# suyashk12/hipgp

Hardware: NVIDIA B200
Metric: toeplitz_matvec_GBps_in_pcg_1e6grid (higher is better)
Workload: dtype f32

## Files before the change

### hipgp_b200/csrc/cols_blk_kernel.cuh

```cuda
#pragma once
#include "fast_kernels.cuh"
#include "tma_maps.cuh"

namespace hipgp {

#ifdef HIPGP_EMU
static inline void nbar_sync(int id, int count) { emu::g_named_barrier[id].sync(count); }
static inline void warp_sync_all() {
    const int tid = (int)(threadIdx.x + blockDim.x * (threadIdx.y + blockDim.y * threadIdx.z));
    emu::g_warp_barrier[tid >> 5].wait();
}
#else
__device__ __forceinline__ void nbar_sync(int id, int count) { asm volatile("bar.sync %0, %1;" ::"r"(id), "r"(count) : "memory"); }
__device__ __forceinline__ void warp_sync_all() { __syncwarp(); }
#endif

template <int GS> __device__ __forceinline__ void blk_sync(int b) {
    if (GS == 32) warp_sync_all(); else nbar_sync(1 + b, GS);
}

template <int R, int S, class T>
__device__ __forceinline__ void blk_fill_pairs(TwPair<T>* dst, const cplx<T>* tab, int tid, int nt) {
    for (int i = tid; i < TwPairs<R>::n * S; i += nt) { const int p = i / S; dst[i] = tw_pair_global<R, S, T>(tab, p, i - p * S); }
}
template <int R, int S, bool SM, class T> __device__ __forceinline__ TwPair<T> blk_pair(const cplx<T>* tab, int p, int j) {
    return SM ? reinterpret_cast<const TwPair<T>*>(tab)[p * S + j] : tw_pair_global<R, S, T>(tab, p, j);
}

template <int R, int S, bool SM, class T>
__device__ __forceinline__ void blk_twiddles(cplx<T>* w, const cplx<T>* tab, int j) {
#pragma unroll
    for (int p = 0; p < TwPairs<R>::n; ++p) {
        const TwPair<T> e = blk_pair<R, S, SM, T>(tab, p, j);
        w[2 * p + 1] = e.a;
        if (2 * p + 2 < R) w[2 * p + 2] = e.b;
    }
}

template <int R, int S, bool SM, bool CONJ, int CH, class T>
__device__ __forceinline__ void blk_twiddle_mul(Lane<T>* v, const cplx<T>* tab, int j) {
    constexpr int PC = CH / 2 > 0 ? CH / 2 : 1;
#pragma unroll
    for (int p0 = 0; p0 < TwPairs<R>::n; p0 += PC) {
        TwPair<T> e[PC];
#pragma unroll
        for (int c = 0; c < PC; ++c) if (p0 + c < TwPairs<R>::n) e[c] = blk_pair<R, S, SM, T>(tab, p0 + c, j);
#pragma unroll
        for (int c = 0; c < PC; ++c) if (p0 + c < TwPairs<R>::n) {
            const int r = 2 * (p0 + c) + 1;
            v[r] = CONJ ? lmulc(v[r], e[c].a) : lmul(v[r], e[c].a);
            if (r + 1 < R) v[r + 1] = CONJ ? lmulc(v[r + 1], e[c].b) : lmul(v[r + 1], e[c].b);
        }
#ifndef HIPGP_EMU
        if (p0 + PC < TwPairs<R>::n) asm volatile("" ::: "memory");
#endif
    }
}

template <class T, int NL, int NT, int MINB, int R0, int R1, int R2>
struct ColsBlkCfg {
    using G = TileGeo<T, NL, R0, R1, R2>;
    static constexpr int Ln = G::Ln, BS = Ln / R0, GS = NT / R0;
    static constexpr int IB2 = (BS / R1) * NL, IB3 = (BS / R2) * NL;
    static constexpr bool ok = (NT % R0 == 0) && (GS % 32 == 0) && (GS == 32 || R0 <= 15) && (IB2 % GS == 0) && (IB3 % GS == 0) &&
                               ((IB2 / GS) * R1 <= 16) && ((IB3 / GS) * R2 <= 16) && (BS % R2 == 0);
    static constexpr size_t tw_bytes = 2 * sizeof(cplx<T>) * (size_t)((R0 / 2) * (Ln / R0) + (R1 / 2) * (BS / R1));
    static constexpr size_t side_bytes = (size_t)(Ln + Ln / R2) * NL * 8;
    static constexpr bool tw_smem = (size_t)MINB * (G::smem_bytes() + side_bytes + tw_bytes + 1024) <= 228 * 1024;
    static constexpr size_t smem_bytes = G::smem_bytes() + side_bytes + (tw_smem ? tw_bytes : 0);
};

template <class T, int NL, int NT, int MINB, int R0, int R1, int R2>
__global__ void __launch_bounds__(NT, MINB) cols_blk_kernel(const HIPGP_GRID_CONSTANT ColsParams<T> P, const HIPGP_GRID_CONSTANT ColsTmaMaps maps) {
    using Cfg = ColsBlkCfg<T, NL, NT, MINB, R0, R1, R2>;
    using G = typename Cfg::G;
    constexpr int Ln = G::Ln, RLAST = R2, LPT = LaneInfo<T>::LPT, TBL = NL * LPT, S0 = Ln / R0;
    constexpr int BS = Cfg::BS, GS = Cfg::GS, S1 = BS / R1;
    constexpr bool TWS = Cfg::tw_smem;
    constexpr int TWCH = R0 >= 16 ? 5 : R0;
    static_assert(Cfg::ok, "radix list / tile shape not usable with block-local middle sections");
    constexpr int LEG0 = G::leg(S0), LEG1 = G::leg(S1);
    constexpr int SPEC_LANE = 8;
    constexpr int SIDE_SLOTS = Ln + Ln / RLAST;
    constexpr int SIDE_LANES = SIDE_SLOTS * NL / 2;
    HIPGP_DYN_SMEM(smem_raw);
    Lane<T>* s = reinterpret_cast<Lane<T>*>(smem_raw);
    unsigned char* side = smem_raw + G::smem_bytes();
    const int tid = threadIdx.x;
    if (P.done_flag && *P.done_flag) return;
    const int blk = tid / GS, u = tid - blk * GS;

    const cplx<T>* tw0 = P.f.twst + P.f.twoff[0];
    const cplx<T>* tw1 = P.f.twst + P.f.twoff[1];
    __shared__ unsigned long long s_bar[3];
    const bool tma_in = P.tma_in != 0, tma_spec = P.tma_spec != 0;
    if ((tma_in || tma_spec) && tid == 0) { tma_bar_init(&s_bar[0]); tma_bar_init(&s_bar[1]); warps_bar_init(&s_bar[2], NT / 32); tma_fence_before_issue(); }
    if (tma_in || tma_spec) __syncthreads();
    if (TWS) {
        TwPair<T>* t0 = reinterpret_cast<TwPair<T>*>(side + Cfg::side_bytes);
        TwPair<T>* t1 = t0 + TwPairs<R0>::n * S0;
        blk_fill_pairs<R0, S0, T>(t0, tw0, tid, NT);
        blk_fill_pairs<R1, S1, T>(t1, tw1, tid, NT);
        tw0 = reinterpret_cast<const cplx<T>*>(t0); tw1 = reinterpret_cast<const cplx<T>*>(t1);
        __syncthreads();
    }

    const int mode = P.mode;
    const size_t pitch = (size_t)P.pitch;
    const size_t spitch = P.spec_pitch ? (size_t)P.spec_pitch : (size_t)P.pitch;
    const long ntiles = (long)P.nx * P.ny * P.nz;
    unsigned tile_bz = 0;
    auto tile_origin = [&](long t, long& c0, size_t& ioff, size_t& ooff) {
        const unsigned tt = (unsigned)t, nx = (unsigned)P.nx, ny = (unsigned)P.ny, nz = (unsigned)P.nz;
        unsigned bx, by, bz;
        if (P.batch_fastest) { bz = tt % nz; const unsigned r = tt / nz; bx = r % nx; by = r / nx; }
        else { bx = tt % nx; const unsigned r = tt / nx; by = r % ny; bz = r / ny; }
        c0 = (long)bx * TBL;
        tile_bz = bz;
        ioff = (size_t)by * P.in_ostride + (size_t)bz * P.in_bstride + c0;
        ooff = (size_t)by * P.out_ostride + (size_t)bz * P.out_bstride + c0;
    };
    auto sslot = [](int p) { return p + (p >> G::LOGRL); };
    const bool spec_smem = P.spec_stage != 0;
    const int n_in = P.n_in, n_out = P.n_out;
    const bool stage_in = P.in_stage != 0;
    const bool zero_hi = is_pow2(R0) && n_in <= Ln / 2;
    const bool out_lo = is_pow2(R0) && n_out <= Ln / 2;
    const size_t rstep = (size_t)S0 * pitch;

    auto prefetch_input = [&](long t) {
        long c0; size_t ioff, ooff;
        tile_origin(t, c0, ioff, ooff);
        const long nvalid = P.inner - c0;
        const cplx<T>* in = P.in + ioff;
        constexpr int NIT = (SIDE_LANES + NT - 1) / NT;
        const int total = n_in * NL;
#pragma unroll
        for (int k = 0; k < NIT; ++k) {
            const int w = tid + k * NT;
            const int i = w / NL, lane = w - i * NL;
            if (w < total && (long)lane * LPT < nvalid) cp_async<16>(side + (size_t)w * 16, in + (size_t)i * pitch + lane * LPT);
        }
        cp_async_commit();
    };

    auto issue_input = [&](long t) {
        long c0; size_t ioff, ooff;
        tile_origin(t, c0, ioff, ooff);
        const unsigned box_bytes = (unsigned)P.tma_in_rows * NL * 16u;
        tma_fence_before_issue();
        tma_bar_expect(&s_bar[0], box_bytes * (unsigned)P.tma_in_nbox);
        for (int k = 0; k < P.tma_in_nbox; ++k)
            tma_load_box3(side + (size_t)k * box_bytes, &maps.in, (int)(2 * c0), k * P.tma_in_rows, (int)tile_bz, &s_bar[0]);
    };
    auto stage_next = [&](long tn) {
        if (tn >= ntiles) return;
        if (tma_in) { if (tid == 0) issue_input(tn); }
        else if (stage_in) prefetch_input(tn);
    };

    stage_next((long)blockIdx.x);
    for (unsigned iter = 0;; ++iter) {
        const long t = (long)blockIdx.x + (long)iter * gridDim.x;
        if (t >= ntiles) break;
        const unsigned ph = iter & 1u;
        long c0; size_t ioff, ooff;
        tile_origin(t, c0, ioff, ooff);
        const long nvalid = P.inner - c0;
        const cplx<T>* in = P.in + ioff;
        cplx<T>* out = P.out + ooff;
        if (tma_in) { tma_bar_wait(&s_bar[0], ph, 8, NT); if (mode != CM_FUSED) __syncthreads(); }
        else { cp_async_wait_all(); __syncthreads(); }

        if (mode != CM_INV) {
#pragma unroll 1
            for (int it = tid; it < S0 * NL; it += NT) {
                const int lane = it % NL, j = it / NL;
                const bool ok = (long)lane * LPT < nvalid;
                Lane<T> v[R0];
                if (tma_in) {
                    const Lane<T>* sp = reinterpret_cast<const Lane<T>*>(side) + (j * NL + lane);
#pragma unroll
                    for (int r = 0; r < R0 / 2; ++r) v[r] = sp[r * S0 * NL];
                    lbfly_zero_hi<R0, T>(v);
                } else if (stage_in) {
                    const Lane<T>* sp = reinterpret_cast<const Lane<T>*>(side) + (j * NL + lane);
                    if (zero_hi) {
#pragma unroll
                        for (int r = 0; r < R0 / 2; ++r) v[r] = (ok && j + r * S0 < n_in) ? sp[r * S0 * NL] : lzero<T>();
                        lbfly_zero_hi<R0, T>(v);
                    } else {
#pragma unroll
                        for (int r = 0; r < R0; ++r) v[r] = (ok && j + r * S0 < n_in) ? sp[r * S0 * NL] : lzero<T>();
                        lbfly<R0, false, T>(v);
                    }
                } else {
                    const cplx<T>* gp = in + (size_t)j * pitch + lane * LPT;
                    if (zero_hi) {
#pragma unroll
                        for (int r = 0; r < R0 / 2; ++r) v[r] = (ok && j + r * S0 < n_in) ? lane_from_global(gp + r * rstep) : lzero<T>();
                        lbfly_zero_hi<R0, T>(v);
                    } else {
#pragma unroll
                        for (int r = 0; r < R0; ++r) v[r] = (ok && j + r * S0 < n_in) ? lane_from_global(gp + r * rstep) : lzero<T>();
                        lbfly<R0, false, T>(v);
                    }
                }
                blk_twiddle_mul<R0, S0, TWS, false, TWCH>(v, tw0, j);
                Lane<T>* base = s + (G::slot(j) * NL + lane);
#pragma unroll
                for (int r = 0; r < R0; ++r) base[r * LEG0] = v[r];
            }
            __syncthreads();
            if (!(mode == CM_FUSED && spec_smem)) stage_next(t + gridDim.x);
        }

        const int pb = blk * BS;
        if (mode == CM_FUSED && spec_smem && tma_spec) {
            if (tid == 0) {
                tma_fence_before_issue();
                tma_bar_expect(&s_bar[1], (unsigned)Cfg::side_bytes);
                tma_load_box3(side, &maps.spec, (int)c0, 0, 0, &s_bar[1]);
            }
        } else if (mode == CM_FUSED && spec_smem) {
            const unsigned char* sp = reinterpret_cast<const unsigned char*>(P.spec) + (size_t)c0 * sizeof(T);
            constexpr int ROWB = NL * SPEC_LANE;
            constexpr int CH = ROWB >= 16 ? 16 : 8, NCH = ROWB / CH;
            constexpr int NIT = (BS * NCH + GS - 1) / GS;
#pragma unroll
            for (int k = 0; k < NIT; ++k) {
                const int w = u + k * GS;
                const int p = pb + w / NCH, c = w % NCH;
                if (w < BS * NCH) cp_async<CH>(side + (size_t)sslot(p) * ROWB + c * CH, sp + (size_t)p * spitch * sizeof(T) + c * CH);
            }
            cp_async_commit();
        }
        if (mode != CM_INV) {
            constexpr int NIT = Cfg::IB2 / GS;
            Lane<T> v[NIT][R1];
            cplx<T> w[NIT][R1];
            Lane<T>* base[NIT];
#pragma unroll
            for (int k = 0; k < NIT; ++k) {
                const int q = u + k * GS;
                const int lane = q % NL, j = q / NL;
                base[k] = s + (G::slot(pb + j) * NL + lane);
                blk_twiddles<R1, S1, TWS>(w[k], tw1, j);
#pragma unroll
                for (int r = 0; r < R1; ++r) v[k][r] = base[k][r * LEG1];
            }
#pragma unroll
            for (int k = 0; k < NIT; ++k) {
                lbfly<R1, false, T>(v[k]);
#pragma unroll
                for (int r = 1; r < R1; ++r) v[k][r] = lmul(v[k][r], w[k][r]);
#pragma unroll
                for (int r = 0; r < R1; ++r) base[k][r * LEG1] = v[k][r];
            }
            if (mode == CM_FUSED && spec_smem) {
                if (tma_spec) tma_bar_wait(&s_bar[1], ph, 9, NT);
                else cp_async_wait_all();
            }
            blk_sync<GS>(blk);
        }
        {
            constexpr int NIT = Cfg::IB3 / GS;
// ... 106 lines not shown
```

### hipgp_b200/csrc/conv_kernels.cuh

```cuda
#pragma once
#include "fft_engine.cuh"

namespace hipgp {

enum RowsFwdMode { RF_PLAIN = 0, RF_PUPDATE = 1, RF_XRUPDATE = 2, RF_SELFDOT = 3 };
enum RowsInvMode { RI_PLAIN = 0, RI_DOT = 1 };
enum DotKind { DOT_PAP = 0, DOT_ZR = 1, DOT_RR = 2 };
enum ColsMode { CM_FWD = 0, CM_INV = 1, CM_FUSED = 2 };
enum SpecKind { SPEC_NONE = 0, SPEC_REAL = 1, SPEC_CPLX = 2, SPEC_CPLX_CONJ = 3 };

struct PcgDev {
    double* zr;
    double* zr_prev;
    double* pAp;
    double* rr;
    const double* rr_all;
    double* partial;
    unsigned* row_cnt;
    unsigned* rhs_cnt;
    int* flags;
    double tol;
    int B;
    int cg_mode;
};

template <class T> __device__ __forceinline__ T warp_sum(T v) {
#pragma unroll
    for (int o = 16; o > 0; o >>= 1) v += __shfl_xor_sync(0xffffffffu, v, o);
    return v;
}

__device__ __forceinline__ void pcg_finalize(const PcgDev& st, int kind, long g0, long g1, int nrows, int tid, int nthreads) {
    __shared__ unsigned s_last;
    __shared__ double s_red[32];
    const int b0 = (int)(g0 / nrows), b1 = (int)((g1 - 1) / nrows);
    for (int b = b0; b <= b1; ++b) {
        const long lo = g0 > (long)b * nrows ? g0 : (long)b * nrows;
        const long hi = g1 < (long)(b + 1) * nrows ? g1 : (long)(b + 1) * nrows;
        __syncthreads();
        if (tid == 0) {
            __threadfence();
            const unsigned done = atomicAdd(st.row_cnt + b, (unsigned)(hi - lo)) + (unsigned)(hi - lo);
            s_last = (done == (unsigned)nrows);
        }
        __syncthreads();
        if (!s_last) continue;
        __threadfence();
        double acc = 0.0;
        const volatile double* part = st.partial + (long)b * nrows;
        for (int i = tid; i < nrows; i += nthreads) acc += part[i];
        acc = warp_sum(acc);
        if ((tid & 31) == 0) s_red[tid >> 5] = acc;
        __syncthreads();
        if (tid < 32) {
            double v = tid < (nthreads >> 5) ? s_red[tid] : 0.0;
            v = warp_sum(v);
            if (tid == 0) {
                st.row_cnt[b] = 0;
                if (kind == DOT_PAP) st.pAp[b] = v;
                else if (kind == DOT_ZR) { st.zr_prev[b] = st.zr[b]; st.zr[b] = v; }
                else {
                    st.rr[b] = v;
                    if (st.cg_mode) { st.zr_prev[b] = st.zr[b]; st.zr[b] = v; }
                }
                __threadfence();
                if (kind == DOT_RR) {
                    const unsigned nb = atomicAdd(st.rhs_cnt, 1u) + 1u;
                    if (nb == (unsigned)st.B) {
                        __threadfence();
                        bool all = true;
                        const volatile double* rr = st.rr_all ? st.rr_all : st.rr;
                        for (int i = 0; i < st.B; ++i) all = all && (sqrt(rr[i]) < st.tol);
                        st.rhs_cnt[0] = 0;
                        st.flags[1] += 1;
                        st.flags[2] = 0;
                        if (all) st.flags[0] = 1;
                    }
                }
            }
        }
    }
}

template <class T>
struct RowsParams {
    const T* in;
    T* out;
    T* v0;
    T* v1;
    const T* v2;
    cplx<T>* W;
    long total_rows;
    int nrows;
    int n_real;
    int L, H;
    long W_pitch;
    int W_rows;
    LineFft<T> f;
    const cplx<T>* twL;
    const cplx<T>* twLp;
    const int* part;
    const int* pairq;
    const int* pairs; const cplx<T>* pairw; int npair0;
    const int* quadq; const cplx<T>* quadw; int nquad;
    int RB, RBP;
    int mode, dot_kind, do_fft;
    int vec_ok;
    int vec16_ok;
    int tma_ok;
    int tma_op;
    const void* spec; int spec_kind;
    PcgDev st;
};

template <class T>
__global__ void __launch_bounds__(256) rows_fwd_kernel(RowsParams<T> P) {
    HIPGP_DYN_SMEM(smem_raw);
    cplx<T>* s = reinterpret_cast<cplx<T>*>(smem_raw);
    const int tid = threadIdx.x, nthreads = blockDim.x;
    const int warp = tid >> 5, lane = tid & 31, nwarps = nthreads >> 5;
    if (P.mode != RF_PLAIN && P.st.flags[0]) return;
    const long g0 = (long)blockIdx.x * P.RB;
    const long g1 = g0 + P.RB < P.total_rows ? g0 + P.RB : P.total_rows;
    const int nl = (int)(g1 - g0);
    const int H = P.H, RBP = P.RBP, n = P.n_real;

    for (int line = warp; line < P.RB; line += nwarps) {
        if (line >= nl) {
            if (P.do_fft) for (int k = lane; k < H; k += 32) s[(size_t)k * RBP + line] = mk<T>(0, 0);
            continue;
        }
        const long g = g0 + line;
        const int b = (int)(g / P.nrows);
        const size_t off = (size_t)g * n;
        T acc = 0;
        T coef = 0;
        bool first = false;
        if (P.mode == RF_PUPDATE) {
            first = P.st.flags[2] != 0;
            coef = first ? (T)0 : (T)(P.st.zr[b] / P.st.zr_prev[b]);
        } else if (P.mode == RF_XRUPDATE) {
            coef = (T)(P.st.zr[b] / P.st.pAp[b]);
        }
        for (int k = lane; k < H; k += 32) {
            T e[2];
#pragma unroll
            for (int h = 0; h < 2; ++h) {
                const int i = 2 * k + h;
                T val = 0;
                if (i < n) {
                    if (P.mode == RF_PLAIN) {
                        val = P.in[off + i];
                    } else if (P.mode == RF_PUPDATE) {
                        const T z = P.in[off + i];
                        val = first ? z : z + coef * P.v0[off + i];
                        P.v0[off + i] = val;
                    } else if (P.mode == RF_SELFDOT) {
                        val = P.in[off + i];
                        acc += val * val;
                    } else {
                        const T pv = P.v2[off + i];
                        P.v1[off + i] = P.v1[off + i] + coef * pv;
                        val = P.v0[off + i] - coef * P.in[off + i];
                        P.v0[off + i] = val;
                        acc += val * val;
                    }
                }
                e[h] = val;
            }
            if (P.do_fft) s[(size_t)k * RBP + line] = mk<T>(e[0], e[1]);
        }
        if (P.mode == RF_XRUPDATE || P.mode == RF_SELFDOT) {
            const double tot = warp_sum((double)acc);
            if (lane == 0) P.st.partial[g] = tot;
        }
    }
    if (P.mode == RF_XRUPDATE) pcg_finalize(P.st, DOT_RR, g0, g1, P.nrows, tid, nthreads);
    if (P.mode == RF_SELFDOT) pcg_finalize(P.st, DOT_ZR, g0, g1, P.nrows, tid, nthreads);
    if (!P.do_fft) return;
    __syncthreads();

    fft_forward(s, RBP, P.RB, P.f, tid, nthreads);

    for (int w = tid; w < H * P.RB; w += nthreads) {
        const int line = w % P.RB, p = w / P.RB;
        const int k = P.f.rev[p];
        if (k == 0) {
            const cplx<T> z = s[line];
            s[line] = mk<T>((T)2 * (z.x + z.y), 0);
            s[(size_t)H * RBP + line] = mk<T>((T)2 * (z.x - z.y), 0);
        } else {
            const int k2 = H - k;
            if (k <= k2) {
                const int p2 = P.f.pos[k2];
                const cplx<T> a = s[(size_t)p * RBP + line], c = conj(s[(size_t)p2 * RBP + line]);
                const cplx<T> E = a + c;
                const cplx<T> d = a - c;
                const cplx<T> O = mk<T>(d.y, -d.x);
                const cplx<T> t = P.twL[k] * O;
                s[(size_t)p * RBP + line] = E + t;
                if (k != k2) s[(size_t)p2 * RBP + line] = conj(E - t);
            }
        }
    }
    __syncthreads();

    for (int line = warp; line < nl; line += nwarps) {
        const long g = g0 + line;
        cplx<T>* dst = P.W + ((size_t)(g / P.nrows) * P.W_rows + (g % P.nrows)) * P.W_pitch;
        for (int q = lane; q <= H; q += 32) dst[q] = s[(size_t)q * RBP + line];
    }
}

template <class T>
__device__ __forceinline__ cplx<T> apply_spec(cplx<T> v, const void* spec, int kind, size_t idx) {
    if (kind == SPEC_REAL) return v * reinterpret_cast<const T*>(spec)[idx];
    const cplx<T> sv = reinterpret_cast<const cplx<T>*>(spec)[idx];
    return kind == SPEC_CPLX ? v * sv : mulc(v, sv);
}

template <class T>
__global__ void __launch_bounds__(256) rows_inv_kernel(RowsParams<T> P) {
    HIPGP_DYN_SMEM(smem_raw);
    cplx<T>* s = reinterpret_cast<cplx<T>*>(smem_raw);
    const int tid = threadIdx.x, nthreads = blockDim.x;
    const int warp = tid >> 5, lane = tid & 31, nwarps = nthreads >> 5;
    if (P.mode != RI_PLAIN && P.st.flags[0]) return;
    const long g0 = (long)blockIdx.x * P.RB;
    const long g1 = g0 + P.RB < P.total_rows ? g0 + P.RB : P.total_rows;
    const int nl = (int)(g1 - g0);
    const int H = P.H, RBP = P.RBP, n = P.n_real;

    for (int line = warp; line < P.RB; line += nwarps) {
        if (line >= nl) {
            for (int q = lane; q <= H; q += 32) s[(size_t)q * RBP + line] = mk<T>(0, 0);
            continue;
        }
        const long g = g0 + line;
        const cplx<T>* src = P.W + ((size_t)(g / P.nrows) * P.W_rows + (g % P.nrows)) * P.W_pitch;
        for (int q = lane; q <= H; q += 32) {
            cplx<T> v = src[q];
            if (P.spec_kind != SPEC_NONE) v = apply_spec(v, P.spec, P.spec_kind, (size_t)q);
            s[(size_t)q * RBP + line] = v;
        }
    }
    __syncthreads();

    for (int w = tid; w < H * P.RB; w += nthreads) {
        const int line = w % P.RB, p = w / P.RB;
        const int k = P.f.rev[p];
        if (k == 0) {
            const T y0 = s[line].x, yh = s[(size_t)H * RBP + line].x;
            s[line] = mk<T>(y0 + yh, y0 - yh);
        } else {
            const int k2 = H - k;
            if (k <= k2) {
                const int p2 = P.f.pos[k2];
                const cplx<T> a = s[(size_t)p * RBP + line], c = conj(s[(size_t)p2 * RBP + line]);
                const cplx<T> E = a + c;
                const cplx<T> O = mulc(a - c, P.twL[k]);
                const cplx<T> iO = mk<T>(-O.y, O.x);
                s[(size_t)p * RBP + line] = E + iO;
                if (k != k2) s[(size_t)p2 * RBP + line] = conj(E - iO);
            }
        }
    }
    __syncthreads();

    fft_inverse(s, RBP, P.RB, P.f, tid, nthreads);

    for (int line = warp; line < nl; line += nwarps) {
        const long g = g0 + line;
        const size_t off = (size_t)g * n;
        T acc = 0;
        for (int k = lane; k < H; k += 32) {
            const cplx<T> z = s[(size_t)k * RBP + line];
            const int i = 2 * k;
            if (i < n) { P.out[off + i] = z.x; if (P.mode == RI_DOT) acc += z.x * P.v0[off + i]; }
            if (i + 1 < n) { P.out[off + i + 1] = z.y; if (P.mode == RI_DOT) acc += z.y * P.v0[off + i + 1]; }
        }
        if (P.mode == RI_DOT) {
            const double tot = warp_sum((double)acc);
            if (lane == 0) P.st.partial[g] = tot;
        }
    }
    if (P.mode == RI_DOT) pcg_finalize(P.st, P.dot_kind, g0, g1, P.nrows, tid, nthreads);
}

template <class T>
struct ColsParams {
    const cplx<T>* in;
    cplx<T>* out;
    int n_in, n_out;
    long inner;
    long pitch;
    long in_ostride, in_bstride, out_ostride, out_bstride;
    LineFft<T> f;
    int TB, TBP;
    int mode;
    const void* spec; int spec_kind;
    long spec_pitch;
    int spec_stage;
    int in_stage;
    int nx, ny, nz;
    int tma_in, tma_in_rows, tma_in_nbox;
    int tma_spec;
    int batch_fastest;
    const int* done_flag;
    int out_split_len; long out_split_stride;
    int in_split_len; long in_split_stride;
};
template <class T> __device__ __forceinline__ size_t cols_rowoff(int i, long pitch, int split_len, long split_stride) {
    return split_len ? (size_t)(i / split_len) * split_stride + (size_t)(i % split_len) * pitch : (size_t)i * pitch;
}

template <class T>
__global__ void __launch_bounds__(512) cols_pass_kernel(ColsParams<T> P) {
    HIPGP_DYN_SMEM(smem_raw);
    cplx<T>* s = reinterpret_cast<cplx<T>*>(smem_raw);
    const int tid = threadIdx.x, nthreads = blockDim.x;
    if (P.done_flag && *P.done_flag) return;
    const long c0 = (long)blockIdx.x * P.TB;
    const int nc = (int)(P.inner - c0 < P.TB ? P.inner - c0 : P.TB);
    const int L = P.f.Ln, TB = P.TB, TBP = P.TBP;
    const cplx<T>* in = P.in + (size_t)blockIdx.y * P.in_ostride + (size_t)blockIdx.z * P.in_bstride + c0;
    cplx<T>* out = P.out + (size_t)blockIdx.y * P.out_ostride + (size_t)blockIdx.z * P.out_bstride + c0;

    const int rows_in = P.mode == CM_INV ? L : P.n_in;
    for (int w = tid; w < L * TB; w += nthreads) {
        const int c = w % TB, i = w / TB;
        cplx<T> v = mk<T>(0, 0);
        if (i < rows_in && c < nc) v = in[cols_rowoff<T>(i, P.pitch, P.in_split_len, P.in_split_stride) + c];
        s[(size_t)i * TBP + c] = v;
    }
    __syncthreads();

    if (P.mode != CM_INV) fft_forward(s, TBP, TB, P.f, tid, nthreads);
    if (P.mode == CM_FUSED) {
        for (int w = tid; w < L * TB; w += nthreads) {
            const int c = w % TB, i = w / TB;
            if (c < nc) s[(size_t)i * TBP + c] = apply_spec(s[(size_t)i * TBP + c], P.spec, P.spec_kind, (size_t)i * (P.spec_pitch ? P.spec_pitch : P.pitch) + c0 + c);
        }
        __syncthreads();
    }
    if (P.mode != CM_FWD) fft_inverse(s, TBP, TB, P.f, tid, nthreads);

    const int rows_out = P.mode == CM_FWD ? L : P.n_out;
    for (int w = tid; w < rows_out * TB; w += nthreads) {
        const int c = w % TB, i = w / TB;
        if (c < nc) out[cols_rowoff<T>(i, P.pitch, P.out_split_len, P.out_split_stride) + c] = s[(size_t)i * TBP + c];
    }
}


}
```

### hipgp_b200/csrc/fast_kernels.cuh

```cuda
#pragma once
#include "lane_fft.cuh"

namespace hipgp {

template <class T> __device__ __forceinline__ void ld2(const T* p, bool vec, T& a, T& b, bool ok0, bool ok1) {
    if (vec && ok1) { const cplx<T> t = ld_stream(reinterpret_cast<const cplx<T>*>(p)); a = t.x; b = t.y; }
    else { a = ok0 ? ld_stream(p) : (T)0; b = ok1 ? ld_stream(p + 1) : (T)0; }
}
template <class T> __device__ __forceinline__ void st2(T* p, bool vec, T a, T b, bool ok0, bool ok1) {
    if (vec && ok1) { st_stream(reinterpret_cast<cplx<T>*>(p), mk<T>(a, b)); }
    else { if (ok0) st_stream(p, a); if (ok1) st_stream(p + 1, b); }
}

__device__ __forceinline__ double team_sum(double v, int tw) {
    for (int o = tw >> 1; o > 0; o >>= 1) v += __shfl_xor_sync(0xffffffffu, v, o);
    return v;
}

__device__ __forceinline__ Lane<float> lane_spec(Lane<float> v, const void* spec, int kind, size_t idx) {
    if (kind == SPEC_REAL) {
        const cplx<float> sv = ld_stream(reinterpret_cast<const cplx<float>*>(reinterpret_cast<const float*>(spec) + idx));
        return lmul_real2(v, sv.x, sv.y);
    }
    const cplx<float>* sp = reinterpret_cast<const cplx<float>*>(spec) + idx;
    const cplx<float> w0 = ld_stream(sp), w1 = ld_stream(sp + 1);
    return kind == SPEC_CPLX ? lmul_cplx2<false>(v, w0, w1) : lmul_cplx2<true>(v, w0, w1);
}
__device__ __forceinline__ Lane<double> lane_spec(Lane<double> v, const void* spec, int kind, size_t idx) {
    if (kind == SPEC_REAL) return lscale(v, ld_stream(reinterpret_cast<const double*>(spec) + idx));
    const cplx<double> w = ld_stream(reinterpret_cast<const cplx<double>*>(spec) + idx);
    return kind == SPEC_CPLX ? lmul(v, w) : lmulc(v, w);
}
__device__ __forceinline__ Lane<float> lane_spec_smem(Lane<float> v, const void* p) {
    const float2 s2 = *reinterpret_cast<const float2*>(p);
    Lane<float> r; r.re = __fmul2_rn(v.re, s2); r.im = __fmul2_rn(v.im, s2); return r;
}
__device__ __forceinline__ Lane<double> lane_spec_smem(Lane<double> v, const void* p) { return lscale(v, *reinterpret_cast<const double*>(p)); }

template <class T, int NL, int NT, int MINB, int R0, int... Rs>
__global__ void __launch_bounds__(NT, MINB) cols_fast_kernel(ColsParams<T> P) {
    using G = TileGeo<T, NL, R0, Rs...>;
    constexpr int Ln = G::Ln, NST = G::NST, RLAST = G::RLAST, LPT = LaneInfo<T>::LPT, TBL = NL * LPT, S0 = Ln / R0;
    HIPGP_DYN_SMEM(smem_raw);
    Lane<T>* s = reinterpret_cast<Lane<T>*>(smem_raw);
    const int tid = threadIdx.x;
    if (P.done_flag && *P.done_flag) return;
    const int mode = P.mode;
    const size_t pitch = (size_t)P.pitch;
    const size_t spitch = P.spec_pitch ? (size_t)P.spec_pitch : (size_t)P.pitch;
    const long ntiles = (long)P.nx * P.ny * P.nz;
    auto tile_origin = [&](long t, long& c0, size_t& ioff, size_t& ooff) {
        long bx, by, bz;
        if (P.batch_fastest) { bz = t % P.nz; const long r = t / P.nz; bx = r % P.nx; by = r / P.nx; }
        else { bx = t % P.nx; const long r = t / P.nx; by = r % P.ny; bz = r / P.ny; }
        c0 = bx * TBL;
        ioff = (size_t)by * P.in_ostride + (size_t)bz * P.in_bstride + c0;
        ooff = (size_t)by * P.out_ostride + (size_t)bz * P.out_bstride + c0;
    };

    if constexpr (NST == 1) {
        for (long t = blockIdx.x; t < ntiles; t += gridDim.x) {
            long c0; size_t ioff, ooff;
            tile_origin(t, c0, ioff, ooff);
            const long nvalid = P.inner - c0;
            const cplx<T>* in = P.in + ioff;
            cplx<T>* out = P.out + ooff;
            for (int lane = tid; lane < NL; lane += NT) {
                if ((long)lane * LPT >= nvalid) continue;
                const int rows_in = mode == CM_INV ? Ln : P.n_in;
                const int rows_out = mode == CM_FWD ? Ln : P.n_out;
                Lane<T> v[R0];
#pragma unroll
                for (int r = 0; r < R0; ++r)
                    v[r] = r < rows_in ? lane_from_global(in + cols_rowoff<T>(r, P.pitch, P.in_split_len, P.in_split_stride) + lane * LPT) : lzero<T>();
                if (mode != CM_INV) lbfly<R0, false, T>(v);
                if (mode == CM_FUSED) {
#pragma unroll
                    for (int r = 0; r < R0; ++r) v[r] = lane_spec(v[r], P.spec, P.spec_kind, (size_t)r * spitch + c0 + lane * LPT);
                }
                if (mode != CM_FWD) lbfly<R0, true, T>(v);
#pragma unroll
                for (int r = 0; r < R0; ++r)
                    if (r < rows_out) lane_to_global(out + cols_rowoff<T>(r, P.pitch, P.out_split_len, P.out_split_stride) + lane * LPT, v[r]);
            }
        }
        return;
    } else {
        constexpr int LEG0 = G::leg(S0);
        constexpr int SPEC_LANE = 8;
        constexpr int SIDE_SLOTS = Ln + Ln / RLAST;
        constexpr int SIDE_LANES = SIDE_SLOTS * NL / 2;
        unsigned char* side = smem_raw + G::smem_bytes();
        auto sslot = [](int p) { return p + (p >> G::LOGRL); };
        const cplx<T>* tw0 = P.f.twst + P.f.twoff[0];
        const bool spec_smem = P.spec_stage != 0;
        const int n_in = P.n_in, n_out = P.n_out;
        const bool stage_in = P.in_stage != 0;
        const bool zero_hi = is_pow2(R0) && n_in <= Ln / 2;
        const bool out_lo = is_pow2(R0) && n_out <= Ln / 2;
        const size_t rstep = (size_t)S0 * pitch;

        auto prefetch_input = [&](long t) {
            long c0; size_t ioff, ooff;
            tile_origin(t, c0, ioff, ooff);
            const long nvalid = P.inner - c0;
            const cplx<T>* in = P.in + ioff;
            constexpr int NIT = (SIDE_LANES + NT - 1) / NT;
            const int total = n_in * NL;
#pragma unroll
            for (int k = 0; k < NIT; ++k) {
                const int w = tid + k * NT;
                const int i = w / NL, lane = w - i * NL;
                if (w < total && (long)lane * LPT < nvalid) cp_async<16>(side + (size_t)w * 16, in + (size_t)i * pitch + lane * LPT);
            }
            cp_async_commit();
        };

        long t = blockIdx.x;
        if (stage_in && t < ntiles) prefetch_input(t);
        for (; t < ntiles; t += gridDim.x) {
            long c0; size_t ioff, ooff;
            tile_origin(t, c0, ioff, ooff);
            const long nvalid = P.inner - c0;
            const cplx<T>* in = P.in + ioff;
            cplx<T>* out = P.out + ooff;
            cp_async_wait_all();
            __syncthreads();

            if (mode != CM_INV) {
#pragma unroll 1
                for (int it = tid; it < S0 * NL; it += NT) {
                    const int lane = it % NL, j = it / NL;
                    const bool ok = (long)lane * LPT < nvalid;
                    cplx<T> w[R0];
                    lane_twiddles<R0, S0>(w, tw0, j);
                    Lane<T> v[R0];
                    if (stage_in) {
                        const Lane<T>* sp = reinterpret_cast<const Lane<T>*>(side) + (j * NL + lane);
                        if (zero_hi) {
#pragma unroll
                            for (int r = 0; r < R0 / 2; ++r) v[r] = (ok && j + r * S0 < n_in) ? sp[r * S0 * NL] : lzero<T>();
                            lbfly_zero_hi<R0, T>(v);
                        } else {
#pragma unroll
                            for (int r = 0; r < R0; ++r) v[r] = (ok && j + r * S0 < n_in) ? sp[r * S0 * NL] : lzero<T>();
                            lbfly<R0, false, T>(v);
                        }
                    } else {
                        const cplx<T>* gp = in + (size_t)j * pitch + lane * LPT;
                        if (zero_hi) {
#pragma unroll
                            for (int r = 0; r < R0 / 2; ++r) v[r] = (ok && j + r * S0 < n_in) ? lane_from_global(gp + r * rstep) : lzero<T>();
                            lbfly_zero_hi<R0, T>(v);
                        } else {
#pragma unroll
                            for (int r = 0; r < R0; ++r) v[r] = (ok && j + r * S0 < n_in) ? lane_from_global(gp + r * rstep) : lzero<T>();
                            lbfly<R0, false, T>(v);
                        }
                    }
#pragma unroll
                    for (int r = 1; r < R0; ++r) v[r] = lmul(v[r], w[r]);
                    Lane<T>* base = s + (G::slot(j) * NL + lane);
#pragma unroll
                    for (int r = 0; r < R0; ++r) base[r * LEG0] = v[r];
                }
                __syncthreads();
                if (spec_smem) {
                    const unsigned char* sp = reinterpret_cast<const unsigned char*>(P.spec) + (size_t)c0 * sizeof(T);
                    constexpr int ROWB = NL * SPEC_LANE;
                    constexpr int CH = ROWB >= 16 ? 16 : 8, NCH = ROWB / CH;
                    constexpr int NIT = (Ln * NCH + NT - 1) / NT;
#pragma unroll
                    for (int k = 0; k < NIT; ++k) {
                        const int w = tid + k * NT;
                        const int p = w / NCH, c = w - p * NCH;
                        if (w < Ln * NCH) cp_async<CH>(side + (size_t)sslot(p) * ROWB + c * CH, sp + (size_t)p * spitch * sizeof(T) + c * CH);
                    }
                    cp_async_commit();
                }
                LaneMidFwd<G, T, NL, NT, Ln / R0, 1, Rs...>::run(s, P.f, tid);
                if (spec_smem) { cp_async_wait_all(); __syncthreads(); }
            }

            {
#pragma unroll 2
                for (int it = tid; it < (Ln / RLAST) * NL; it += NT) {
                    const int lane = it % NL, bf = it / NL;
                    const bool ok = (long)lane * LPT < nvalid;
                    const int p0 = bf * RLAST;
                    Lane<T>* base = s + (G::slot(p0) * NL + lane);
                    Lane<T> v[RLAST];
                    if (mode == CM_INV) {
                        const cplx<T>* gp = in + cols_rowoff<T>(p0, P.pitch, P.in_split_len, P.in_split_stride) + lane * LPT;
#pragma unroll
                        for (int r = 0; r < RLAST; ++r) v[r] = ok ? lane_from_global(gp + r * pitch) : lzero<T>();
                    } else {
#pragma unroll
                        for (int r = 0; r < RLAST; ++r) v[r] = base[r * NL];
                        lbfly<RLAST, false, T>(v);
                    }
                    if (mode == CM_FUSED) {
                        if (spec_smem) {
                            const unsigned char* sp = side + ((size_t)sslot(p0) * NL + lane) * SPEC_LANE;
#pragma unroll
                            for (int r = 0; r < RLAST; ++r) v[r] = lane_spec_smem(v[r], sp + r * NL * SPEC_LANE);
                        } else if (ok) {
                            const size_t sidx = (size_t)p0 * spitch + c0 + lane * LPT;
#pragma unroll
                            for (int r = 0; r < RLAST; ++r) v[r] = lane_spec(v[r], P.spec, P.spec_kind, sidx + (size_t)r * spitch);
                        }
                    }
                    if (mode == CM_FWD) {
                        if (ok) {
                            cplx<T>* gp = out + cols_rowoff<T>(p0, P.pitch, P.out_split_len, P.out_split_stride) + lane * LPT;
#pragma unroll
                            for (int r = 0; r < RLAST; ++r) lane_to_global(gp + r * pitch, v[r]);
                        }
                    } else {
                        lbfly<RLAST, true, T>(v);
#pragma unroll
                        for (int r = 0; r < RLAST; ++r) base[r * NL] = v[r];
                    }
                }
                __syncthreads();
            }
            if (stage_in && t + gridDim.x < ntiles) prefetch_input(t + gridDim.x);
            if (mode == CM_FWD) continue;

            LaneMidInv<G, T, NL, NT, Ln / R0, 1, Rs...>::run(s, P.f, tid);
            {
#pragma unroll 1
                for (int it = tid; it < S0 * NL; it += NT) {
                    const int lane = it % NL, j = it / NL;
                    const bool ok = (long)lane * LPT < nvalid;
                    cplx<T> w[R0];
                    lane_twiddles<R0, S0>(w, tw0, j);
                    const Lane<T>* base = s + (G::slot(j) * NL + lane);
                    Lane<T> v[R0];
#pragma unroll
                    for (int r = 0; r < R0; ++r) v[r] = base[r * LEG0];
#pragma unroll
                    for (int r = 1; r < R0; ++r) v[r] = lmulc(v[r], w[r]);
                    cplx<T>* gp = out + (size_t)j * pitch + lane * LPT;
                    lbfly<R0, true, T>(v);
                    if (ok) {
                        if (out_lo) {
#pragma unroll
                            for (int r = 0; r < R0 / 2; ++r) if (j + r * S0 < n_out) lane_to_global(gp + r * rstep, v[r]);
                        } else {
#pragma unroll
                            for (int r = 0; r < R0; ++r) if (j + r * S0 < n_out) lane_to_global(gp + r * rstep, v[r]);
                        }
                    }
                }
            }
        }
    }
}

struct __align__(8) QuadIdx { int a, b; };

template <class T, int NL, int NT, int MINB, int R0, int... Rs>
__global__ void __launch_bounds__(NT, MINB) rows_fwd_fast_kernel(RowsParams<T> P) {
    using G = TileGeo<T, NL, R0, Rs...>;
    constexpr int H = G::Ln, NST = G::NST, RLAST = G::RLAST, LPT = LaneInfo<T>::LPT, NROW = NL * LPT, S0 = H / R0;
    constexpr int LEG0 = G::leg(NST > 1 ? S0 : 1);
    HIPGP_DYN_SMEM(smem_raw);
    Lane<T>* s = reinterpret_cast<Lane<T>*>(smem_raw);
    const int tid = threadIdx.x;
    if (P.mode != RF_PLAIN && P.st.flags[0]) return;
    const long g0 = (long)blockIdx.x * NROW;
    const long g1 = g0 + NROW < P.total_rows ? g0 + NROW : P.total_rows;
    const int nl = (int)(g1 - g0);
    const int n = P.n_real;
    const int mode = P.mode;
    const bool vec = ((n & 1) == 0) && P.vec_ok;
    const bool first_it = (mode == RF_PUPDATE) && (P.st.flags[2] != 0);
    const bool want_dot = (mode == RF_XRUPDATE || mode == RF_SELFDOT);
    __shared__ T s_coef[32];
    __shared__ long s_wbase[32];
    __shared__ double s_part[32];
    if (tid < NROW && tid < nl) {
        const long gr = g0 + tid;
        const long b = gr / P.nrows;
        s_wbase[tid] = (b * P.W_rows + (gr - b * P.nrows)) * P.W_pitch;
        T coef = 0;
        if (mode == RF_PUPDATE) coef = first_it ? (T)0 : (T)(P.st.zr[b] / P.st.zr_prev[b]);
        else if (mode == RF_XRUPDATE) coef = (T)(P.st.zr[b] / P.st.pAp[b]);
        s_coef[tid] = coef;
    }
    __syncthreads();

    const int SROW = (n + 3) & ~3;
    T* side = reinterpret_cast<T*>(smem_raw + G::smem_bytes());
    bool streamed = false;
#ifndef HIPGP_EMU
    bool bulk_store_pending = false;
    if (P.tma_ok && P.vec16_ok && SROW == n && (mode == RF_PLAIN || mode == RF_SELFDOT || P.tma_op)) {
        constexpr int CH = 16 / (int)sizeof(T);
        __shared__ __align__(8) unsigned long long s_mbar;
        const unsigned bytes = (unsigned)((size_t)nl * n * sizeof(T));
        const size_t goff = (size_t)g0 * n;
        T* bufA = reinterpret_cast<T*>(smem_raw);
        T* bufB = bufA + (size_t)NROW * SROW;
        const bool two = mode == RF_PUPDATE && !first_it, three = mode == RF_XRUPDATE;
        if (tid == 0) { mbar_init(&s_mbar, 1); fence_proxy_async(); }
        __syncthreads();
        if (tid == 0) {
            mbar_arrive_expect_tx(&s_mbar, bytes * (three ? 3u : (two ? 2u : 1u)));
            bulk_g2s(side, P.in + goff, bytes, &s_mbar);
            if (two) bulk_g2s(bufA, (const T*)P.v0 + goff, bytes, &s_mbar);
            if (three) { bulk_g2s(bufA, (const T*)P.v0 + goff, bytes, &s_mbar); bulk_g2s(bufB, P.v2 + goff, bytes, &s_mbar); }
        }
        constexpr int NW = NT / 32, WPR = NW > NROW ? NW / NROW : 1;
        constexpr int tws = WPR > 1 ? 32 : (H / CH >= 32 ? 32 : (H / CH >= 16 ? 16 : (H / CH >= 8 ? 8 : 4)));
        constexpr int rpw = 32 / tws, TW = WPR > 1 ? 32 * WPR : tws, rstep = WPR > 1 ? NW / WPR : NW * rpw;
        const int warp = tid >> 5, l32 = tid & 31;
        const int ln = WPR > 1 ? l32 + 32 * (warp % WPR) : l32 % tws;
        const int nch = n / CH;
        mbar_wait(&s_mbar, 0);
        if (mode != RF_PLAIN && !(mode == RF_PUPDATE && first_it)) {
            for (int rbase = WPR > 1 ? warp / WPR : warp * rpw; rbase < nl; rbase += rstep) {
                const int row = rbase + (WPR > 1 ? 0 : l32 / tws);
                const bool ractive = row < nl;
                double acc = 0.0;
                if (ractive) {
                    T* srow = side + (size_t)row * SROW;
                    const T* arow = bufA + (size_t)row * SROW;
                    const T* brow = bufB + (size_t)row * SROW;
                    const size_t off = goff + (size_t)row * n;
                    const T coef = s_coef[row];
                    if (three) {
                        constexpr int BS = 4;
                        for (int cb = ln; cb < nch; cb += TW * BS) {
                            Vec16<T> xv[BS];
#pragma unroll
                            for (int k = 0; k < BS; ++k) { const int c = cb + TW * k; if (c < nch) xv[k] = ldv_stream((const T*)P.v1 + off + (size_t)c * CH); }
#pragma unroll
                            for (int k = 0; k < BS; ++k) {
                                const int c = cb + TW * k;
                                if (c < nch) {
                                    Vec16<T> q = *reinterpret_cast<const Vec16<T>*>(srow + c * CH);
                                    const Vec16<T> rv = *reinterpret_cast<const Vec16<T>*>(arow + c * CH);
                                    const Vec16<T> pv = *reinterpret_cast<const Vec16<T>*>(brow + c * CH);
#pragma unroll
                                    for (int e = 0; e < CH; ++e) { xv[k].v[e] = xv[k].v[e] + coef * pv.v[e]; q.v[e] = rv.v[e] - coef * q.v[e]; acc += (double)(q.v[e] * q.v[e]); }
                                    stv_stream(P.v1 + off + (size_t)c * CH, xv[k]);
                                    *reinterpret_cast<Vec16<T>*>(srow + c * CH) = q;
                                }
                            }
                        }
                    } else if (two) {
                        for (int c = ln; c < nch; c += TW) {
                            Vec16<T> z = *reinterpret_cast<const Vec16<T>*>(srow + c * CH);
                            const Vec16<T> pv = *reinterpret_cast<const Vec16<T>*>(arow + c * CH);
#pragma unroll
                            for (int e = 0; e < CH; ++e) z.v[e] = z.v[e] + coef * pv.v[e];
                            *reinterpret_cast<Vec16<T>*>(srow + c * CH) = z;
                        }
                    } else {
                        for (int c = ln; c < nch; c += TW) {
                            const Vec16<T> z = *reinterpret_cast<const Vec16<T>*>(srow + c * CH);
#pragma unroll
                            for (int e = 0; e < CH; ++e) acc += (double)(z.v[e] * z.v[e]);
                        }
                    }
                }
                if (want_dot) {
                    acc = team_sum(acc, WPR > 1 ? 32 : tws);
                    if (ractive && (WPR > 1 ? l32 == 0 : ln == 0)) s_part[row * WPR + warp % WPR] = acc;
                }
            }
        }
        if (mode == RF_PUPDATE || mode == RF_XRUPDATE) {
            fence_proxy_async();
            __syncthreads();
            if (tid == 0) {
                asm volatile("cp.async.bulk.global.shared::cta.bulk_group [%0], [%1], %2;" ::"l"(P.v0 + goff), "r"((unsigned)__cvta_generic_to_shared(side)), "r"(bytes) : "memory");
                asm volatile("cp.async.bulk.commit_group;" ::: "memory");
            }
            bulk_store_pending = true;
        }
        if (want_dot) {
            __syncthreads();
            if (tid < nl) { double a = 0.0; for (int k = 0; k < WPR; ++k) a += s_part[tid * WPR + k]; P.st.partial[g0 + tid] = a; }
        }
        streamed = true;
    }
#endif
    if (!streamed) {
        constexpr int CH = 16 / (int)sizeof(T);
        constexpr int NW = NT / 32, WPR = NW > NROW ? NW / NROW : 1;
        const bool chunked = P.vec16_ok && (n % CH == 0);
        constexpr int tws = WPR > 1 ? 32 : (H / CH >= 32 ? 32 : (H / CH >= 16 ? 16 : (H / CH >= 8 ? 8 : 4)));
        constexpr int rpw = 32 / tws;
        constexpr int TW = WPR > 1 ? 32 * WPR : tws;
        const int warp = tid >> 5, l32 = tid & 31;
        const int ln = WPR > 1 ? l32 + 32 * (warp % WPR) : l32 % tws;
        constexpr int rstep = WPR > 1 ? NW / WPR : NW * rpw;
        for (int rbase = WPR > 1 ? warp / WPR : warp * rpw; rbase < nl; rbase += rstep) {
            const int row = rbase + (WPR > 1 ? 0 : l32 / tws);
            const bool ractive = row < nl;
            T* srow = side + (size_t)(ractive ? row : 0) * SROW;
            const size_t off = (size_t)(g0 + (ractive ? row : 0)) * n;
            const T coef = s_coef[ractive ? row : 0];
            double acc = 0.0;
            if (!ractive) {
            } else if (chunked) {
                const int nch = n / CH;
                auto finish = [&](int c, Vec16<T> a) {
                    if (want_dot) {
#pragma unroll
                        for (int k = 0; k < CH; ++k) acc += (double)(a.v[k] * a.v[k]);
                    }
                    *reinterpret_cast<Vec16<T>*>(srow + c * CH) = a;
                };
#define HIPGP_PIPE(LOAD, PROC)                                                                              \
                {                                                                                           \
                    const int step = TW * BS;                                                               \
                    int cb = ln;                                                                            \
                    LOAD(0, cb);                                                                            \
                    for (; cb < nch; cb += 2 * step) {                                                      \
                        if (cb + step < nch) { LOAD(1, cb + step); }                                        \
                        PROC(0, cb);                                                                        \
                        if (cb + 2 * step < nch) { LOAD(0, cb + 2 * step); }                                \
                        if (cb + step < nch) { PROC(1, cb + step); }                                        \
                    }                                                                                       \
                }
                if (mode == RF_XRUPDATE) {
                    constexpr int BS = 1;
                    Vec16<T> a[2][BS], pv[2][BS], xv[2][BS], rv[2][BS];
#define HIPGP_LD(S, CB)                                                                                     \
                    _Pragma("unroll") for (int k = 0; k < BS; ++k) {                                        \
                        const int c = (CB) + TW * k;                                                        \
                        if (c < nch) {                                                                      \
                            const size_t o = off + (size_t)c * CH;                                          \
                            a[S][k] = ldv_stream(P.in + o); pv[S][k] = ldv_stream(P.v2 + o);                \
                            xv[S][k] = ldv_stream((const T*)P.v1 + o); rv[S][k] = ldv_stream((const T*)P.v0 + o); \
                        }                                                                                   \
                    }
#define HIPGP_PR(S, CB)                                                                                     \
                    _Pragma("unroll") for (int k = 0; k < BS; ++k) {                                        \
                        const int c = (CB) + TW * k;                                                        \
                        if (c < nch) {                                                                      \
                            const size_t o = off + (size_t)c * CH;                                          \
                            _Pragma("unroll") for (int e = 0; e < CH; ++e) {                                \
                                xv[S][k].v[e] = xv[S][k].v[e] + coef * pv[S][k].v[e];                       \
                                a[S][k].v[e] = rv[S][k].v[e] - coef * a[S][k].v[e];                         \
                            }                                                                               \
                            stv_stream(P.v1 + o, xv[S][k]);                                                 \
                            stv_stream(P.v0 + o, a[S][k]);                                                  \
                            finish(c, a[S][k]);                                                             \
                        }                                                                                   \
                    }
                    HIPGP_PIPE(HIPGP_LD, HIPGP_PR)
#undef HIPGP_LD
#undef HIPGP_PR
                } else if (mode == RF_PUPDATE && !first_it) {
                    constexpr int BS = 2;
                    Vec16<T> a[2][BS], pv[2][BS];
#define HIPGP_LD(S, CB)                                                                                     \
                    _Pragma("unroll") for (int k = 0; k < BS; ++k) {                                        \
                        const int c = (CB) + TW * k;                                                        \
                        if (c < nch) { const size_t o = off + (size_t)c * CH; a[S][k] = ldv_stream(P.in + o); pv[S][k] = ldv_stream((const T*)P.v0 + o); } \
                    }
#define HIPGP_PR(S, CB)                                                                                     \
                    _Pragma("unroll") for (int k = 0; k < BS; ++k) {                                        \
                        const int c = (CB) + TW * k;                                                        \
                        if (c < nch) {                                                                      \
                            _Pragma("unroll") for (int e = 0; e < CH; ++e) a[S][k].v[e] = a[S][k].v[e] + coef * pv[S][k].v[e]; \
                            stv_stream(P.v0 + off + (size_t)c * CH, a[S][k]);                               \
                            finish(c, a[S][k]);                                                             \
                        }                                                                                   \
                    }
                    HIPGP_PIPE(HIPGP_LD, HIPGP_PR)
#undef HIPGP_LD
#undef HIPGP_PR
                } else {
                    constexpr int BS = 4;
                    const bool wr = mode == RF_PUPDATE;
                    Vec16<T> a[2][BS];
#define HIPGP_LD(S, CB)                                                                                     \
                    _Pragma("unroll") for (int k = 0; k < BS; ++k) { const int c = (CB) + TW * k; if (c < nch) a[S][k] = ldv_stream(P.in + off + (size_t)c * CH); }
#define HIPGP_PR(S, CB)                                                                                     \
                    _Pragma("unroll") for (int k = 0; k < BS; ++k) {                                        \
                        const int c = (CB) + TW * k;                                                        \
                        if (c < nch) { if (wr) stv_stream(P.v0 + off + (size_t)c * CH, a[S][k]); finish(c, a[S][k]); } \
                    }
                    HIPGP_PIPE(HIPGP_LD, HIPGP_PR)
#undef HIPGP_LD
#undef HIPGP_PR
                }
#undef HIPGP_PIPE
            } else {
                for (int i = ln; i < n; i += TW) {
                    const size_t o = off + i;
                    T a = ld_stream(P.in + o);
                    if (mode == RF_PUPDATE) {
                        if (!first_it) a = a + coef * ld_stream((const T*)P.v0 + o);
                        st_stream(P.v0 + o, a);
                    } else if (mode == RF_XRUPDATE) {
                        const T pv = ld_stream(P.v2 + o);
                        st_stream(P.v1 + o, ld_stream((const T*)P.v1 + o) + coef * pv);
                        a = ld_stream((const T*)P.v0 + o) - coef * a;
                        st_stream(P.v0 + o, a);
                    }
                    if (want_dot) acc += (double)(a * a);
                    srow[i] = a;
                }
            }
            if (ractive) for (int i = n + ln; i < SROW; i += TW) srow[i] = (T)0;
            if (want_dot) {
                acc = team_sum(acc, WPR > 1 ? 32 : tws);
                if (ractive && (WPR > 1 ? l32 == 0 : ln == 0)) s_part[row * WPR + warp % WPR] = acc;
            }
        }
        if (want_dot) {
            __syncthreads();
            if (tid < nl) { double a = 0.0; for (int k = 0; k < WPR; ++k) a += s_part[tid * WPR + k]; P.st.partial[g0 + tid] = a; }
        }
    }
    __syncthreads();
    if (want_dot) pcg_finalize(P.st, mode == RF_XRUPDATE ? DOT_RR : DOT_ZR, g0, g1, P.nrows, tid, NT);

    {
        const bool zero_hi = is_pow2(R0) && R0 > 1 && (n + 1) / 2 <= H / 2;
        const cplx<T>* tw0 = P.f.twst + P.f.twoff[0];
#pragma unroll 1
        for (int it = tid; it < S0 * NL; it += NT) {
            const int lane = it % NL, j = it / NL;
            cplx<T> w[R0];
            if (NST > 1) lane_twiddles<R0, S0>(w, tw0, j);
            const T* srow0 = side + (size_t)(lane * LPT) * SROW;
            const T* srow1 = side + (size_t)(lane * LPT + LPT - 1) * SROW;
            const bool ok0 = lane * LPT < nl, ok1 = lane * LPT + LPT - 1 < nl;
            auto elem = [&](int r) -> Lane<T> {
                const int i = 2 * (j + r * S0);
                const bool in_row = i < SROW;
                const cplx<T> e0 = (ok0 && in_row) ? *reinterpret_cast<const cplx<T>*>(srow0 + i) : mk<T>(0, 0);
                const cplx<T> e1 = (LPT == 2 && ok1 && in_row) ? *reinterpret_cast<const cplx<T>*>(srow1 + i) : mk<T>(0, 0);
                return lane_make(e0, e1);
            };
            Lane<T> v[R0];
            if (zero_hi) {
#pragma unroll
                for (int r = 0; r < R0 / 2; ++r) v[r] = elem(r);
                lbfly_zero_hi<R0, T>(v);
            } else {
#pragma unroll
                for (int r = 0; r < R0; ++r) v[r] = elem(r);
                lbfly<R0, false, T>(v);
            }
            if (NST > 1) {
#pragma unroll
                for (int r = 1; r < R0; ++r) v[r] = lmul(v[r], w[r]);
            }
            Lane<T>* base = s + (G::slot(j) * NL + lane);
#pragma unroll
            for (int r = 0; r < R0; ++r) base[r * LEG0] = v[r];
        }
    }
    __syncthreads();

    if constexpr (NST > 1) {
        LaneMidFwd<G, T, NL, NT, H / R0, 1, Rs...>::run(s, P.f, tid);
        lane_stage<G, T, NL, NT, RLAST, RLAST, false>(s, P.f.twst, tid);
        __syncthreads();
    }

    constexpr int NPAIR0 = NST > 1 ? RLAST / 2 + 1 : H / 2 + 1;
    constexpr int NQUAD = NST > 1 ? (H - RLAST) / 4 : 0;
#pragma unroll 1
    for (int it = tid; it < NPAIR0 * NL; it += NT) {
        const int lane = it % NL, pi = it / NL;
        const QuadIdx pq = reinterpret_cast<const QuadIdx*>(P.pairs)[pi];
        const int q = pq.a, q2 = pq.b;
        Lane<T> Xa, Xb;
        bool two;
        if (q == 0) {
            const Lane<T> z = s[lane];
            Lane<T> zs; zs.re = z.im; zs.im = z.re;
            Xa = lscale(z + zs, (T)2); Xb = lscale(z - zs, (T)2);
            Xa.im = lzero<T>().im; Xb.im = lzero<T>().im;
            two = true;
        } else {
            const cplx<T> wq = ldg_c(P.pairw + pi);
            const Lane<T> a = s[G::slot(q) * NL + lane], c = lconj(s[G::slot(q2) * NL + lane]);
            const Lane<T> E = a + c;
            const Lane<T> t = lmul(lmi<false>(a - c), wq);
            Xa = E + t; Xb = lconj(E - t);
            two = q2 != q;
        }
#pragma unroll
        for (int l = 0; l < LPT; ++l) {
            const int row = lane * LPT + l;
            if (row < nl) {
                cplx<T>* dst = P.W + s_wbase[row];
                WRow<T>::store1(dst, q, lane_get(Xa, l));
                if (two) WRow<T>::store1(dst, q2, lane_get(Xb, l));
            }
        }
    }
    if constexpr (NQUAD > 0) {
        constexpr int QIT = (NQUAD * NL + NT - 1) / NT;
        QuadIdx qq[QIT]; cplx<T> wa[QIT], wa1[QIT];
#pragma unroll
        for (int k = 0; k < QIT; ++k) {
            const int it = tid + k * NT, qi = it / NL;
            if (it < NQUAD * NL) { qq[k] = reinterpret_cast<const QuadIdx*>(P.quadq)[qi]; wa[k] = ldg_c(P.quadw + 2 * qi); wa1[k] = ldg_c(P.quadw + 2 * qi + 1); }
        }
#pragma unroll
        for (int k = 0; k < QIT; ++k) {
            const int it = tid + k * NT, lane = it % NL;
            if (it < NQUAD * NL) {
                const Lane<T>* pa = s + (G::slot(qq[k].a) * NL + lane);
                const Lane<T>* pb = s + (G::slot(qq[k].b) * NL + lane);
                const Lane<T> za = pa[0], za1 = pa[NL], zb = pb[0], zb1 = pb[NL];
                Lane<T> c = lconj(zb1);
                Lane<T> E = za + c;
                Lane<T> t = lmul(lmi<false>(za - c), wa[k]);
                const Lane<T> Xa = E + t, Xb1 = lconj(E - t);
                c = lconj(zb);
                E = za1 + c;
                t = lmul(lmi<false>(za1 - c), wa1[k]);
                const Lane<T> Xa1 = E + t, Xb = lconj(E - t);
                const bool self = qq[k].a == qq[k].b;
#pragma unroll
                for (int l = 0; l < LPT; ++l) {
                    const int row = lane * LPT + l;
                    if (row < nl) {
                        cplx<T>* dst = P.W + s_wbase[row];
                        if (self) WRow<T>::store2(dst, qq[k].a, lane_get(Xa, l), lane_get(Xb1, l));
                        else { WRow<T>::store2(dst, qq[k].a, lane_get(Xa, l), lane_get(Xa1, l)); WRow<T>::store2(dst, qq[k].b, lane_get(Xb, l), lane_get(Xb1, l)); }
                    }
                }
            }
        }
    }
#ifndef HIPGP_EMU
    if (bulk_store_pending && tid == 0) asm volatile("cp.async.bulk.wait_group.read 0;" ::: "memory");
#endif
}

template <class T, int NL, int NT, int MINB, int R0, int... Rs>
__global__ void __launch_bounds__(NT, MINB) rows_inv_fast_kernel(RowsParams<T> P) {
    using G = TileGeo<T, NL, R0, Rs...>;
    constexpr int H = G::Ln, NST = G::NST, RLAST = G::RLAST, LPT = LaneInfo<T>::LPT, NROW = NL * LPT, S0 = H / R0;
    constexpr int LEG0 = G::leg(NST > 1 ? S0 : 1);
    HIPGP_DYN_SMEM(smem_raw);
    Lane<T>* s = reinterpret_cast<Lane<T>*>(smem_raw);
    const int tid = threadIdx.x;
    if (P.mode != RI_PLAIN && P.st.flags[0]) return;
    const long g0 = (long)blockIdx.x * NROW;
    const long g1 = g0 + NROW < P.total_rows ? g0 + NROW : P.total_rows;
    const int nl = (int)(g1 - g0);
    const int n = P.n_real;

    __shared__ long s_wbase[32];
    __shared__ double s_part[32];
    if (tid < NROW && tid < nl) {
        const long gr = g0 + tid;
        const long b = gr / P.nrows;
        s_wbase[tid] = (b * P.W_rows + (gr - b * P.nrows)) * P.W_pitch;
    }
    __syncthreads();

    const int spec_kind = P.spec_kind;
    constexpr int NPAIR0 = NST > 1 ? RLAST / 2 + 1 : H / 2 + 1;
    constexpr int NQUAD = NST > 1 ? (H - RLAST) / 4 : 0;
#pragma unroll 1
    for (int it = tid; it < NPAIR0 * NL; it += NT) {
        const int lane = it % NL, pi = it / NL;
        const QuadIdx pq = reinterpret_cast<const QuadIdx*>(P.pairs)[pi];
        const int q = pq.a, q2 = pq.b;
        const cplx<T> wq = ldg_c(P.pairw + pi);
        cplx<T> ya[LPT], yc[LPT];
#pragma unroll
        for (int l = 0; l < LPT; ++l) {
            const int row = lane * LPT + l;
            ya[l] = mk<T>(0, 0); yc[l] = mk<T>(0, 0);
            if (row < nl) {
                const cplx<T>* src = P.W + s_wbase[row];
                ya[l] = WRow<T>::load1(src, q); yc[l] = WRow<T>::load1(src, q2);
                if (spec_kind != SPEC_NONE) { ya[l] = apply_spec(ya[l], P.spec, spec_kind, (size_t)q); yc[l] = apply_spec(yc[l], P.spec, spec_kind, (size_t)q2); }
            }
        }
        const Lane<T> a = lane_make(ya[0], ya[LPT - 1]);
        Lane<T> c = lane_make(yc[0], yc[LPT - 1]);
        if (q == 0) {
            Lane<T> z; z.re = (a + c).re; z.im = (a - c).re;
            s[lane] = z;
        } else {
            c = lconj(c);
            const Lane<T> E = a + c;
            const Lane<T> iO = lmi<true>(lmulc(a - c, wq));
            s[G::slot(q) * NL + lane] = E + iO;
            if (q2 != q) s[G::slot(q2) * NL + lane] = lconj(E - iO);
        }
    }
    if constexpr (NQUAD > 0) {
        constexpr int QIT = (NQUAD * NL + NT - 1) / NT;
        QuadIdx qq[QIT]; cplx<T> wa[QIT], wa1[QIT];
        cplx<T> ya[QIT][LPT], ya1[QIT][LPT], yb[QIT][LPT], yb1[QIT][LPT];
#pragma unroll
        for (int k = 0; k < QIT; ++k) {
            int it = tid + k * NT;
            it = it < NQUAD * NL ? it : NQUAD * NL - 1;
            const int qi = it / NL;
            qq[k] = reinterpret_cast<const QuadIdx*>(P.quadq)[qi]; wa[k] = ldg_c(P.quadw + 2 * qi); wa1[k] = ldg_c(P.quadw + 2 * qi + 1);
        }
#pragma unroll
        for (int k = 0; k < QIT; ++k) {
            int it = tid + k * NT;
            it = it < NQUAD * NL ? it : NQUAD * NL - 1;
            const int lane = it % NL;
#pragma unroll
            for (int l = 0; l < LPT; ++l) {
                const int row = lane * LPT + l;
                const cplx<T>* src = P.W + s_wbase[row < nl ? row : nl - 1];
                WRow<T>::load2(src, qq[k].a, ya[k][l], ya1[k][l]);
                WRow<T>::load2(src, qq[k].b, yb[k][l], yb1[k][l]);
            }
        }
#pragma unroll
        for (int k = 0; k < QIT; ++k) {
            const int it = tid + k * NT, lane = it % NL;
            if (it < NQUAD * NL) {
                const bool self = qq[k].a == qq[k].b;
                if (spec_kind != SPEC_NONE) {
#pragma unroll
                    for (int l = 0; l < LPT; ++l) {
                        ya[k][l] = apply_spec(ya[k][l], P.spec, spec_kind, (size_t)qq[k].a); ya1[k][l] = apply_spec(ya1[k][l], P.spec, spec_kind, (size_t)qq[k].a + 1);
                        yb[k][l] = apply_spec(yb[k][l], P.spec, spec_kind, (size_t)qq[k].b); yb1[k][l] = apply_spec(yb1[k][l], P.spec, spec_kind, (size_t)qq[k].b + 1);
                    }
                }
                const Lane<T> A = lane_make(ya[k][0], ya[k][LPT - 1]), A1 = lane_make(ya1[k][0], ya1[k][LPT - 1]);
                const Lane<T> Bn = lane_make(yb[k][0], yb[k][LPT - 1]), B1 = lane_make(yb1[k][0], yb1[k][LPT - 1]);
                Lane<T>* pa = s + (G::slot(qq[k].a) * NL + lane);
                Lane<T>* pb = s + (G::slot(qq[k].b) * NL + lane);
                Lane<T> c = lconj(B1);
                Lane<T> E = A + c;
                Lane<T> iO = lmi<true>(lmulc(A - c, wa[k]));
                pa[0] = E + iO;
                pb[NL] = lconj(E - iO);
                if (!self) {
                    c = lconj(Bn);
                    E = A1 + c;
                    iO = lmi<true>(lmulc(A1 - c, wa1[k]));
                    pa[NL] = E + iO;
                    pb[0] = lconj(E - iO);
                }
            }
        }
    }
    __syncthreads();

    if constexpr (NST > 1) {
        lane_stage<G, T, NL, NT, RLAST, RLAST, true>(s, P.f.twst, tid);
        __syncthreads();
        LaneMidInv<G, T, NL, NT, H / R0, 1, Rs...>::run(s, P.f, tid);
    }

    const int SROW = (n + 3) & ~3;
    T* side = reinterpret_cast<T*>(smem_raw + G::smem_bytes());
    const bool want_dot = P.mode == RI_DOT;
    {
        const bool out_lo = is_pow2(R0) && R0 > 1 && (n + 1) / 2 <= H / 2;
        const cplx<T>* tw0 = P.f.twst + P.f.twoff[0];
#pragma unroll 1
        for (int it = tid; it < S0 * NL; it += NT) {
            const int lane = it % NL, j = it / NL;
            cplx<T> w[R0];
            if (NST > 1) lane_twiddles<R0, S0>(w, tw0, j);
            const Lane<T>* base = s + (G::slot(j) * NL + lane);
            Lane<T> v[R0];
#pragma unroll
            for (int r = 0; r < R0; ++r) v[r] = base[r * LEG0];
            if (NST > 1) {
#pragma unroll
                for (int r = 1; r < R0; ++r) v[r] = lmulc(v[r], w[r]);
            }
            lbfly<R0, true, T>(v);
            T* srow0 = side + (size_t)(lane * LPT) * SROW;
            T* srow1 = side + (size_t)(lane * LPT + LPT - 1) * SROW;
            auto put = [&](int r) {
                const int i = 2 * (j + r * S0);
                if (i < SROW) {
                    *reinterpret_cast<cplx<T>*>(srow0 + i) = lane_get(v[r], 0);
                    if (LPT == 2) *reinterpret_cast<cplx<T>*>(srow1 + i) = lane_get(v[r], LPT - 1);
                }
            };
            if (out_lo) {
#pragma unroll
                for (int r = 0; r < R0 / 2; ++r) put(r);
            } else {
#pragma unroll
                for (int r = 0; r < R0; ++r) put(r);
            }
        }
    }
#ifndef HIPGP_EMU
    const bool tma_any = P.tma_ok && P.vec16_ok && SROW == n;
    const bool tma_out = !want_dot && tma_any;
    const bool tma_dot = want_dot && tma_any;
    if (tma_any) fence_proxy_async();
#else
    const bool tma_out = false, tma_dot = false;
#endif
    __syncthreads();
#ifndef HIPGP_EMU
    if (tma_out) {
        if (tid == 0) bulk_s2g(P.out + (size_t)g0 * n, side, (unsigned)((size_t)nl * n * sizeof(T)));
        return;
    }
    if (tma_dot && tid == 0) bulk_s2g_issue(P.out + (size_t)g0 * n, side, (unsigned)((size_t)nl * n * sizeof(T)));
#endif
    {
        constexpr int CH = 16 / (int)sizeof(T);
        constexpr int NW = NT / 32, WPR = NW > NROW ? NW / NROW : 1;
        const bool chunked = P.vec16_ok && (n % CH == 0);
        constexpr int tws = WPR > 1 ? 32 : (H / CH >= 32 ? 32 : (H / CH >= 16 ? 16 : (H / CH >= 8 ? 8 : 4)));
        constexpr int rpw = 32 / tws;
        constexpr int TW = WPR > 1 ? 32 * WPR : tws;
        const int warp = tid >> 5, l32 = tid & 31;
        const int ln = WPR > 1 ? l32 + 32 * (warp % WPR) : l32 % tws;
        constexpr int rstep = WPR > 1 ? NW / WPR : NW * rpw;
        for (int rbase = WPR > 1 ? warp / WPR : warp * rpw; rbase < nl; rbase += rstep) {
            const int row = rbase + (WPR > 1 ? 0 : l32 / tws);
            const bool ractive = row < nl;
            const T* srow = side + (size_t)(ractive ? row : 0) * SROW;
            const size_t off = (size_t)(g0 + (ractive ? row : 0)) * n;
            double acc = 0.0;
            if (!ractive) {
            } else if (chunked) {
                const int nch = n / CH;
                constexpr int BS = 8;
                for (int cb = ln; cb < nch; cb += TW * BS) {
                    Vec16<T> ov[BS];
                    if (want_dot) {
#pragma unroll
                        for (int k = 0; k < BS; ++k) { const int c = cb + TW * k; if (c < nch) ov[k] = ldv_stream((const T*)P.v0 + off + (size_t)c * CH); }
                    }
#pragma unroll
                    for (int k = 0; k < BS; ++k) {
                        const int c = cb + TW * k;
                        if (c < nch) {
                            const Vec16<T> y = *reinterpret_cast<const Vec16<T>*>(srow + c * CH);
                            if (want_dot) {
#pragma unroll
                                for (int e = 0; e < CH; ++e) acc += (double)(y.v[e] * ov[k].v[e]);
                            }
                            if (!tma_dot) stv_stream(P.out + off + (size_t)c * CH, y);
                        }
                    }
                }
            } else if (sizeof(T) == 4 && (n & 1) == 0 && P.vec_ok) {
                for (int c = ln; c < n / 2; c += TW) {
                    const cplx<T> y = *reinterpret_cast<const cplx<T>*>(srow + 2 * c);
                    if (want_dot) {
                        const cplx<T> ov = ld_stream(reinterpret_cast<const cplx<T>*>((const T*)P.v0 + off + 2 * c));
                        acc += (double)(y.x * ov.x) + (double)(y.y * ov.y);
                    }
                    st_stream(reinterpret_cast<cplx<T>*>(P.out + off + 2 * c), y);
                }
            } else {
                for (int i = ln; i < n; i += TW) {
                    const T y = srow[i];
                    if (want_dot) acc += (double)(y * ld_stream((const T*)P.v0 + off + i));
                    st_stream(P.out + off + i, y);
                }
            }
            if (want_dot) {
                acc = team_sum(acc, WPR > 1 ? 32 : tws);
                if (ractive && (WPR > 1 ? l32 == 0 : ln == 0)) s_part[row * WPR + warp % WPR] = acc;
            }
        }
    }
#ifndef HIPGP_EMU
    if (tma_dot && tid == 0) bulk_s2g_wait();
#endif
    if (want_dot) {
        __syncthreads();
        constexpr int WPR2 = (NT / 32) > NROW ? (NT / 32) / NROW : 1;
        if (tid < nl) { double a = 0.0; for (int k = 0; k < WPR2; ++k) a += s_part[tid * WPR2 + k]; P.st.partial[g0 + tid] = a; }
        pcg_finalize(P.st, P.dot_kind, g0, g1, P.nrows, tid, NT);
    }
}

}
```

### hipgp_b200/csrc/fast_launch.cuh

```cuda
#pragma once
#include "plan_types.cuh"
#include "fast_kernels.cuh"
#include "cols_blk_kernel.cuh"

namespace hipgp {

constexpr int cfg_min(int a, int b) { return a < b ? a : b; }
constexpr int cfg_max(int a, int b) { return a > b ? a : b; }
constexpr int pow2_floor(int x) { return x <= 1 ? 1 : 2 * pow2_floor(x / 2); }

template <class T, int... Rs>
struct FastCfg {
    using List = RL<Rs...>;
    static constexpr int Ln = RLInfo<List>::N;
    static constexpr int RMAX = RLMax<List>::value;
    static constexpr int BFN = Ln / RMAX;
    static constexpr int NL0 = pow2_floor(cfg_max(1, cfg_min(256 / cfg_max(BFN, 1), 4096 / Ln)));
    static constexpr int NL = cfg_max(1, cfg_min(16, NL0));
    static constexpr int NT = cfg_min(512, cfg_max(32, (BFN * NL + 31) / 32 * 32));
    static constexpr int MINB = cfg_max(1, 512 / NT);
    static constexpr int LPT = LaneInfo<T>::LPT;
    static constexpr int S0 = Ln / (RLInfo<List>::count ? RLFirst<List>::value : 1);
    static constexpr int NLR = cfg_max(1, NL / 4);
    static constexpr int NTR = cfg_min(512, cfg_max(32, (BFN * NLR + 31) / 32 * 32));
    static constexpr int MINBR = cfg_max(1, 512 / NTR);
    static constexpr int RLASTv = RLLast<List>::value;
    static constexpr bool WIDEN = (NL == 1) && (RLInfo<List>::count > 1) && ((size_t)(Ln + Ln / RLASTv) * 2 * 24 <= 222 * 1024);
    static constexpr int CMULF = 2;
    static constexpr bool CMUL = !WIDEN && NL == 2 && ((size_t)(Ln + Ln / RLASTv) * NL * CMULF * 24 <= 222 * 1024) && BFN * NL * CMULF <= 512;
    static constexpr int NLC = WIDEN ? 2 : (CMUL ? NL * CMULF : NL);
    static constexpr int NTC = (WIDEN || CMUL) ? cfg_min(512, cfg_max(32, (BFN * NLC + 31) / 32 * 32)) : NT;
    static constexpr int MINBC = (WIDEN || CMUL) ? cfg_max(1, 512 / NTC) : MINB;
};

static void launch_check(const char* what, int len, int nl, int nt, size_t smem, long grid) {
    const cudaError_t e = cudaGetLastError();
    if (e != cudaSuccess)
        throw Error(std::string(what) + " launch failed (length " + std::to_string(len) + ", lanes " + std::to_string(nl) + ", threads " + std::to_string(nt) +
                    ", shared " + std::to_string(smem) + " B, grid " + std::to_string(grid) + "): " + cudaGetErrorString(e));
}

template <class T, int... Rs>
static void launch_rows_fast_t(hipgp_plan* pl, bool inverse, RowsParams<T>& P, cudaStream_t st) {
    using C = FastCfg<T, Rs...>;
    using G = TileGeo<T, C::NLR, Rs...>;
    constexpr int NROW = C::NLR * C::LPT;
    static_assert(NROW <= 32, "per-row scalars are held in 32-entry shared arrays");
    P.RB = NROW; P.RBP = NROW;
    {
        constexpr int NST = G::NST, H = C::Ln;
        const int want_q = NST > 1 ? (H - G::RLAST) / 4 : 0, want_p = NST > 1 ? G::RLAST / 2 + 1 : H / 2 + 1;
        if (P.nquad != want_q || P.npair0 != want_p) throw Error("internal: unexpected r2c pair structure for H = " + std::to_string(H));
    }
    const size_t smem = G::smem_bytes() + sizeof(T) * (size_t)((P.n_real + 3) & ~3) * NROW;
    if (smem > 227 * 1024) throw Error("row pass: rows too long for the shared-memory side buffer");
    static const char* env_nt = getenv("HIPGP_NO_TMA");
    static const char* env_nf = getenv("HIPGP_NO_TMA_FUSED");
    P.tma_ok = env_nt ? 0 : 1;
    P.tma_op = (!env_nf && !inverse && 2 * sizeof(T) * (size_t)((P.n_real + 3) & ~3) * NROW <= G::smem_bytes()) ? 1 : 0;
    dim3 grid((unsigned)((P.total_rows + NROW - 1) / NROW));
    PROF_BEGIN(pl, inverse ? 2 : 0, st);
    if (inverse) {
        auto k = rows_inv_fast_kernel<T, C::NLR, C::NTR, C::MINBR, Rs...>;
        if (smem > 40 * 1024) HIPGP_SET_MAX_SMEM(k, smem);
        HIPGP_LAUNCH(k, grid, dim3(C::NTR), smem, st, P);
    } else {
        auto k = rows_fwd_fast_kernel<T, C::NLR, C::NTR, C::MINBR, Rs...>;
        if (smem > 40 * 1024) HIPGP_SET_MAX_SMEM(k, smem);
        HIPGP_LAUNCH(k, grid, dim3(C::NTR), smem, st, P);
    }
    PROF_END(pl, st);
    launch_check("row pass", C::Ln, C::NLR, C::NTR, smem, (long)grid.x);
    pl->launches++;
}

template <class K>
static int resident_ctas(K kernel, int nthreads, size_t smem) {
#ifdef HIPGP_EMU
    (void)kernel; (void)nthreads; (void)smem;
    return 3;
#else
    int dev = 0, sms = 0, per = 0;
    CK(cudaGetDevice(&dev));
    CK(cudaDeviceGetAttribute(&sms, cudaDevAttrMultiProcessorCount, dev));
    CK(cudaOccupancyMaxActiveBlocksPerMultiprocessor(&per, kernel, nthreads, smem));
    return sms * (per > 0 ? per : 1);
#endif
}

template <class T, int LEN, int... Rs>
static void launch_cols_fast_t(hipgp_plan* pl, ColsParams<T>& P, long n_outer, long B, cudaStream_t st) {
    using C = FastCfg<T, Rs...>;
    using G = TileGeo<T, C::NLC, Rs...>;
    static_assert(C::Ln == LEN, "radix list does not multiply to the length");
    constexpr int TBL = C::NLC * C::LPT;
    P.TB = TBL; P.TBP = TBL;
    if ((P.in_split_len && (P.mode != CM_INV || P.in_split_len % G::RLAST)) || (P.out_split_len && (P.mode != CM_FWD || P.out_split_len % G::RLAST)))
        throw Error("split row blocks are supported for forward-only outputs / inverse-only inputs, in multiples of the last radix");
    const size_t side_bytes = G::NST > 1 ? (size_t)(C::Ln + C::Ln / G::RLAST) * C::NLC * 8 : 0;
    static const char* env_ns = getenv("HIPGP_NO_STAGE");
    const bool use_side = G::NST > 1 && !env_ns;
    P.spec_stage = (use_side && P.mode == CM_FUSED && P.spec_kind == SPEC_REAL) ? 1 : 0;
    P.in_stage = (use_side && P.mode != CM_INV && (size_t)P.n_in * C::NLC * 16 <= side_bytes) ? 1 : 0;
    const size_t smem = G::smem_bytes() + ((P.spec_stage || P.in_stage) ? side_bytes : 0);
    P.nx = (int)((P.inner + TBL - 1) / TBL); P.ny = (int)n_outer; P.nz = (int)B;
    {
        const size_t spec_bytes = (size_t)G::Ln * (size_t)P.inner * (P.spec_kind == SPEC_REAL ? sizeof(T) : 2 * sizeof(T));
        P.batch_fastest = (P.mode == CM_FUSED && B > 1 && spec_bytes > ((size_t)48 << 20) && (size_t)TBL * sizeof(cplx<T>) >= 128) ? 1 : 0;
    }
    auto k = cols_fast_kernel<T, C::NLC, C::NTC, C::MINBC, Rs...>;
    if (smem > 40 * 1024) HIPGP_SET_MAX_SMEM(k, smem);
    const long ntiles = (long)P.nx * P.ny * P.nz;
    const long grid = std::min<long>(ntiles, resident_ctas(k, C::NTC, smem));
    PROF_BEGIN(pl, 1, st);
    HIPGP_LAUNCH(k, dim3((unsigned)grid), dim3(C::NTC), smem, st, P);
    PROF_END(pl, st);
    launch_check("column pass", C::Ln, C::NLC, C::NTC, smem, grid);
    pl->launches++;
}

template <class T, int LEN, int... Rs> struct ColsBlkLaunch {
    static bool run(hipgp_plan*, ColsParams<T>&, long, long, cudaStream_t) { return false; }
};
template <class T, int LEN, int R0, int R1, int R2> struct ColsBlkLaunch<T, LEN, R0, R1, R2> {
    using C = FastCfg<T, R0, R1, R2>;
    using Cfg = ColsBlkCfg<T, C::NLC, C::NTC, C::MINBC, R0, R1, R2>;
    static bool run(hipgp_plan* pl, ColsParams<T>& P, long n_outer, long B, cudaStream_t st) {
        if constexpr (!Cfg::ok) { (void)pl; (void)P; (void)n_outer; (void)B; (void)st; return false; }
        else {
            static const char* env_blk = getenv("HIPGP_COLS_BLK");
            if (env_blk && env_blk[0] == '0') return false;
            static const char* env_tws = getenv("HIPGP_BLK_NEEDS_TWS");
            if (!Cfg::tw_smem && env_tws && env_tws[0] == '1') return false;
            if ((long)((P.inner + C::NLC * C::LPT - 1) / (C::NLC * C::LPT)) * n_outer * B >= (1L << 31)) return false;
            using G = typename Cfg::G;
            constexpr int TBL = C::NLC * C::LPT;
            P.TB = TBL; P.TBP = TBL;
            if ((P.in_split_len && (P.mode != CM_INV || P.in_split_len % G::RLAST)) || (P.out_split_len && (P.mode != CM_FWD || P.out_split_len % G::RLAST)))
                throw Error("split row blocks are supported for forward-only outputs / inverse-only inputs, in multiples of the last radix");
            static const char* env_ns = getenv("HIPGP_NO_STAGE");
            const bool use_side = !env_ns;
            P.spec_stage = (use_side && P.mode == CM_FUSED && P.spec_kind == SPEC_REAL) ? 1 : 0;
            P.in_stage = (use_side && P.mode != CM_INV && (size_t)P.n_in * C::NLC * 16 <= Cfg::side_bytes) ? 1 : 0;
            const size_t smem = Cfg::smem_bytes;
            P.nx = (int)((P.inner + TBL - 1) / TBL); P.ny = (int)n_outer; P.nz = (int)B;
            {
                const size_t spec_bytes = (size_t)G::Ln * (size_t)P.inner * (P.spec_kind == SPEC_REAL ? sizeof(T) : 2 * sizeof(T));
                P.batch_fastest = (P.mode == CM_FUSED && B > 1 && spec_bytes > ((size_t)48 << 20) && (size_t)TBL * sizeof(cplx<T>) >= 128) ? 1 : 0;
            }
            ColsTmaMaps maps{};
            P.tma_in = P.tma_spec = 0;
            static const char* env_nt = getenv("HIPGP_NO_TMA_COLS");
            if (!env_nt) {
                constexpr int HALF = C::Ln / 2;
                const int nbox = (HALF + 255) / 256;
                if (P.in_stage && P.n_in <= HALF && P.in_ostride == 0 && n_outer == 1 && HALF % nbox == 0 && is_pow2(R0)) {
                    const unsigned long long dim[3] = {(unsigned long long)(2 * P.pitch), (unsigned long long)P.n_in, (unsigned long long)B};
                    const unsigned long long bstr = (unsigned long long)(P.in_bstride ? P.in_bstride : (long)P.n_in * P.pitch);
                    const unsigned long long str[2] = {(unsigned long long)P.pitch * sizeof(cplx<T>), bstr * sizeof(cplx<T>)};
                    const unsigned box[3] = {(unsigned)(2 * TBL), (unsigned)(HALF / nbox), 1u};
                    if (encode_map3(&maps.in, P.in, (int)sizeof(T), dim, str, box)) { P.tma_in = 1; P.tma_in_rows = HALF / nbox; P.tma_in_nbox = nbox; }
                }
                if (P.spec_stage && C::Ln / R2 <= 256 && (TBL * sizeof(T)) % 16 == 0) {
                    const long sp = P.spec_pitch ? P.spec_pitch : P.pitch;
                    const unsigned long long dim[3] = {(unsigned long long)sp, (unsigned long long)R2, (unsigned long long)(C::Ln / R2)};
                    const unsigned long long str[2] = {(unsigned long long)sp * sizeof(T), (unsigned long long)sp * R2 * sizeof(T)};
                    const unsigned box[3] = {(unsigned)TBL, (unsigned)(R2 + 1), (unsigned)(C::Ln / R2)};
                    if (encode_map3(&maps.spec, P.spec, (int)sizeof(T), dim, str, box)) P.tma_spec = 1;
                }
            }
            auto k = cols_blk_kernel<T, C::NLC, C::NTC, C::MINBC, R0, R1, R2>;
            if (smem > 40 * 1024) HIPGP_SET_MAX_SMEM(k, smem);
            const long ntiles = (long)P.nx * P.ny * P.nz;
            const long grid = std::min<long>(ntiles, resident_ctas(k, C::NTC, smem));
            PROF_BEGIN(pl, 1, st);
            HIPGP_LAUNCH(k, dim3((unsigned)grid), dim3(C::NTC), smem, st, P, maps);
            PROF_END(pl, st);
            launch_check("column pass (block-local)", C::Ln, C::NLC, C::NTC, smem, grid);
            pl->launches++;
            return true;
        }
    }
};

template <class T>
static bool cols_lane_aligned(const ColsParams<T>& P) {
    constexpr long A = 16 / (long)sizeof(cplx<T>);
    auto al = [&](long v) { return v % A == 0; };
    return ((uintptr_t)P.in % 16 == 0) && ((uintptr_t)P.out % 16 == 0) && ((uintptr_t)P.spec % 16 == 0) && al(P.pitch) && al(P.in_ostride) &&
           al(P.in_bstride) && al(P.out_ostride) && al(P.out_bstride) && al(P.in_split_stride) && al(P.out_split_stride) &&
           al(P.spec_pitch);
}

template <class T, int LEN> struct FastList;
#define X(LEN, ...)                                                                                         \
    template <class T> struct FastList<T, LEN> {                                                            \
        static void rows(hipgp_plan* pl, bool inv, RowsParams<T>& P, cudaStream_t st) { launch_rows_fast_t<T, __VA_ARGS__>(pl, inv, P, st); } \
        static void cols(hipgp_plan* pl, ColsParams<T>& P, long no, long B, cudaStream_t st) {         \
            if (!ColsBlkLaunch<T, LEN, __VA_ARGS__>::run(pl, P, no, B, st)) launch_cols_fast_t<T, LEN, __VA_ARGS__>(pl, P, no, B, st); } \
    };
HIPGP_FAST_LIST(X)
#undef X
template <class T, int LEN> void launch_rows_fast_len(hipgp_plan* pl, bool inverse, RowsParams<T>& P, cudaStream_t st) { FastList<T, LEN>::rows(pl, inverse, P, st); }
template <class T, int LEN> bool launch_cols_fast_len(hipgp_plan* pl, ColsParams<T>& P, long n_outer, long B, cudaStream_t st) {
    if (!cols_lane_aligned<T>(P)) throw Error("column pass: pointers / strides are not 16-byte aligned");
    FastList<T, LEN>::cols(pl, P, n_outer, B, st);
    return true;
}
}
```

### hipgp_b200/csrc/lane_fft.cuh

```cuda
#pragma once
#include "conv_kernels.cuh"

namespace hipgp {

#ifdef HIPGP_EMU
static inline float2 __fadd2_rn(float2 a, float2 b) { return float2{a.x + b.x, a.y + b.y}; }
static inline float2 __fmul2_rn(float2 a, float2 b) { return float2{a.x * b.x, a.y * b.y}; }
static inline float2 __ffma2_rn(float2 a, float2 b, float2 c) { return float2{std::fma(a.x, b.x, c.x), std::fma(a.y, b.y, c.y)}; }
#endif

template <class T> struct Lane;
template <> struct __align__(16) Lane<float> { float2 re, im; };
template <> struct __align__(16) Lane<double> { double re, im; };
template <class T> struct LaneInfo { static constexpr int LPT = sizeof(T) == 4 ? 2 : 1; };

__device__ __forceinline__ float2 bc2(float s) { return make_float2(s, s); }
__device__ __forceinline__ float2 neg2(float2 a) { return make_float2(-a.x, -a.y); }

template <class T> __device__ __forceinline__ Lane<T> lzero();
template <> __device__ __forceinline__ Lane<float> lzero<float>() { Lane<float> r; r.re = bc2(0.f); r.im = bc2(0.f); return r; }
template <> __device__ __forceinline__ Lane<double> lzero<double>() { Lane<double> r; r.re = 0.0; r.im = 0.0; return r; }

__device__ __forceinline__ Lane<float> operator+(Lane<float> a, Lane<float> b) { Lane<float> r; r.re = __fadd2_rn(a.re, b.re); r.im = __fadd2_rn(a.im, b.im); return r; }
__device__ __forceinline__ Lane<float> operator-(Lane<float> a, Lane<float> b) { Lane<float> r; r.re = __fadd2_rn(a.re, neg2(b.re)); r.im = __fadd2_rn(a.im, neg2(b.im)); return r; }
__device__ __forceinline__ Lane<float> lmul(Lane<float> a, cplx<float> w) {
    Lane<float> r;
    r.re = __ffma2_rn(a.re, bc2(w.x), __fmul2_rn(a.im, bc2(-w.y)));
    r.im = __ffma2_rn(a.re, bc2(w.y), __fmul2_rn(a.im, bc2(w.x)));
    return r;
}
__device__ __forceinline__ Lane<float> lmulc(Lane<float> a, cplx<float> w) {
    Lane<float> r;
    r.re = __ffma2_rn(a.re, bc2(w.x), __fmul2_rn(a.im, bc2(w.y)));
    r.im = __ffma2_rn(a.im, bc2(w.x), __fmul2_rn(a.re, bc2(-w.y)));
    return r;
}
__device__ __forceinline__ Lane<float> lscale(Lane<float> a, float s) { Lane<float> r; r.re = __fmul2_rn(a.re, bc2(s)); r.im = __fmul2_rn(a.im, bc2(s)); return r; }
__device__ __forceinline__ Lane<float> lfma(Lane<float> a, float s, Lane<float> c) { Lane<float> r; r.re = __ffma2_rn(a.re, bc2(s), c.re); r.im = __ffma2_rn(a.im, bc2(s), c.im); return r; }
__device__ __forceinline__ Lane<float> lconj(Lane<float> a) { a.im = neg2(a.im); return a; }
template <bool INV> __device__ __forceinline__ Lane<float> lmi(Lane<float> a) {
    Lane<float> r;
    if (INV) { r.re = neg2(a.im); r.im = a.re; } else { r.re = a.im; r.im = neg2(a.re); }
    return r;
}
__device__ __forceinline__ Lane<float> lmul_real2(Lane<float> a, float s0, float s1) {
    Lane<float> r; const float2 s = make_float2(s0, s1); r.re = __fmul2_rn(a.re, s); r.im = __fmul2_rn(a.im, s); return r;
}
template <bool CONJ> __device__ __forceinline__ Lane<float> lmul_cplx2(Lane<float> a, cplx<float> w0, cplx<float> w1) {
    const float2 wx = make_float2(w0.x, w1.x), wy = make_float2(CONJ ? -w0.y : w0.y, CONJ ? -w1.y : w1.y);
    Lane<float> r;
    r.re = __ffma2_rn(a.re, wx, __fmul2_rn(a.im, neg2(wy)));
    r.im = __ffma2_rn(a.re, wy, __fmul2_rn(a.im, wx));
    return r;
}

__device__ __forceinline__ Lane<double> operator+(Lane<double> a, Lane<double> b) { Lane<double> r; r.re = a.re + b.re; r.im = a.im + b.im; return r; }
__device__ __forceinline__ Lane<double> operator-(Lane<double> a, Lane<double> b) { Lane<double> r; r.re = a.re - b.re; r.im = a.im - b.im; return r; }
__device__ __forceinline__ Lane<double> lmul(Lane<double> a, cplx<double> w) { Lane<double> r; r.re = a.re * w.x - a.im * w.y; r.im = a.re * w.y + a.im * w.x; return r; }
__device__ __forceinline__ Lane<double> lmulc(Lane<double> a, cplx<double> w) { Lane<double> r; r.re = a.re * w.x + a.im * w.y; r.im = a.im * w.x - a.re * w.y; return r; }
__device__ __forceinline__ Lane<double> lscale(Lane<double> a, double s) { Lane<double> r; r.re = a.re * s; r.im = a.im * s; return r; }
__device__ __forceinline__ Lane<double> lfma(Lane<double> a, double s, Lane<double> c) { Lane<double> r; r.re = c.re + s * a.re; r.im = c.im + s * a.im; return r; }
__device__ __forceinline__ Lane<double> lconj(Lane<double> a) { a.im = -a.im; return a; }
template <bool INV> __device__ __forceinline__ Lane<double> lmi(Lane<double> a) {
    Lane<double> r;
    if (INV) { r.re = -a.im; r.im = a.re; } else { r.re = a.im; r.im = -a.re; }
    return r;
}

__device__ __forceinline__ cplx<float> lane_get(const Lane<float>& a, int l) { return l ? mk<float>(a.re.y, a.im.y) : mk<float>(a.re.x, a.im.x); }
__device__ __forceinline__ cplx<double> lane_get(const Lane<double>& a, int) { return mk<double>(a.re, a.im); }
__device__ __forceinline__ void lane_set(Lane<float>& a, int l, cplx<float> v) { if (l) { a.re.y = v.x; a.im.y = v.y; } else { a.re.x = v.x; a.im.x = v.y; } }
__device__ __forceinline__ void lane_set(Lane<double>& a, int, cplx<double> v) { a.re = v.x; a.im = v.y; }

struct __align__(16) Raw16f { float a, b, c, d; };
#ifdef HIPGP_EMU
template <class V> __device__ __forceinline__ V ld_stream(const V* p) { return *p; }
template <class V> __device__ __forceinline__ void st_stream(V* p, V v) { *p = v; }
#else
__device__ __forceinline__ float ld_stream(const float* p) { return __ldcg(p); }
__device__ __forceinline__ double ld_stream(const double* p) { return __ldcg(p); }
__device__ __forceinline__ cplx<float> ld_stream(const cplx<float>* p) { const float2 t = __ldcg(reinterpret_cast<const float2*>(p)); return mk<float>(t.x, t.y); }
__device__ __forceinline__ cplx<double> ld_stream(const cplx<double>* p) { const double2 t = __ldcg(reinterpret_cast<const double2*>(p)); return mk<double>(t.x, t.y); }
__device__ __forceinline__ void st_stream(float* p, float v) { __stcg(p, v); }
__device__ __forceinline__ void st_stream(double* p, double v) { __stcg(p, v); }
__device__ __forceinline__ void st_stream(cplx<float>* p, cplx<float> v) { __stcg(reinterpret_cast<float2*>(p), make_float2(v.x, v.y)); }
__device__ __forceinline__ void st_stream(cplx<double>* p, cplx<double> v) { __stcg(reinterpret_cast<double2*>(p), make_double2(v.x, v.y)); }
#endif
template <class T> struct Vec16;
template <> struct __align__(16) Vec16<float> { float v[4]; };
template <> struct __align__(16) Vec16<double> { double v[2]; };
#ifdef HIPGP_EMU
template <class T> __device__ __forceinline__ Vec16<T> ldv_stream(const T* p) { return *reinterpret_cast<const Vec16<T>*>(p); }
template <class T> __device__ __forceinline__ void stv_stream(T* p, Vec16<T> v) { *reinterpret_cast<Vec16<T>*>(p) = v; }
#else
__device__ __forceinline__ Vec16<float> ldv_stream(const float* p) { const float4 t = __ldcg(reinterpret_cast<const float4*>(p)); Vec16<float> r; r.v[0] = t.x; r.v[1] = t.y; r.v[2] = t.z; r.v[3] = t.w; return r; }
__device__ __forceinline__ Vec16<double> ldv_stream(const double* p) { const double2 t = __ldcg(reinterpret_cast<const double2*>(p)); Vec16<double> r; r.v[0] = t.x; r.v[1] = t.y; return r; }
__device__ __forceinline__ void stv_stream(float* p, Vec16<float> v) { __stcg(reinterpret_cast<float4*>(p), make_float4(v.v[0], v.v[1], v.v[2], v.v[3])); }
__device__ __forceinline__ void stv_stream(double* p, Vec16<double> v) { __stcg(reinterpret_cast<double2*>(p), make_double2(v.v[0], v.v[1])); }
#endif
__device__ __forceinline__ Lane<float> lane_from_global(const cplx<float>* p) {
#ifdef HIPGP_EMU
    return *reinterpret_cast<const Lane<float>*>(p);
#else
    const float4 t = __ldcg(reinterpret_cast<const float4*>(p));
    Lane<float> r; r.re = make_float2(t.x, t.y); r.im = make_float2(t.z, t.w); return r;
#endif
}
__device__ __forceinline__ Lane<double> lane_from_global(const cplx<double>* p) {
#ifdef HIPGP_EMU
    return *reinterpret_cast<const Lane<double>*>(p);
#else
    const double2 t = __ldcg(reinterpret_cast<const double2*>(p));
    Lane<double> r; r.re = t.x; r.im = t.y; return r;
#endif
}
__device__ __forceinline__ void lane_to_global(cplx<float>* p, Lane<float> v) {
#ifdef HIPGP_EMU
    *reinterpret_cast<Lane<float>*>(p) = v;
#else
    __stcg(reinterpret_cast<float4*>(p), make_float4(v.re.x, v.re.y, v.im.x, v.im.y));
#endif
}
__device__ __forceinline__ void lane_to_global(cplx<double>* p, Lane<double> v) {
#ifdef HIPGP_EMU
    *reinterpret_cast<Lane<double>*>(p) = v;
#else
    __stcg(reinterpret_cast<double2*>(p), make_double2(v.re, v.im));
#endif
}

__device__ __forceinline__ float2 pack2(float a, float b) {
#ifdef HIPGP_EMU
    return make_float2(a, b);
#else
    unsigned long long r;
    asm("mov.b64 %0, {%1, %2};" : "=l"(r) : "f"(a), "f"(b));
    float2 o;
    asm("mov.b64 {%0, %1}, %2;" : "=f"(o.x), "=f"(o.y) : "l"(r));
    return o;
#endif
}
__device__ __forceinline__ Lane<float> lane_make(cplx<float> v0, cplx<float> v1) { Lane<float> r; r.re = pack2(v0.x, v1.x); r.im = pack2(v0.y, v1.y); return r; }
__device__ __forceinline__ Lane<double> lane_make(cplx<double> v0, cplx<double>) { Lane<double> r; r.re = v0.x; r.im = v0.y; return r; }

template <class T> struct WRow;
template <> struct WRow<float> {
    static __device__ __forceinline__ void store1(cplx<float>* row, int q, cplx<float> v) {
        float* f = reinterpret_cast<float*>(row) + 4 * (q >> 1) + (q & 1); st_stream(f, v.x); st_stream(f + 2, v.y);
    }
    static __device__ __forceinline__ cplx<float> load1(const cplx<float>* row, int q) {
        const float* f = reinterpret_cast<const float*>(row) + 4 * (q >> 1) + (q & 1); return mk<float>(ld_stream(f), ld_stream(f + 2));
    }
    static __device__ __forceinline__ void store2(cplx<float>* row, int q, cplx<float> v0, cplx<float> v1) {
        Lane<float> t; t.re = make_float2(v0.x, v1.x); t.im = make_float2(v0.y, v1.y);
        lane_to_global(row + q, t);
    }
    static __device__ __forceinline__ void load2(const cplx<float>* row, int q, cplx<float>& v0, cplx<float>& v1) {
        const Lane<float> t = lane_from_global(row + q);
        v0 = mk<float>(t.re.x, t.im.x); v1 = mk<float>(t.re.y, t.im.y);
    }
};
template <> struct WRow<double> {
    static __device__ __forceinline__ void store1(cplx<double>* row, int q, cplx<double> v) { st_stream(row + q, v); }
    static __device__ __forceinline__ cplx<double> load1(const cplx<double>* row, int q) { return ld_stream(row + q); }
    static __device__ __forceinline__ void store2(cplx<double>* row, int q, cplx<double> v0, cplx<double> v1) { st_stream(row + q, v0); st_stream(row + q + 1, v1); }
    static __device__ __forceinline__ void load2(const cplx<double>* row, int q, cplx<double>& v0, cplx<double>& v1) { v0 = ld_stream(row + q); v1 = ld_stream(row + q + 1); }
};

template <int BYTES> __device__ __forceinline__ void cp_async(void* smem_dst, const void* gmem_src) {
#ifdef HIPGP_EMU
    std::memcpy(smem_dst, gmem_src, BYTES);
#else
    const unsigned sa = (unsigned)__cvta_generic_to_shared(smem_dst);
    if (BYTES == 16) asm volatile("cp.async.cg.shared.global [%0], [%1], 16;" ::"r"(sa), "l"(gmem_src));
    else asm volatile("cp.async.ca.shared.global [%0], [%1], 8;" ::"r"(sa), "l"(gmem_src));
#endif
}
__device__ __forceinline__ void cp_async_commit() {
#ifndef HIPGP_EMU
    asm volatile("cp.async.commit_group;" ::: "memory");
#endif
}
__device__ __forceinline__ void cp_async_wait_all() {
#ifndef HIPGP_EMU
    asm volatile("cp.async.wait_group 0;" ::: "memory");
#endif
}

#ifndef HIPGP_EMU
__device__ __forceinline__ void mbar_init(unsigned long long* bar, unsigned count) {
    asm volatile("mbarrier.init.shared::cta.b64 [%0], %1;" ::"r"((unsigned)__cvta_generic_to_shared(bar)), "r"(count) : "memory");
}
__device__ __forceinline__ void fence_proxy_async() { asm volatile("fence.proxy.async.shared::cta;" ::: "memory"); }
__device__ __forceinline__ void mbar_arrive_expect_tx(unsigned long long* bar, unsigned bytes) {
    asm volatile("mbarrier.arrive.expect_tx.shared::cta.b64 _, [%0], %1;" ::"r"((unsigned)__cvta_generic_to_shared(bar)), "r"(bytes) : "memory");
}
__device__ __forceinline__ void mbar_wait(unsigned long long* bar, unsigned parity) {
    const unsigned a = (unsigned)__cvta_generic_to_shared(bar);
    asm volatile(
        "{\n\t.reg .pred P1;\n\t"
        "HIPGP_MBAR_WAIT:\n\t"
        "mbarrier.try_wait.parity.shared::cta.b64 P1, [%0], %1, 0x989680;\n\t"
        "@P1 bra HIPGP_MBAR_DONE;\n\t"
        "bra HIPGP_MBAR_WAIT;\n\t"
        "HIPGP_MBAR_DONE:\n\t}" ::"r"(a), "r"(parity) : "memory");
}
__device__ __forceinline__ void bulk_g2s(void* smem_dst, const void* gmem_src, unsigned bytes, unsigned long long* bar) {
    asm volatile("cp.async.bulk.shared::cluster.global.mbarrier::complete_tx::bytes [%0], [%1], %2, [%3];"
                 ::"r"((unsigned)__cvta_generic_to_shared(smem_dst)), "l"(gmem_src), "r"(bytes), "r"((unsigned)__cvta_generic_to_shared(bar)) : "memory");
}
__device__ __forceinline__ void bulk_s2g(void* gmem_dst, const void* smem_src, unsigned bytes) {
    asm volatile("cp.async.bulk.global.shared::cta.bulk_group [%0], [%1], %2;" ::"l"(gmem_dst), "r"((unsigned)__cvta_generic_to_shared(smem_src)), "r"(bytes) : "memory");
    asm volatile("cp.async.bulk.commit_group;" ::: "memory");
    asm volatile("cp.async.bulk.wait_group.read 0;" ::: "memory");
}
__device__ __forceinline__ void bulk_s2g_issue(void* gmem_dst, const void* smem_src, unsigned bytes) {
    asm volatile("cp.async.bulk.global.shared::cta.bulk_group [%0], [%1], %2;" ::"l"(gmem_dst), "r"((unsigned)__cvta_generic_to_shared(smem_src)), "r"(bytes) : "memory");
    asm volatile("cp.async.bulk.commit_group;" ::: "memory");
}
__device__ __forceinline__ void bulk_s2g_wait() { asm volatile("cp.async.bulk.wait_group.read 0;" ::: "memory"); }
#endif

template <bool INV, class E> __device__ __forceinline__ void lb2(E* v) { const E a = v[0], b = v[1]; v[0] = a + b; v[1] = a - b; }
template <bool INV, class E> __device__ __forceinline__ void lb4(E* v) {
    const E a = v[0] + v[2], b = v[0] - v[2], c = v[1] + v[3], d = lmi<INV>(v[1] - v[3]);
    v[0] = a + c; v[1] = b + d; v[2] = a - c; v[3] = b - d;
}
template <bool INV, class T, class E> __device__ __forceinline__ void lb8(E* v) {
    const T h = (T)0.70710678118654752440;
    E e[4] = {v[0] + v[4], v[1] + v[5], v[2] + v[6], v[3] + v[7]};
    E o[4] = {v[0] - v[4], v[1] - v[5], v[2] - v[6], v[3] - v[7]};
    o[1] = lmul(o[1], mk<T>(h, INV ? h : -h));
    o[2] = lmi<INV>(o[2]);
    o[3] = lmul(o[3], mk<T>(-h, INV ? h : -h));
    lb4<INV>(e); lb4<INV>(o);
    v[0] = e[0]; v[2] = e[1]; v[4] = e[2]; v[6] = e[3];
    v[1] = o[0]; v[3] = o[1]; v[5] = o[2]; v[7] = o[3];
}
template <bool INV, class T, class E> __device__ __forceinline__ void lb16_tail(E (&t)[4][4], E* v) {
    const T c1 = (T)0.92387953251128675613, s1 = (T)0.38268343236508977173, h = (T)0.70710678118654752440;
    const cplx<T> w1 = mk<T>(c1, INV ? s1 : -s1), w2 = mk<T>(h, INV ? h : -h), w3 = mk<T>(s1, INV ? c1 : -c1);
    const cplx<T> w6 = mk<T>(-h, INV ? h : -h), w9 = mk<T>(-c1, INV ? -s1 : s1);
    t[1][1] = lmul(t[1][1], w1); t[1][2] = lmul(t[1][2], w2); t[1][3] = lmul(t[1][3], w3);
    t[2][1] = lmul(t[2][1], w2); t[2][2] = lmi<INV>(t[2][2]); t[2][3] = lmul(t[2][3], w6);
    t[3][1] = lmul(t[3][1], w3); t[3][2] = lmul(t[3][2], w6); t[3][3] = lmul(t[3][3], w9);
#pragma unroll
    for (int c = 0; c < 4; ++c) {
        E u[4] = {t[0][c], t[1][c], t[2][c], t[3][c]};
        lb4<INV>(u);
#pragma unroll
        for (int d = 0; d < 4; ++d) v[c + 4 * d] = u[d];
    }
}
template <bool INV, class T, class E> __device__ __forceinline__ void lb16(E* v) {
    E t[4][4];
#pragma unroll
    for (int b = 0; b < 4; ++b) {
        E u[4] = {v[b], v[b + 4], v[b + 8], v[b + 12]};
        lb4<INV>(u);
#pragma unroll
        for (int c = 0; c < 4; ++c) t[b][c] = u[c];
    }
    lb16_tail<INV, T>(t, v);
}
template <bool INV, class T, class E> __device__ __forceinline__ void lb3(E* v) {
    const T s = (T)0.86602540378443864676;
    const E t = v[1] + v[2];
    const E m = lfma(t, (T)-0.5, v[0]);
    const E j = lmi<INV>(lscale(v[1] - v[2], s));
    v[0] = v[0] + t; v[1] = m + j; v[2] = m - j;
}
template <bool INV, class T, class E> __device__ __forceinline__ void lb5(E* v) {
    const T c1 = (T)0.30901699437494742410, c2 = (T)-0.80901699437494742410;
    const T s1 = (T)0.95105651629515357212, s2 = (T)0.58778525229247312917;
    const E a1 = v[1] + v[4], a2 = v[2] + v[3], b1 = v[1] - v[4], b2 = v[2] - v[3];
    const E m1 = lfma(a2, c2, lfma(a1, c1, v[0]));
    const E m2 = lfma(a2, c1, lfma(a1, c2, v[0]));
    const E j1 = lmi<INV>(lfma(b2, s2, lscale(b1, s1)));
    const E j2 = lmi<INV>(lfma(b2, -s1, lscale(b1, s2)));
    v[0] = v[0] + a1 + a2;
    v[1] = m1 + j1; v[4] = m1 - j1; v[2] = m2 + j2; v[3] = m2 - j2;
}
template <int R, bool INV, class T, class E> __device__ __forceinline__ void lbfly(E* v) {
    if (R == 2) lb2<INV>(v);
    else if (R == 3) lb3<INV, T>(v);
    else if (R == 4) lb4<INV>(v);
    else if (R == 5) lb5<INV, T>(v);
    else if (R == 8) lb8<INV, T>(v);
    else lb16<INV, T>(v);
}
template <int R, class T, class E> __device__ __forceinline__ void lbfly_zero_hi(E* v) {
    if (R == 2) { v[1] = v[0]; }
    else if (R == 4) {
        const E a = v[0], c = v[1], d = lmi<false>(v[1]);
        v[0] = a + c; v[1] = a + d; v[2] = a - c; v[3] = a - d;
    } else if (R == 8) {
        const T h = (T)0.70710678118654752440;
        E e[4] = {v[0], v[1], v[2], v[3]};
        E o[4] = {v[0], lmul(v[1], mk<T>(h, -h)), lmi<false>(v[2]), lmul(v[3], mk<T>(-h, -h))};
        lb4<false>(e); lb4<false>(o);
        v[0] = e[0]; v[2] = e[1]; v[4] = e[2]; v[6] = e[3];
        v[1] = o[0]; v[3] = o[1]; v[5] = o[2]; v[7] = o[3];
    } else {
        E t[4][4];
#pragma unroll
        for (int b = 0; b < 4; ++b) {
            const E a = v[b], c = v[b + 4], d = lmi<false>(c);
            t[b][0] = a + c; t[b][1] = a + d; t[b][2] = a - c; t[b][3] = a - d;
        }
        lb16_tail<false, T>(t, v);
    }
}

template <int... Rs> struct RL {};
template <class L> struct RLInfo;
template <> struct RLInfo<RL<>> { static constexpr int N = 1; static constexpr int count = 0; };
template <int R0, int... Rs> struct RLInfo<RL<R0, Rs...>> {
    static constexpr int N = R0 * RLInfo<RL<Rs...>>::N;
    static constexpr int count = 1 + RLInfo<RL<Rs...>>::count;
};
template <class L> struct RLLast;
template <int R0> struct RLLast<RL<R0>> { static constexpr int value = R0; };
template <int R0, int R1, int... Rs> struct RLLast<RL<R0, R1, Rs...>> { static constexpr int value = RLLast<RL<R1, Rs...>>::value; };
template <class L> struct RLFirst;
template <int R0, int... Rs> struct RLFirst<RL<R0, Rs...>> { static constexpr int value = R0; };
template <class L> struct RLMax;
template <int R0> struct RLMax<RL<R0>> { static constexpr int value = R0; };
template <int R0, int R1, int... Rs> struct RLMax<RL<R0, R1, Rs...>> {
    static constexpr int rest = RLMax<RL<R1, Rs...>>::value;
    static constexpr int value = R0 > rest ? R0 : rest;
};
__host__ __device__ constexpr bool is_pow2(int x) { return x > 0 && (x & (x - 1)) == 0; }
__host__ __device__ constexpr int ilog2(int x) { return x <= 1 ? 0 : 1 + ilog2(x >> 1); }

template <class T, int NL, int... Rs>
struct TileGeo {
    using List = RL<Rs...>;
    static constexpr int Ln = RLInfo<List>::N;
    static constexpr int NST = RLInfo<List>::count;
    static constexpr int RLAST = RLLast<List>::value;
    static constexpr int LOGRL = ilog2(RLAST);
    static constexpr bool PAD = (NL < 8) && (NST > 1) && is_pow2(RLAST);
    __host__ __device__ static constexpr int slot(int p) { return PAD ? p + (p >> LOGRL) : p; }
    static constexpr int SLOTS = PAD ? Ln + Ln / RLAST : Ln;
    __host__ __device__ static constexpr size_t smem_bytes(int extra_slots = 0) { return sizeof(Lane<T>) * (size_t)(SLOTS + extra_slots) * NL; }
    __host__ __device__ static constexpr int leg(int S) { return (S == 1 ? 1 : (PAD ? S + (S >> LOGRL) : S)) * NL; }
};

template <int R, int S, class T>
__device__ __forceinline__ void lane_twiddles(cplx<T>* w, const cplx<T>* __restrict__ tab, int j) {
    if (TwLayout<T>::paired) {
#pragma unroll
        for (int p = 0; p < TwPairs<R>::n; ++p) {
            const TwPair<T> e = tw_pair_global<R, S, T>(tab, p, j);
            w[2 * p + 1] = e.a;
            if (2 * p + 2 < R) w[2 * p + 2] = e.b;
        }
    } else {
#pragma unroll
        for (int r = 1; r < R; ++r) w[r] = ldg_c(tab + (r - 1) * S + j);
    }
}

template <class G, class T, int NL, int Nt, int R, bool INV>
__device__ __forceinline__ void lane_stage_item(Lane<T>* s, const cplx<T>* __restrict__ tab, int it) {
    constexpr int S = Nt / R, LEG = G::leg(S);
    const int lane = it % NL, bf = it / NL;
    const int blk = bf / S, j = bf - blk * S;
    Lane<T>* base = s + (G::slot(blk * Nt + j) * NL + lane);
    cplx<T> w[R];
    if (S > 1) lane_twiddles<R, S>(w, tab, j);
    Lane<T> v[R];
#pragma unroll
    for (int r = 0; r < R; ++r) v[r] = base[r * LEG];
    if (INV) {
        if (S > 1) {
#pragma unroll
            for (int r = 1; r < R; ++r) v[r] = lmulc(v[r], w[r]);
        }
        lbfly<R, true, T>(v);
    } else {
        lbfly<R, false, T>(v);
        if (S > 1) {
#pragma unroll
            for (int r = 1; r < R; ++r) v[r] = lmul(v[r], w[r]);
        }
    }
#pragma unroll
    for (int r = 0; r < R; ++r) base[r * LEG] = v[r];
}
template <class G, class T, int NL, int NT, int Nt, int R, bool INV>
__device__ __forceinline__ void lane_stage(Lane<T>* s, const cplx<T>* __restrict__ tab, int tid) {
    constexpr int ITEMS = (G::Ln / R) * NL, NIT = (ITEMS + NT - 1) / NT;
    if constexpr (ITEMS % NT == 0 && NIT * R <= 16) {
#pragma unroll
        for (int k = 0; k < NIT; ++k) lane_stage_item<G, T, NL, Nt, R, INV>(s, tab, tid + k * NT);
    } else {
#pragma unroll 1
        for (int it = tid; it < ITEMS; it += NT) lane_stage_item<G, T, NL, Nt, R, INV>(s, tab, it);
    }
}

template <class G, class T, int NL, int NT, int Nt, int STG, int... Rs> struct LaneMidFwd;
template <class G, class T, int NL, int NT, int Nt, int STG, int R0> struct LaneMidFwd<G, T, NL, NT, Nt, STG, R0> {
    static __device__ __forceinline__ void run(Lane<T>*, const LineFft<T>&, int) {}
};
template <class G, class T, int NL, int NT, int Nt, int STG, int R0, int R1, int... Rs> struct LaneMidFwd<G, T, NL, NT, Nt, STG, R0, R1, Rs...> {
    static __device__ __forceinline__ void run(Lane<T>* s, const LineFft<T>& f, int tid) {
        lane_stage<G, T, NL, NT, Nt, R0, false>(s, f.twst + f.twoff[STG], tid);
        __syncthreads();
        LaneMidFwd<G, T, NL, NT, Nt / R0, STG + 1, R1, Rs...>::run(s, f, tid);
    }
};
template <class G, class T, int NL, int NT, int Nt, int STG, int... Rs> struct LaneMidInv;
template <class G, class T, int NL, int NT, int Nt, int STG, int R0> struct LaneMidInv<G, T, NL, NT, Nt, STG, R0> {
    static __device__ __forceinline__ void run(Lane<T>*, const LineFft<T>&, int) {}
};
template <class G, class T, int NL, int NT, int Nt, int STG, int R0, int R1, int... Rs> struct LaneMidInv<G, T, NL, NT, Nt, STG, R0, R1, Rs...> {
    static __device__ __forceinline__ void run(Lane<T>* s, const LineFft<T>& f, int tid) {
        LaneMidInv<G, T, NL, NT, Nt / R0, STG + 1, R1, Rs...>::run(s, f, tid);
        lane_stage<G, T, NL, NT, Nt, R0, true>(s, f.twst + f.twoff[STG], tid);
        __syncthreads();
    }
};

}
```

### hipgp_b200/csrc/plan.cu

```cuda
#include "plan_types.cuh"
#include "setup_kernels.cuh"
#include "kxu_kernels.cuh"

namespace hipgp {
thread_local std::string g_err;
bool g_no_fast = false;
}

namespace hipgp {

template <class T> struct Tag {};
static Geom<float>& geom(hipgp_plan* p, bool wide, Tag<float>) { return wide ? p->gw32 : p->gn32; }
static Geom<double>& geom(hipgp_plan* p, bool wide, Tag<double>) { return wide ? p->gw64 : p->gn64; }

template <class T> static size_t rows_smem(int H, int RBP) { return sizeof(cplx<T>) * (size_t)(H + 1) * RBP; }

template <class T>
static void pick_rows_tiling(long total_rows, int H, int* RB, int* RBP, int* nthreads) {
    int rb = 8;
    while (rb > 1 && (rows_smem<T>(H, rb + 1) > 96 * 1024 || total_rows < (long)rb * 148)) rb >>= 1;
    if (rows_smem<T>(H, rb + 1) > 200 * 1024) throw Error("row axis too long for the shared-memory FFT (L = " + std::to_string(2 * H) + ")");
    *RB = rb; *RBP = rb == 1 ? 1 : rb + 1;
    long work = (long)H * rb / 8;
    *nthreads = work >= 256 ? 256 : (work >= 128 ? 128 : (work >= 64 ? 64 : 32));
}

template <class T> static bool aligned2(const void* p) { return ((uintptr_t)p % (2 * sizeof(T))) == 0; }

template <class T>
static bool launch_rows_fast(hipgp_plan* pl, bool inverse, RowsParams<T>& P, cudaStream_t st) {
    if (g_no_fast) return false;
    switch (P.H) {
#define X(LEN, ...) case LEN: launch_rows_fast_len<T, LEN>(pl, inverse, P, st); return true;
        HIPGP_FAST_LIST(X)
#undef X
        default: return false;
    }
}

template <class T>
static bool geom_allows_fast(const Geom<T>& g) {
    if (sizeof(T) == 8) return true;
    if (g_no_fast || fast_radices(g.H).empty()) return false;
    for (int d = 0; d + 1 < g.D; ++d) if (fast_radices(g.L[d]).empty()) return false;
    return true;
}

template <class T>
static void launch_rows(hipgp_plan* pl, bool inverse, RowsParams<T>& P, cudaStream_t st, bool allow_fast = true) {
    P.vec_ok = (aligned2<T>(P.in) && aligned2<T>(P.out) && aligned2<T>(P.v0) && aligned2<T>(P.v1) && aligned2<T>(P.v2)) ? 1 : 0;
    {
        auto a16 = [](const void* q) { return ((uintptr_t)q % 16) == 0; };
        P.vec16_ok = (a16(P.in) && a16(P.out) && a16(P.v0) && a16(P.v1) && a16(P.v2)) ? 1 : 0;
    }
    if (allow_fast && P.do_fft && launch_rows_fast<T>(pl, inverse, P, st)) return;
    int nth;
    pick_rows_tiling<T>(P.total_rows, P.H, &P.RB, &P.RBP, &nth);
    const size_t smem = rows_smem<T>(P.H, P.RBP);
    dim3 grid((unsigned)((P.total_rows + P.RB - 1) / P.RB));
    PROF_BEGIN(pl, inverse ? 2 : 0, st);
    if (inverse) {
        auto k = rows_inv_kernel<T>;
        if (smem > 48 * 1024) HIPGP_SET_MAX_SMEM(k, smem);
        HIPGP_LAUNCH(k, grid, dim3(nth), smem, st, P);
    } else {
        auto k = rows_fwd_kernel<T>;
        if (smem > 48 * 1024) HIPGP_SET_MAX_SMEM(k, smem);
        HIPGP_LAUNCH(k, grid, dim3(nth), smem, st, P);
    }
    PROF_END(pl, st);
    CK_LAUNCH();
    pl->launches++;
}

template <class T>
static bool launch_cols_fast(hipgp_plan* pl, ColsParams<T>& P, long n_outer, long B, cudaStream_t st) {
    if (g_no_fast) return false;
    switch (P.f.Ln) {
#define X(LEN, ...) case LEN: return launch_cols_fast_len<T, LEN>(pl, P, n_outer, B, st);
        HIPGP_FAST_LIST(X)
#undef X
        default: return false;
    }
}

template <class T>
static void launch_cols(hipgp_plan* pl, ColsParams<T>& P, long n_outer, long B, cudaStream_t st, bool allow_fast = true) {
    if (allow_fast && launch_cols_fast<T>(pl, P, n_outer, B, st)) return;
    const int L = P.f.Ln;
    int tb = sizeof(T) == 4 ? 16 : 8;
    while (tb > 1 && sizeof(cplx<T>) * (size_t)L * (tb + 1) > 100 * 1024) tb >>= 1;
    while (tb > 1 && (long)tb > P.inner) tb >>= 1;
    const int tbp = tb == 1 ? 1 : tb + 1;
    const size_t smem = sizeof(cplx<T>) * (size_t)L * tbp;
    if (smem > 220 * 1024) throw Error("grid axis too long for the shared-memory FFT (L = " + std::to_string(L) + ")");
    P.TB = tb; P.TBP = tbp;
    long work = (long)L * tb / 8;
    int nth = work >= 512 ? 512 : (work >= 256 ? 256 : (work >= 128 ? 128 : (work >= 64 ? 64 : 32)));
    dim3 grid((unsigned)((P.inner + tb - 1) / tb), (unsigned)n_outer, (unsigned)B);
    auto k = cols_pass_kernel<T>;
    if (smem > 48 * 1024) HIPGP_SET_MAX_SMEM(k, smem);
    PROF_BEGIN(pl, 1, st);
    HIPGP_LAUNCH(k, grid, dim3(nth), smem, st, P);
    PROF_END(pl, st);
    CK_LAUNCH();
    pl->launches++;
}

template <class T>
static void rows_geom(RowsParams<T>& R, Geom<T>& g) {
    R.L = g.L[g.D - 1]; R.H = g.H; R.W_pitch = g.P;
    R.f = g.frow.dev; R.twL = g.twL.template as<cplx<T>>(); R.twLp = g.twLp.template as<cplx<T>>();
    R.part = g.part.template as<int>(); R.pairq = g.pairq.template as<int>();
    R.pairs = g.pairs.template as<int>(); R.pairw = g.pairw.template as<cplx<T>>(); R.npair0 = g.npair0;
    R.quadq = g.quadq.template as<int>(); R.quadw = g.quadw.template as<cplx<T>>(); R.nquad = g.nquad;
}

static void ws_elems(int D, const int* L, long P, const int* n_in, const int* n_out, long B, long* w1, long* w2) {
    if (D == 1) { *w1 = B * P; *w2 = 0; return; }
    if (D == 2) { *w1 = B * std::max(n_in[0], n_out[0]) * P; *w2 = 0; return; }
    const long R01 = std::max((long)n_in[0] * n_in[1], (long)n_out[0] * n_out[1]);
    const long R0 = std::max(n_in[0], n_out[0]);
    *w1 = B * R01 * P; *w2 = B * R0 * (long)L[1] * P;
}

template <class T>
static void run_pipeline_group(hipgp_plan* pl, Geom<T>& g, const int* n_in, const int* n_out, const void* spec, int spec_kind,
                         long B, const RowsFusion& ff, const RowsFusion& fi, const PcgDev& st, bool gated, cudaStream_t s) {
    const int D = g.D;
    long w1, w2;
    ws_elems(D, g.L, g.P, n_in, n_out, B, &w1, &w2);
    pl->W1.ensure(sizeof(cplx<T>) * (size_t)w1, &pl->dev_bytes);
    if (w2) pl->W2.ensure(sizeof(cplx<T>) * (size_t)w2, &pl->dev_bytes);
    cplx<T>* W1 = pl->W1.as<cplx<T>>();
    cplx<T>* W2 = pl->W2.as<cplx<T>>();
    const long P = g.P;
    const int* done = gated ? st.flags : nullptr;
    const bool fast = geom_allows_fast(g);

    long rows_in = 1, rows_out = 1;
    for (int d = 0; d + 1 < D; ++d) { rows_in *= n_in[d]; rows_out *= n_out[d]; }
    const long Wrows = std::max(rows_in, rows_out);

    RowsParams<T> R{};
    rows_geom(R, g);
    R.W = W1; R.W_rows = (int)Wrows; R.st = st;
    R.in = (const T*)ff.in; R.v0 = (T*)ff.v0; R.v1 = (T*)ff.v1; R.v2 = (const T*)ff.v2;
    R.mode = ff.mode; R.do_fft = 1; R.total_rows = B * rows_in; R.nrows = (int)rows_in; R.n_real = n_in[D - 1];
    R.spec = nullptr; R.spec_kind = SPEC_NONE;
    launch_rows<T>(pl, false, R, s, fast);

    if (D == 2) {
        ColsParams<T> C{};
        C.in = W1; C.out = W1; C.n_in = n_in[0]; C.n_out = n_out[0]; C.inner = g.H + 1; C.pitch = P;
        C.in_ostride = C.out_ostride = 0; C.in_bstride = C.out_bstride = Wrows * P;
        C.f = g.fcol[0].dev; C.mode = CM_FUSED; C.spec = spec; C.spec_kind = spec_kind; C.done_flag = done;
        launch_cols<T>(pl, C, 1, B, s, fast);
    } else if (D == 3) {
        const long R0 = std::max(n_in[0], n_out[0]);
        const long L1 = g.L[1];
        ColsParams<T> C{};
        C.done_flag = done; C.spec = nullptr; C.spec_kind = SPEC_NONE;
        C.in = W1; C.out = W2; C.n_in = n_in[1]; C.n_out = n_in[1]; C.inner = g.H + 1; C.pitch = P;
        C.in_ostride = (long)n_in[1] * P; C.in_bstride = Wrows * P; C.out_ostride = L1 * P; C.out_bstride = R0 * L1 * P;
        C.f = g.fcol[1].dev; C.mode = CM_FWD;
        launch_cols<T>(pl, C, n_in[0], B, s, fast);
        C.in = W2; C.out = W2; C.n_in = n_in[0]; C.n_out = n_out[0]; C.inner = L1 * P; C.pitch = L1 * P;
        C.in_ostride = C.out_ostride = 0; C.in_bstride = C.out_bstride = R0 * L1 * P;
        C.f = g.fcol[0].dev; C.mode = CM_FUSED; C.spec = spec; C.spec_kind = spec_kind;
        launch_cols<T>(pl, C, 1, B, s, fast);
        C.in = W2; C.out = W1; C.n_in = n_out[1]; C.n_out = n_out[1]; C.inner = g.H + 1; C.pitch = P;
        C.in_ostride = L1 * P; C.in_bstride = R0 * L1 * P; C.out_ostride = (long)n_out[1] * P; C.out_bstride = Wrows * P;
        C.f = g.fcol[1].dev; C.mode = CM_INV; C.spec = nullptr; C.spec_kind = SPEC_NONE;
        launch_cols<T>(pl, C, n_out[0], B, s, fast);
    }

    R.out = (T*)fi.out; R.v0 = (T*)fi.v0; R.mode = fi.mode; R.dot_kind = fi.dot_kind;
    R.total_rows = B * rows_out; R.nrows = (int)rows_out; R.n_real = n_out[D - 1];
    if (D == 1) { R.spec = spec; R.spec_kind = spec_kind; }
    launch_rows<T>(pl, true, R, s, fast);
}


template <class T>
static long pass_group(hipgp_plan* pl, Geom<T>& g, const int* n_in, const int* n_out, long B) {
    static const char* env = getenv("HIPGP_L2_GROUP_MB");
    const double budget_mb = env ? atof(env) : 0.0;
    if (budget_mb <= 0 || B <= 1) return B;
    long w1, w2;
    ws_elems(g.D, g.L, g.P, n_in, n_out, 1, &w1, &w2);
    long vin = 1, vout = 1;
    for (int d = 0; d < g.D; ++d) { vin *= n_in[d]; vout *= n_out[d]; }
    const double per_rhs = (double)sizeof(cplx<T>) * (double)(w1 + w2) + (double)sizeof(T) * (double)(vin + vout);
    long grp = (long)(budget_mb * 1048576.0 / per_rhs);
    (void)pl;
    return std::max<long>(1, std::min<long>(B, grp));
}

template <class T>
static void run_pipeline(hipgp_plan* pl, Geom<T>& g, const int* n_in, const int* n_out, const void* spec, int spec_kind,
                         long B, const RowsFusion& ff, const RowsFusion& fi, const PcgDev& st, bool gated, cudaStream_t s) {
    const long grp = pass_group<T>(pl, g, n_in, n_out, B);
    if (grp >= B) { run_pipeline_group<T>(pl, g, n_in, n_out, spec, spec_kind, B, ff, fi, st, gated, s); return; }
    long vin = 1, vout = 1, rows_in = 1, rows_out = 1;
    for (int d = 0; d < g.D; ++d) { vin *= n_in[d]; vout *= n_out[d]; }
    for (int d = 0; d + 1 < g.D; ++d) { rows_in *= n_in[d]; rows_out *= n_out[d]; }
    auto shift = [](const void* p, long elems) -> const void* { return p ? (const void*)((const T*)p + elems) : nullptr; };
    for (long b0 = 0; b0 < B; b0 += grp) {
        const long nb = std::min(grp, B - b0);
        RowsFusion f2 = ff, i2 = fi;
        f2.in = shift(ff.in, b0 * vin); f2.v0 = (void*)shift(ff.v0, b0 * vin); f2.v1 = (void*)shift(ff.v1, b0 * vin); f2.v2 = shift(ff.v2, b0 * vin);
        i2.out = (void*)shift(fi.out, b0 * vout); i2.v0 = (void*)shift(fi.v0, b0 * vout);
        PcgDev s2 = st;
        if (st.zr) {
            s2.zr = st.zr + b0; s2.zr_prev = st.zr_prev + b0; s2.pAp = st.pAp + b0; s2.rr = st.rr + b0;
            s2.rr_all = st.rr_all ? st.rr_all : st.rr;
            s2.row_cnt = st.row_cnt + b0;
            s2.partial = st.partial + b0 * std::max(rows_in, rows_out);
        }
        run_pipeline_group<T>(pl, g, n_in, n_out, spec, spec_kind, nb, f2, i2, s2, gated, s);
    }
}

static void forward_full(hipgp_plan* pl, Geom<double>& g, const double* h, cudaStream_t s) {
    const int D = g.D;
    long rows = 1;
    for (int d = 0; d + 1 < D; ++d) rows *= g.L[d];
    pl->W1.ensure(sizeof(cplx<double>) * (size_t)rows * g.P, &pl->dev_bytes);
    cplx<double>* W = pl->W1.as<cplx<double>>();
    RowsParams<double> R{};
    rows_geom(R, g);
    R.in = h; R.W = W; R.W_rows = (int)rows; R.mode = RF_PLAIN; R.do_fft = 1;
    R.total_rows = rows; R.nrows = (int)rows; R.n_real = g.L[D - 1];
    launch_rows<double>(pl, false, R, s);
    if (D >= 2) {
        ColsParams<double> C{};
        C.in = W; C.out = W; C.mode = CM_FWD; C.done_flag = nullptr; C.spec_kind = SPEC_NONE;
        if (D == 3) {
            C.n_in = C.n_out = g.L[1]; C.inner = g.H + 1; C.pitch = g.P;
            C.in_ostride = C.out_ostride = (long)g.L[1] * g.P; C.in_bstride = C.out_bstride = 0;
            C.f = g.fcol[1].dev;
            launch_cols<double>(pl, C, g.L[0], 1, s);
            C.n_in = C.n_out = g.L[0]; C.inner = (long)g.L[1] * g.P; C.pitch = (long)g.L[1] * g.P;
            C.in_ostride = C.out_ostride = 0; C.f = g.fcol[0].dev;
            launch_cols<double>(pl, C, 1, 1, s);
        } else {
            C.n_in = C.n_out = g.L[0]; C.inner = g.H + 1; C.pitch = g.P;
            C.in_ostride = C.out_ostride = 0; C.in_bstride = C.out_bstride = 0; C.f = g.fcol[0].dev;
            launch_cols<double>(pl, C, 1, 1, s);
        }
    }
}

static const double* axis_costab(hipgp_plan* pl, int d) {
    DevBuf& b = pl->costabs[d];
    if (!b.p) {
        const int md = pl->m[d];
        const int Nn = md > 1 ? 2 * (md - 1) : 1;
        std::vector<double> tab(Nn);
        for (int t = 0; t < Nn; ++t) tab[t] = md > 1 ? std::cos(M_PI * (double)t / (double)(md - 1)) : 1.0;
        b.ensure(sizeof(double) * Nn, &pl->dev_bytes);
        CK(cudaMemcpy(b.p, tab.data(), sizeof(double) * Nn, cudaMemcpyHostToDevice));
    }
    return b.as<double>();
}

static const double* axis_cosmat(hipgp_plan* pl, int d, cudaStream_t s) {
    const int md = pl->m[d];
    if (md > 2048) return nullptr;
    DevBuf& b = pl->cosmats[d];
    if (!b.p) {
        const double* tab = axis_costab(pl, d);
        const size_t h = (size_t)(md + 1) / 2;
        b.ensure(sizeof(double) * 2 * h * h, &pl->dev_bytes);
        auto k = dct1_cosmat_sym_kernel;
        HIPGP_LAUNCH(k, dim3((unsigned)std::min<size_t>(148 * 4, (2 * h * h + 255) / 256)), dim3(256), 0, s, tab, b.as<double>(), md);
        CK_LAUNCH(); pl->launches++;
    }
    return b.as<double>();
}

static void dct_all_axes(hipgp_plan* pl, const double* in, double* out, double* tmp, bool normalise, cudaStream_t s) {
    const double* src = in;
    const int D = pl->D;
    double* bufs[2] = {out, tmp};
    int which = (D % 2 == 1) ? 0 : 1;
    static const char* env_old = getenv("HIPGP_DCT_DENSE");
    for (int d = 0; d < D; ++d) {
        const int md = pl->m[d];
        long inner = 1, outer = 1;
        for (int e = d + 1; e < D; ++e) inner *= pl->m[e];
        for (int e = 0; e < d; ++e) outer *= pl->m[e];
        const double* tab = axis_costab(pl, d);
        const int Nn = md > 1 ? 2 * (md - 1) : 1;
        double* dst = bufs[which];
        const double scale = normalise ? 1.0 / (double)Nn : 1.0;
        if (env_old) {
            int bx = 64;
            while (bx > 1 && bx / 2 >= inner) bx >>= 1;
            dim3 block(bx, 256 / bx);
            const int nx = (int)((inner + bx - 1) / bx);
            dim3 grid((unsigned)((long)nx * outer), (unsigned)((md + block.y - 1) / block.y), 1);
            auto k = dct1_axis_kernel;
            HIPGP_LAUNCH(k, grid, block, 0, s, src, dst, tab, md, inner, scale, nx);
        } else if (inner == 1) {
            dim3 grid((unsigned)((md + 63) / 64), (unsigned)((outer + 127) / 128), 1);
            const double* cw = md > 2 ? axis_cosmat(pl, d, s) : nullptr;
            if (cw) {
                const int hk0 = (md + 1) / 2;
                dim3 gs((unsigned)((hk0 + 63) / 64), (unsigned)((outer + 127) / 128), 2);
                auto k = dct1_sym_kernel<true>; HIPGP_LAUNCH(k, gs, dim3(256), 0, s, src, dst, cw, md, inner, outer, scale, 0);
            } else { auto k = dct1_tile_kernel<true>; HIPGP_LAUNCH(k, grid, dim3(256), 0, s, src, dst, tab, md, inner, outer, scale); }
        } else {
            if (outer > 65535) throw Error("DCT set-up: more than 65535 outer slices");
            dim3 grid((unsigned)((inner + 63) / 64), (unsigned)((md + 127) / 128), (unsigned)outer);
            const double* cw = md > 2 ? axis_cosmat(pl, d, s) : nullptr;
            if (cw) {
                const int hk0 = (md + 1) / 2, nty = (hk0 + 127) / 128;
                dim3 gs((unsigned)((inner + 63) / 64), (unsigned)(2 * nty), (unsigned)outer);
                auto k = dct1_sym_kernel<false>; HIPGP_LAUNCH(k, gs, dim3(256), 0, s, src, dst, cw, md, inner, outer, scale, nty);
            } else { auto k = dct1_tile_kernel<false>; HIPGP_LAUNCH(k, grid, dim3(256), 0, s, src, dst, tab, md, inner, outer, scale); }
        }
        CK_LAUNCH();
        pl->launches++;
        src = dst; which ^= 1;
    }
}

template <class T>
static void build_spectrum(hipgp_plan* pl, bool wide, const double* col, DevBuf& dst, bool complex_spec, cudaStream_t s) {
    Geom<double>& g = wide ? pl->gw64 : pl->gn64;
    EmbedDims e{};
    e.D = g.D;
    long total = 1;
    for (int d = 0; d < 3; ++d) { e.m[d] = 1; e.N[d] = 1; e.L[d] = 1; e.wide[d] = 0; }
    for (int d = 0; d < g.D; ++d) {
        const int slot = 3 - g.D + d;
        e.m[slot] = pl->m[d]; e.N[slot] = pl->N[d]; e.L[slot] = g.L[d]; e.wide[slot] = wide ? (pl->wide_real ? 2 : 1) : 0;
        total *= g.L[d];
    }
    pl->tmpB.ensure(sizeof(double) * (size_t)total, &pl->dev_bytes);
    {
        auto k = embed_kernel;
        const int nb = (int)std::min<long>((total + 255) / 256, 148 * 8);
        HIPGP_LAUNCH(k, dim3(nb), dim3(256), 0, s, col, pl->tmpB.as<double>(), e);
        CK_LAUNCH(); pl->launches++;
    }
    forward_full(pl, g, pl->tmpB.as<double>(), s);
    const long n = g.spec_elems();
    double scale = 0.25;
    for (int d = 0; d < g.D; ++d) scale /= (double)g.L[d];
    const unsigned nblk = (unsigned)((n + 255) / 256);
    if (complex_spec) {
        dst.ensure(sizeof(cplx<T>) * (size_t)n, &pl->dev_bytes);
        auto k = store_spec_cplx_kernel<T>; HIPGP_LAUNCH(k, dim3(nblk), dim3(256), 0, s, pl->W1.as<cplx<double>>(), dst.as<cplx<T>>(), n, scale);
    } else {
        dst.ensure(sizeof(T) * (size_t)n, &pl->dev_bytes);
        auto k = store_spec_real_kernel<T>; HIPGP_LAUNCH(k, dim3(nblk), dim3(256), 0, s, pl->W1.as<cplx<double>>(), dst.as<T>(), n, scale);
    }
    CK_LAUNCH(); pl->launches++;
}

template <class T>
static void ensure_geoms(hipgp_plan* pl, bool wide) {
    Geom<double>& g64 = wide ? pl->gw64 : pl->gn64;
    const int* L = wide ? pl->Lw : pl->Ln;
    if (!g64.built) g64.build(pl->D, L, &pl->dev_bytes);
    if (sizeof(T) == 4) {
        Geom<float>& g32 = wide ? pl->gw32 : pl->gn32;
        if (!g32.built) g32.build(pl->D, L, &pl->dev_bytes);
    }
}

template <class T>
static void set_first_row(hipgp_plan* pl, const void* column, double clampv, cudaStream_t s) {
    const long M = pl->M;
    pl->clampv = clampv;
    ensure_geoms<T>(pl, false);
    for (DevBuf* b : {&pl->Dm, &pl->Dinv, &pl->Dsqrt, &pl->colK, &pl->colG, &pl->colS, &pl->tmpA})
        b->ensure(sizeof(double) * (size_t)M, &pl->dev_bytes);
    pl->tmpB.ensure(sizeof(double) * (size_t)M, &pl->dev_bytes);
    pl->counts.ensure(sizeof(unsigned) * 4, &pl->dev_bytes);
    CK(cudaMemsetAsync(pl->counts.p, 0, sizeof(unsigned) * 4, s));
    const unsigned nb = (unsigned)((M + 255) / 256);
    {
        auto k = to_double_kernel<T>;
        HIPGP_LAUNCH(k, dim3(nb), dim3(256), 0, s, (const T*)column, pl->colK.as<double>(), M);
        CK_LAUNCH(); pl->launches++;
    }
    dct_all_axes(pl, pl->colK.as<double>(), pl->tmpA.as<double>(), pl->tmpB.as<double>(), false, s);
    {
        auto k = clamp_derive_kernel<T>;
        HIPGP_LAUNCH(k, dim3(nb), dim3(256), 0, s, pl->tmpA.as<double>(), pl->Dm.as<double>(), pl->Dinv.as<double>(),
                     pl->Dsqrt.as<double>(), M, clampv, pl->counts.as<unsigned>());
        CK_LAUNCH(); pl->launches++;
    }
    unsigned hc[4] = {0, 0, 0, 0};
    CK(cudaMemcpyAsync(hc, pl->counts.p, sizeof(hc), cudaMemcpyDeviceToHost, s));
    CK(cudaStreamSynchronize(s));
    pl->nclamped = hc[0];
    if (pl->nclamped != 0 || sizeof(T) == 4)
        dct_all_axes(pl, pl->Dm.as<double>(), pl->colK.as<double>(), pl->tmpB.as<double>(), true, s);
    dct_all_axes(pl, pl->Dinv.as<double>(), pl->colG.as<double>(), pl->tmpB.as<double>(), true, s);
    build_spectrum<T>(pl, false, pl->colK.as<double>(), pl->specK, false, s);
    build_spectrum<T>(pl, false, pl->colG.as<double>(), pl->specCinv, false, s);
    pl->have_spec = true; pl->have_wide = false; pl->have_slabK = pl->have_slabCinv = false;
}

template <class T>
static void ensure_wide(hipgp_plan* pl, cudaStream_t s) {
    if (pl->have_wide) return;
    ensure_geoms<T>(pl, true);
    static const char* env_c = getenv("HIPGP_WIDE_COMPLEX");
    bool real_ok = !env_c;
    for (int d = 0; d < pl->D; ++d) if (pl->Lw[d] < 2 * pl->N[d] - 1) real_ok = false;
    pl->wide_real = real_ok;
    dct_all_axes(pl, pl->Dsqrt.as<double>(), pl->colS.as<double>(), pl->tmpB.as<double>(), true, s);
    build_spectrum<T>(pl, true, pl->colS.as<double>(), pl->specW, !real_ok, s);
    pl->have_wide = true;
}

static PcgDev null_state() { PcgDev st{}; return st; }

template <class T>
static void matvec(hipgp_plan* pl, int mode, const void* in, void* out, long B, cudaStream_t s) {
    if (!pl->have_spec) throw Error("plan has no spectrum: call hipgp_plan_set_first_row first");
    if (B < 0) throw Error("negative number of right-hand sides");
    if (B == 0) return;
    if (!in || !out) throw Error("null vector pointer");
    RowsFusion ff, fi;
    ff.mode = RF_PLAIN; ff.in = in; fi.mode = RI_PLAIN; fi.out = out;
    const bool wide = (mode == HIPGP_MV_RT || mode == HIPGP_MV_R);
    if (wide) ensure_wide<T>(pl, s);
    Geom<T>& g = geom(pl, wide, Tag<T>());
    int n_in[3], n_out[3];
    for (int d = 0; d < pl->D; ++d) {
        n_in[d] = mode == HIPGP_MV_R ? pl->N[d] : pl->m[d];
        n_out[d] = mode == HIPGP_MV_RT ? pl->N[d] : pl->m[d];
    }
    const void* spec; int kind;
    switch (mode) {
        case HIPGP_MV_K: spec = pl->specK.p; kind = SPEC_REAL; break;
        case HIPGP_MV_CINV: spec = pl->specCinv.p; kind = SPEC_REAL; break;
        case HIPGP_MV_RT: spec = pl->specW.p; kind = pl->wide_real ? SPEC_REAL : SPEC_CPLX; break;
        case HIPGP_MV_R: spec = pl->specW.p; kind = pl->wide_real ? SPEC_REAL : SPEC_CPLX_CONJ; break;
        default: throw Error("unknown matvec mode");
    }
    run_pipeline<T>(pl, g, n_in, n_out, spec, kind, B, ff, fi, null_state(), false, s);
}

template <class T>
static PcgDev pcg_state(hipgp_plan* pl, long B, double tol, bool cg_mode) {
    const long M = pl->M;
    long nrows = 1;
    for (int d = 0; d + 1 < pl->D; ++d) nrows *= pl->m[d];
    for (DevBuf* b : {&pl->vr, &pl->vp, &pl->vz, &pl->vAp}) b->ensure(sizeof(T) * (size_t)(B * M), &pl->dev_bytes);
    pl->partial.ensure(sizeof(double) * (size_t)(B * nrows), &pl->dev_bytes);
    pl->scal.ensure(sizeof(double) * (size_t)(4 * B), &pl->dev_bytes);
    const bool fresh = pl->cnt.bytes < sizeof(unsigned) * (size_t)(B + 1);
    pl->cnt.ensure(sizeof(unsigned) * (size_t)(B + 1), &pl->dev_bytes);
    pl->flags.ensure(sizeof(int) * 4, &pl->dev_bytes);
    if (fresh) CK(cudaMemset(pl->cnt.p, 0, pl->cnt.bytes));
    PcgDev st{};
    double* sc = pl->scal.as<double>();
    st.zr = sc; st.zr_prev = sc + B; st.pAp = sc + 2 * B; st.rr = sc + 3 * B;
    st.partial = pl->partial.as<double>();
    st.row_cnt = pl->cnt.as<unsigned>(); st.rhs_cnt = pl->cnt.as<unsigned>() + B;
    st.flags = pl->flags.as<int>();
    st.tol = tol; st.B = (int)B; st.cg_mode = cg_mode ? 1 : 0;
    return st;
}

template <class T>
static void launch_vec(hipgp_plan* pl, int mode, const PcgDev& st, long B, const void* in, void* v0, void* v1, const void* v2,
                       cudaStream_t s) {
    long nrows = 1;
    for (int d = 0; d + 1 < pl->D; ++d) nrows *= pl->m[d];
    RowsParams<T> R{};
    R.in = (const T*)in; R.v0 = (T*)v0; R.v1 = (T*)v1; R.v2 = (const T*)v2;
    R.mode = mode; R.do_fft = 0; R.total_rows = B * nrows; R.nrows = (int)nrows; R.n_real = pl->m[pl->D - 1];
    R.H = (R.n_real + 1) / 2; R.L = 2 * R.H; R.st = st;
    R.RB = 8; R.RBP = 9;
    dim3 grid((unsigned)((R.total_rows + R.RB - 1) / R.RB));
    auto k = rows_fwd_kernel<T>;
    PROF_BEGIN(pl, 3, s);
    HIPGP_LAUNCH(k, grid, dim3(256), 0, s, R);
    PROF_END(pl, s);
    CK_LAUNCH(); pl->launches++;
}

template <class T>
static void pcg_begin(hipgp_plan* pl, const void* b, void* x, long B, double tol, bool precond, cudaStream_t s) {
    if (!pl->have_spec) throw Error("plan has no spectrum: call hipgp_plan_set_first_row first");
    if (B <= 0) throw Error("pcg needs at least one right-hand side");
    if (!b || !x) throw Error("null vector pointer");
    const long M = pl->M;
    PcgDev st = pcg_state<T>(pl, B, tol, !precond);
    if (!pl->pinned) CK(cudaMallocHost(&pl->pinned, 64));
    Geom<T>& g = geom(pl, false, Tag<T>());
    int nn[3];
    for (int d = 0; d < pl->D; ++d) nn[d] = pl->m[d];
    T* r = pl->vr.as<T>(); T* z = precond ? pl->vz.as<T>() : r;
    CK(cudaMemsetAsync(x, 0, sizeof(T) * (size_t)(B * M), s));
    CK(cudaMemcpyAsync(r, b, sizeof(T) * (size_t)(B * M), cudaMemcpyDeviceToDevice, s));
    CK(cudaMemsetAsync(st.flags, 0, sizeof(int) * 4, s));
    CK(cudaMemsetAsync(reinterpret_cast<char*>(st.flags) + 2 * sizeof(int), 1, 1, s));
    RowsFusion ff, fi;
    if (precond) {
        ff.mode = RF_PLAIN; ff.in = r; fi.mode = RI_DOT; fi.dot_kind = DOT_ZR; fi.out = z; fi.v0 = r;
        run_pipeline<T>(pl, g, nn, nn, pl->specCinv.p, SPEC_REAL, B, ff, fi, st, false, s);
    } else {
        launch_vec<T>(pl, RF_SELFDOT, st, B, r, nullptr, nullptr, nullptr, s);
    }
    pl->run_x = x; pl->run_B = B; pl->run_precond = precond; pl->run_tol = tol; pl->run_active = true;
}

template <class T>
static void pcg_iterate(hipgp_plan* pl, int niter, cudaStream_t s) {
    if (!pl->run_active) throw Error("hipgp_pcg_step without hipgp_pcg_begin");
    const long B = pl->run_B;
    const bool precond = pl->run_precond;
    PcgDev st = pcg_state<T>(pl, B, pl->run_tol, !precond);
    Geom<T>& g = geom(pl, false, Tag<T>());
    int nn[3];
    for (int d = 0; d < pl->D; ++d) nn[d] = pl->m[d];
    T* r = pl->vr.as<T>(); T* p = pl->vp.as<T>(); T* z = precond ? pl->vz.as<T>() : r; T* Ap = pl->vAp.as<T>();
    void* x = pl->run_x;
    RowsFusion ff, fi;
    for (int c = 0; c < niter; ++c) {
        ff = RowsFusion(); fi = RowsFusion();
        ff.mode = RF_PUPDATE; ff.in = z; ff.v0 = p;
        fi.mode = RI_DOT; fi.dot_kind = DOT_PAP; fi.out = Ap; fi.v0 = p;
        run_pipeline<T>(pl, g, nn, nn, pl->specK.p, SPEC_REAL, B, ff, fi, st, true, s);
        if (precond) {
            ff = RowsFusion(); fi = RowsFusion();
            ff.mode = RF_XRUPDATE; ff.in = Ap; ff.v0 = r; ff.v1 = x; ff.v2 = p;
            fi.mode = RI_DOT; fi.dot_kind = DOT_ZR; fi.out = z; fi.v0 = r;
            run_pipeline<T>(pl, g, nn, nn, pl->specCinv.p, SPEC_REAL, B, ff, fi, st, true, s);
        } else {
            launch_vec<T>(pl, RF_XRUPDATE, st, B, Ap, r, x, p, s);
        }
    }
}

static void pcg_poll(hipgp_plan* pl, int* done, int* iters, double* max_resid, double* resid_out, cudaStream_t s) {
    int* hflags = reinterpret_cast<int*>(pl->pinned);
    CK(cudaMemcpyAsync(hflags, pl->flags.p, sizeof(int) * 4, cudaMemcpyDeviceToHost, s));
    std::vector<double> rr;
    if (max_resid || resid_out) {
        rr.resize(pl->run_B);
        CK(cudaMemcpyAsync(rr.data(), pl->scal.as<double>() + 3 * pl->run_B, sizeof(double) * pl->run_B, cudaMemcpyDeviceToHost, s));
    }
    CK(cudaStreamSynchronize(s));
    if (done) *done = hflags[0];
    if (iters) *iters = hflags[1];
    if (max_resid) {
        double mx = 0.0; bool nan = false;
        for (double v : rr) { const double q = std::sqrt(v); if (q != q) nan = true; else if (q > mx) mx = q; }
        *max_resid = nan ? NAN : mx;
    }
    if (resid_out) for (long i = 0; i < pl->run_B; ++i) resid_out[i] = std::sqrt(rr[i]);
}

template <class T>
static void pcg(hipgp_plan* pl, const void* b, void* x, long B, int maxiter, double tol, bool precond, int* iters_out,
                int* callbacks_out, double* resid_out, hipgp_iter_cb cb, void* user, cudaStream_t s) {
    if (iters_out) *iters_out = 0;
    if (callbacks_out) *callbacks_out = 0;
    if (B < 0) throw Error("negative number of right-hand sides");
    if (B == 0) return;
    pcg_begin<T>(pl, b, x, B, tol, precond, s);
    const int check_every = cb ? 1 : 8;
    int done = 0, iters = 0, n = 0;
    while (n < maxiter && !done) {
        const int chunk = std::min(check_every, maxiter - n);
        pcg_iterate<T>(pl, chunk, s);
        pcg_poll(pl, &done, &iters, nullptr, nullptr, s);
        n += chunk;
        if (cb && !done) cb(n - 1, x, user);
    }
    if (iters_out) *iters_out = iters;
    if (callbacks_out) *callbacks_out = done ? iters - 1 : iters;
    if (resid_out) pcg_poll(pl, nullptr, nullptr, nullptr, resid_out, s);
    pl->run_active = false;
}

}

#define API_BEGIN try {
#define API_END                                                                          \
    } catch (const std::exception& e) { hipgp::g_err = e.what(); return -1; }            \
      catch (...) { hipgp::g_err = "unknown error"; return -2; }                         \
    return 0;

#define DISPATCH(pl, call_f32, call_f64) do { if ((pl)->dtype == HIPGP_F32) { call_f32; } else { call_f64; } } while (0)

static void need_plan(const hipgp_plan* pl) { if (!pl) throw Error("null plan handle"); }
static void set_device(const hipgp_plan* pl) { need_plan(pl); CK(cudaSetDevice(pl->device)); }

static void slab_peer_close(hipgp_plan* pl) {
#ifndef HIPGP_EMU
    for (int i = 0; i < pl->n_ipc_opened; ++i) if (pl->ipc_opened[i]) cudaIpcCloseMemHandle(pl->ipc_opened[i]);
#endif
    pl->n_ipc_opened = 0; pl->peers_ready = false;
}

extern "C" {

const char* hipgp_last_error(void) { return hipgp::g_err.c_str(); }
int hipgp_version(void) { return 100; }

int hipgp_plan_create(int ndim, const int64_t* m, int dtype, int device, hipgp_plan** out) {
    API_BEGIN
    if (!out || !m || ndim < 1) throw Error("bad arguments");
    if (dtype != HIPGP_F32 && dtype != HIPGP_F64) throw Error("dtype must be HIPGP_F32 or HIPGP_F64");
    hipgp_plan* pl = new hipgp_plan();
    pl->dtype = dtype; pl->device = device; pl->ndim_user = ndim;
    int D = 0;
    for (int d = 0; d < ndim; ++d) {
        if (m[d] < 1) { delete pl; throw Error("grid extents must be >= 1"); }
        pl->m_user.push_back((long)m[d]);
        pl->M *= m[d];
        if (m[d] > 1) {
            if (D == 3) { delete pl; throw Error("at most 3 grid axes of extent > 1 are supported"); }
            pl->m[D] = (int)m[d]; pl->N[D] = 2 * (int)m[d] - 2; pl->E *= pl->N[D]; ++D;
        }
    }
    if (D == 0) { D = 1; pl->m[0] = 1; pl->N[0] = 1; }
    pl->D = D;
    const char* nf = getenv("HIPGP_NO_FAST");
    g_no_fast = nf && nf[0] == '1';
    const char* env = getenv("HIPGP_POW2_ONLY");
    const bool pow2 = env && env[0] == '1';
    for (int d = 0; d < D; ++d) {
        const bool row = (d == D - 1);
        pl->Ln[d] = choose_length(2L * pl->m[d] - 1, row, pow2);
        pl->Lw[d] = choose_length((long)pl->N[d] + pl->m[d] - 1, row, pow2);
    }
    *out = pl;
    API_END
}

int hipgp_plan_destroy(hipgp_plan* pl) {
    API_BEGIN
    if (!pl) return 0;
    size_t* t = &pl->dev_bytes;
    pl->gn32.release(t); pl->gw32.release(t); pl->gn64.release(t); pl->gw64.release(t);
    for (DevBuf* b : {&pl->specK, &pl->specCinv, &pl->specW, &pl->Dm, &pl->Dinv, &pl->Dsqrt, &pl->colK, &pl->colG, &pl->colS,
                      &pl->tmpA, &pl->tmpB, &pl->costab, &pl->counts, &pl->W1, &pl->W2, &pl->vr, &pl->vp, &pl->vz, &pl->vAp,
                      &pl->partial, &pl->scal, &pl->cnt, &pl->flags, &pl->stage_in, &pl->stage_out, &pl->corrU, &pl->corrV, &pl->corrS,
                      &pl->corrLag, &pl->gradA, &pl->slabSpecK, &pl->slabSpecCinv, &pl->slabR1, &pl->slabR2, &pl->slot_in[0], &pl->slot_in[1], &pl->slot_out[0], &pl->slot_out[1], &pl->costabs[0], &pl->costabs[1], &pl->costabs[2], &pl->cosmats[0], &pl->cosmats[1], &pl->cosmats[2]})
        b->release(t);
    slab_peer_close(pl);
#ifndef HIPGP_EMU
    for (auto& se : pl->slot_ev) for (auto& e : se) if (e) cudaEventDestroy(e);
    if (pl->slot_flags) cudaFreeHost(pl->slot_flags);
#else
    delete[] pl->slot_flags;
#endif
    if (pl->pinned) cudaFreeHost(pl->pinned);
#ifndef HIPGP_EMU
    for (auto& cs : pl->copy_streams) if (cs) cudaStreamDestroy(cs);
#endif
    delete pl;
    API_END
}

int hipgp_plan_sizes(const hipgp_plan* pl, int64_t* M, int64_t* Mprime) {
    API_BEGIN
    need_plan(pl);
    if (M) *M = pl->M;
    if (Mprime) *Mprime = pl->E;
    API_END
}

int hipgp_plan_embedding(const hipgp_plan* pl, int64_t* Ln, int64_t* Lw) {
    API_BEGIN
    need_plan(pl);
    int a = 0;
    for (int d = 0; d < pl->ndim_user; ++d) {
        const bool active = pl->m_user[d] > 1 || (pl->D == 1 && pl->M == 1 && d == 0);
        if (Ln) Ln[d] = active ? pl->Ln[a] : 1;
        if (Lw) Lw[d] = active ? pl->Lw[a] : 1;
        if (active) ++a;
    }
    API_END
}

int hipgp_plan_set_first_row(hipgp_plan* pl, const void* column, double clampv, int64_t* clamped_out, void* stream) {
    API_BEGIN
    set_device(pl);
    DISPATCH(pl, set_first_row<float>(pl, column, clampv, (cudaStream_t)stream), set_first_row<double>(pl, column, clampv, (cudaStream_t)stream));
    if (clamped_out) *clamped_out = pl->nclamped;
    API_END
}

int hipgp_plan_spectrum(hipgp_plan* pl, int which, void* out, void* stream) {
    API_BEGIN
    set_device(pl);
    if (!pl->have_spec) throw Error("plan has no spectrum");
    if (which < 0 || which > 3) throw Error("bad spectrum selector");
    EmbedDims e{};
    for (int d = 0; d < 3; ++d) { e.m[d] = 1; e.N[d] = 1; e.L[d] = 1; e.wide[d] = 0; }
    for (int d = 0; d < pl->D; ++d) { const int slot = 3 - pl->D + d; e.m[slot] = pl->m[d]; e.N[slot] = pl->N[d]; }
    const int nb = (int)std::min<long>((pl->E + 255) / 256, 148 * 8);
    cudaStream_t s = (cudaStream_t)stream;
    if (pl->dtype == HIPGP_F32) { auto k = expand_even_kernel<float>; HIPGP_LAUNCH(k, dim3(nb), dim3(256), 0, s, pl->Dm.as<double>(), (float*)out, e, which); }
    else { auto k = expand_even_kernel<double>; HIPGP_LAUNCH(k, dim3(nb), dim3(256), 0, s, pl->Dm.as<double>(), (double*)out, e, which); }
    CK_LAUNCH(); pl->launches++;
    API_END
}

int hipgp_matvec(hipgp_plan* pl, int mode, const void* in, void* out, int64_t B, void* stream) {
    API_BEGIN
    set_device(pl);
    DISPATCH(pl, matvec<float>(pl, mode, in, out, (long)B, (cudaStream_t)stream), matvec<double>(pl, mode, in, out, (long)B, (cudaStream_t)stream));
    API_END
}

static size_t elem_size(const hipgp_plan* pl) { return pl->dtype == HIPGP_F32 ? 4 : 8; }

int hipgp_matvec_host(hipgp_plan* pl, int mode, const void* in_host, void* out_host, int64_t B, void* stream) {
    API_BEGIN
    set_device(pl);
    cudaStream_t s = (cudaStream_t)stream;
    const size_t nin = (size_t)B * (mode == HIPGP_MV_R ? pl->E : pl->M) * elem_size(pl);
    const size_t nout = (size_t)B * (mode == HIPGP_MV_RT ? pl->E : pl->M) * elem_size(pl);
    pl->stage_in.ensure(nin, &pl->dev_bytes); pl->stage_out.ensure(nout, &pl->dev_bytes);
    CK(cudaMemcpyAsync(pl->stage_in.p, in_host, nin, cudaMemcpyHostToDevice, s));
    DISPATCH(pl, matvec<float>(pl, mode, pl->stage_in.p, pl->stage_out.p, (long)B, s), matvec<double>(pl, mode, pl->stage_in.p, pl->stage_out.p, (long)B, s));
    CK(cudaMemcpyAsync(out_host, pl->stage_out.p, nout, cudaMemcpyDeviceToHost, s));
    CK(cudaStreamSynchronize(s));
    API_END
}

int hipgp_pcg(hipgp_plan* pl, const void* b, void* x, int64_t B, int maxiter, double tol, int precond, int* iters_out,
              int* callbacks_out, double* resid_out, hipgp_iter_cb cb, void* user, void* stream) {
    API_BEGIN
    set_device(pl);
    cudaStream_t s = (cudaStream_t)stream;
    DISPATCH(pl, pcg<float>(pl, b, x, (long)B, maxiter, tol, precond != 0, iters_out, callbacks_out, resid_out, cb, user, s),
             pcg<double>(pl, b, x, (long)B, maxiter, tol, precond != 0, iters_out, callbacks_out, resid_out, cb, user, s));
    API_END
}

int hipgp_pcg_begin(hipgp_plan* pl, const void* b, void* x, int64_t B, double tol, int precond, void* stream) {
    API_BEGIN
    set_device(pl);
    cudaStream_t s = (cudaStream_t)stream;
    DISPATCH(pl, pcg_begin<float>(pl, b, x, (long)B, tol, precond != 0, s), pcg_begin<double>(pl, b, x, (long)B, tol, precond != 0, s));
    API_END
}

int hipgp_pcg_step(hipgp_plan* pl, int niter, int* done_out, int* iters_out, double* max_resid_out, void* stream) {
    API_BEGIN
    set_device(pl);
    cudaStream_t s = (cudaStream_t)stream;
    DISPATCH(pl, pcg_iterate<float>(pl, niter, s), pcg_iterate<double>(pl, niter, s));
    if (done_out || iters_out || max_resid_out) pcg_poll(pl, done_out, iters_out, max_resid_out, nullptr, s);
    API_END
}

int hipgp_pcg_host(hipgp_plan* pl, const void* b_host, void* x_host, int64_t B, int maxiter, double tol, int precond,
                   int* iters_out, int* callbacks_out, double* resid_out, void* stream) {
    API_BEGIN
    set_device(pl);
    cudaStream_t s = (cudaStream_t)stream;
    const size_t n = (size_t)B * pl->M * elem_size(pl);
    pl->stage_in.ensure(n, &pl->dev_bytes); pl->stage_out.ensure(n, &pl->dev_bytes);
    CK(cudaMemcpyAsync(pl->stage_in.p, b_host, n, cudaMemcpyHostToDevice, s));
    DISPATCH(pl, pcg<float>(pl, pl->stage_in.p, pl->stage_out.p, (long)B, maxiter, tol, precond != 0, iters_out, callbacks_out, resid_out, nullptr, nullptr, s),
             pcg<double>(pl, pl->stage_in.p, pl->stage_out.p, (long)B, maxiter, tol, precond != 0, iters_out, callbacks_out, resid_out, nullptr, nullptr, s));
    CK(cudaMemcpyAsync(x_host, pl->stage_out.p, n, cudaMemcpyDeviceToHost, s));
    CK(cudaStreamSynchronize(s));
    API_END
}

int hipgp_pcg_host_pipelined(hipgp_plan* pl, const void* b_host, void* x_host, int64_t B, int maxiter, double tol, int precond,
                             int64_t group, int* iters_out, void* stream) {
    API_BEGIN
    set_device(pl);
    if (iters_out) *iters_out = 0;
    if (B < 0) throw Error("negative number of right-hand sides");
    if (B == 0) return 0;
    if (!b_host || !x_host) throw Error("null vector pointer");
    if (group <= 0 || group > B) group = B;
    cudaStream_t s = (cudaStream_t)stream;
#ifndef HIPGP_EMU
    if (!pl->copy_streams[0]) {
        CK(cudaStreamCreateWithFlags(&pl->copy_streams[0], cudaStreamNonBlocking));
        CK(cudaStreamCreateWithFlags(&pl->copy_streams[1], cudaStreamNonBlocking));
    }
#endif
    const size_t row = (size_t)pl->M * elem_size(pl);
    pl->stage_in.ensure((size_t)B * row, &pl->dev_bytes); pl->stage_out.ensure((size_t)B * row, &pl->dev_bytes);
    std::vector<long> gs;
    if (B >= 4 * group) { gs.push_back(group); gs.push_back(B - 2 * group); gs.push_back(group); }
    else for (long b0 = 0; b0 < B; b0 += group) gs.push_back(std::min<long>(group, B - b0));
    const long ng = (long)gs.size();
    std::vector<long> gb0(ng);
    { long acc = 0; for (long g = 0; g < ng; ++g) { gb0[g] = acc; acc += gs[g]; } }
    std::vector<cudaEvent_t> in_ready(ng), solved(ng);
#ifndef HIPGP_EMU
    for (long g = 0; g < ng; ++g) { CK(cudaEventCreateWithFlags(&in_ready[g], cudaEventDisableTiming)); CK(cudaEventCreateWithFlags(&solved[g], cudaEventDisableTiming)); }
    cudaStream_t cin = pl->copy_streams[0], cout = pl->copy_streams[1];
    cudaEvent_t start; CK(cudaEventCreateWithFlags(&start, cudaEventDisableTiming));
    CK(cudaEventRecord(start, s)); CK(cudaStreamWaitEvent(cin, start, 0)); CK(cudaStreamWaitEvent(cout, start, 0));
#else
    cudaStream_t cin = s, cout = s;
#endif
    for (long g = 0; g < ng; ++g) {
        const long b0 = gb0[g], nb = gs[g];
        CK(cudaMemcpyAsync((char*)pl->stage_in.p + b0 * row, (const char*)b_host + b0 * row, nb * row, cudaMemcpyHostToDevice, cin));
#ifndef HIPGP_EMU
        CK(cudaEventRecord(in_ready[g], cin));
#endif
    }
    int iters_max = 0;
    for (long g = 0; g < ng; ++g) {
        const long b0 = gb0[g], nb = gs[g];
#ifndef HIPGP_EMU
        CK(cudaStreamWaitEvent(s, in_ready[g], 0));
#endif
        int it = 0;
        void* bg = (char*)pl->stage_in.p + b0 * row; void* xg = (char*)pl->stage_out.p + b0 * row;
        DISPATCH(pl, pcg<float>(pl, bg, xg, nb, maxiter, tol, precond != 0, &it, nullptr, nullptr, nullptr, nullptr, s),
                 pcg<double>(pl, bg, xg, nb, maxiter, tol, precond != 0, &it, nullptr, nullptr, nullptr, nullptr, s));
        iters_max = std::max(iters_max, it);
#ifndef HIPGP_EMU
        CK(cudaEventRecord(solved[g], s));
        CK(cudaStreamWaitEvent(cout, solved[g], 0));
#endif
        CK(cudaMemcpyAsync((char*)x_host + b0 * row, xg, nb * row, cudaMemcpyDeviceToHost, cout));
    }
#ifndef HIPGP_EMU
    CK(cudaStreamSynchronize(cout));
    CK(cudaStreamSynchronize(s));
    for (long g = 0; g < ng; ++g) { cudaEventDestroy(in_ready[g]); cudaEventDestroy(solved[g]); }
    cudaEventDestroy(start);
#endif
    if (iters_out) *iters_out = iters_max;
    API_END
}

int hipgp_pcg_host_submit(hipgp_plan* pl, const void* b_host, void* x_host, int64_t B, int maxiter, double tol, int precond, int slot,
                          void* stream) {
    API_BEGIN
    set_device(pl);
    if (slot < 0 || slot > 1) throw Error("slot must be 0 or 1");
    if (B <= 0) throw Error("hipgp_pcg_host_submit needs at least one right-hand side");
    if (!b_host || !x_host) throw Error("null vector pointer");
    if (maxiter < 0) throw Error("negative maxiter");
    cudaStream_t s = (cudaStream_t)stream;
#ifndef HIPGP_EMU
    if (!pl->copy_streams[0]) {
        CK(cudaStreamCreateWithFlags(&pl->copy_streams[0], cudaStreamNonBlocking));
        CK(cudaStreamCreateWithFlags(&pl->copy_streams[1], cudaStreamNonBlocking));
    }
    for (int e = 0; e < 3; ++e) if (!pl->slot_ev[slot][e]) CK(cudaEventCreateWithFlags(&pl->slot_ev[slot][e], cudaEventDisableTiming));
    if (!pl->slot_flags) CK(cudaMallocHost((void**)&pl->slot_flags, sizeof(int) * 8));
    if (pl->slot_busy[slot]) { CK(cudaEventSynchronize(pl->slot_ev[slot][2])); pl->slot_busy[slot] = false; }
    cudaStream_t cin = pl->copy_streams[0], cout = pl->copy_streams[1];
#else
    if (!pl->slot_flags) pl->slot_flags = new int[8];
    cudaStream_t cin = s, cout = s;
#endif
    const size_t n = (size_t)B * pl->M * elem_size(pl);
    pl->slot_in[slot].ensure(n, &pl->dev_bytes); pl->slot_out[slot].ensure(n, &pl->dev_bytes);
    CK(cudaMemcpyAsync(pl->slot_in[slot].p, b_host, n, cudaMemcpyHostToDevice, cin));
#ifndef HIPGP_EMU
    CK(cudaEventRecord(pl->slot_ev[slot][0], cin));
    CK(cudaStreamWaitEvent(s, pl->slot_ev[slot][0], 0));
#endif
    if (pl->dtype == HIPGP_F32) { pcg_begin<float>(pl, pl->slot_in[slot].p, pl->slot_out[slot].p, (long)B, tol, precond != 0, s); pcg_iterate<float>(pl, maxiter, s); }
    else { pcg_begin<double>(pl, pl->slot_in[slot].p, pl->slot_out[slot].p, (long)B, tol, precond != 0, s); pcg_iterate<double>(pl, maxiter, s); }
    pl->run_active = false;
    CK(cudaMemcpyAsync(pl->slot_flags + 4 * slot, pl->flags.p, sizeof(int) * 4, cudaMemcpyDeviceToHost, s));
#ifndef HIPGP_EMU
    CK(cudaEventRecord(pl->slot_ev[slot][1], s));
    CK(cudaStreamWaitEvent(cout, pl->slot_ev[slot][1], 0));
#endif
    CK(cudaMemcpyAsync(x_host, pl->slot_out[slot].p, n, cudaMemcpyDeviceToHost, cout));
#ifndef HIPGP_EMU
    CK(cudaEventRecord(pl->slot_ev[slot][2], cout));
#endif
    pl->slot_busy[slot] = true;
    API_END
}
int hipgp_pcg_host_wait(hipgp_plan* pl, int slot, int* iters_out) {
    API_BEGIN
    set_device(pl);
    if (slot < 0 || slot > 1) throw Error("slot must be 0 or 1");
    if (!pl->slot_busy[slot]) throw Error("hipgp_pcg_host_wait: nothing was submitted on this slot");
#ifndef HIPGP_EMU
    CK(cudaEventSynchronize(pl->slot_ev[slot][2]));
#endif
    pl->slot_busy[slot] = false;
    if (iters_out) *iters_out = pl->slot_flags[4 * slot + 1];
    API_END
}

int hipgp_compute_kn(hipgp_plan* pl, const void* Knm, void* kn, int64_t B, int maxiter, double tol, int* iters_out, void* stream) {
    API_BEGIN
    set_device(pl);
    cudaStream_t s = (cudaStream_t)stream;
    const size_t n = (size_t)B * pl->M * elem_size(pl);
    pl->stage_out.ensure(n, &pl->dev_bytes);
    void* d0 = pl->stage_out.p;
    DISPATCH(pl, pcg<float>(pl, Knm, d0, (long)B, maxiter, tol, true, iters_out, nullptr, nullptr, nullptr, nullptr, s),
             pcg<double>(pl, Knm, d0, (long)B, maxiter, tol, true, iters_out, nullptr, nullptr, nullptr, nullptr, s));
    DISPATCH(pl, matvec<float>(pl, HIPGP_MV_RT, d0, kn, (long)B, s), matvec<double>(pl, HIPGP_MV_RT, d0, kn, (long)B, s));
    API_END
}

int hipgp_plan_profile(hipgp_plan* pl, int enable) {
    API_BEGIN
    need_plan(pl);
    pl->profiling = enable != 0;
    API_END
}
int hipgp_plan_profile_read(hipgp_plan* pl, int kernel_class, double* ms_total, int64_t* launches, int reset) {
    API_BEGIN
    need_plan(pl);
    if (kernel_class < 0 || kernel_class > 3) throw Error("kernel_class must be 0..3");
#ifndef HIPGP_EMU
    set_device(pl);
    CK(cudaDeviceSynchronize());
    for (auto& r : pl->prof) {
        float ms = 0;
        CK(cudaEventElapsedTime(&ms, r.e0, r.e1));
        pl->prof_ms[r.cls] += ms; pl->prof_n[r.cls] += 1;
        cudaEventDestroy(r.e0); cudaEventDestroy(r.e1);
    }
    pl->prof.clear();
#endif
    if (ms_total) *ms_total = pl->prof_ms[kernel_class];
    if (launches) *launches = pl->prof_n[kernel_class];
    if (reset) for (int i = 0; i < 4; ++i) { pl->prof_ms[i] = 0; pl->prof_n[i] = 0; }
    API_END
}
int hipgp_plan_device_bytes(const hipgp_plan* pl, size_t* bytes) { API_BEGIN need_plan(pl); if (bytes) *bytes = pl->dev_bytes; API_END }
int hipgp_plan_launch_count(const hipgp_plan* pl, int64_t* launches) { API_BEGIN need_plan(pl); if (launches) *launches = pl->launches; API_END }

}

#include "vec_api.inl"
#include "kxu_api.inl"
#include "corr_api.inl"
#include "block_api.inl"
#include "slab_api.inl"

#ifdef HIPGP_EMU
namespace emu {
thread_local dim3 t_threadIdx, t_blockIdx;
dim3 g_blockDim, g_gridDim;
Barrier g_block_barrier;
Barrier g_warp_barrier[64];
NamedBarrier g_named_barrier[16];
unsigned char* g_dyn_smem = nullptr;
double g_shfl_scratch[64][32][2];
}
#endif
```

### hipgp_b200/csrc/plan_types.cuh

```cuda
#pragma once
#include "../../include/hipgp_b200.h"
#include "conv_kernels.cuh"

#include <string>
#include <stdexcept>

namespace hipgp {

extern thread_local std::string g_err;
struct Error : std::runtime_error { using std::runtime_error::runtime_error; };

#define CK(expr)                                                                                     \
    do {                                                                                             \
        cudaError_t e__ = (expr);                                                                    \
        if (e__ != cudaSuccess)                                                                      \
            throw Error(std::string(#expr) + ": " + cudaGetErrorString(e__));                        \
    } while (0)
#define CK_LAUNCH() CK(cudaGetLastError())

struct DevBuf {
    void* p = nullptr; size_t bytes = 0;
    void ensure(size_t n, size_t* total) {
        if (n <= bytes) return;
        if (p) { cudaFree(p); *total -= bytes; }
// ... 112 lines not shown
        int Nt = Ln;
        auto tw_entry = [](int j, int rr, int Nt_) {
            const long num = ((long)j * rr) % Nt_;
            const double a = -2.0 * M_PI * (double)num / (double)Nt_;
            cplx<T> wv; wv.x = (T)std::cos(a); wv.y = (T)std::sin(a);
            return wv;
        };
        for (size_t i = 0; i < r.size(); ++i) {
            const int R = r[i], S = Nt / R;
            dev.twoff[i] = (int)st.size();
            if (TwLayout<T>::paired) {
                for (int p = 0; p < R / 2; ++p)
                    for (int j = 0; j < S; ++j)
                        for (int e = 0; e < 2; ++e) {
                            const int rr = 2 * p + 1 + e;
                            cplx<T> one; one.x = (T)1; one.y = (T)0;
                            st.push_back(rr < R ? tw_entry(j, rr, Nt) : one);
                        }
            } else {
                for (int rr = 1; rr < R; ++rr)
                    for (int j = 0; j < S; ++j) st.push_back(tw_entry(j, rr, Nt));
            }
            Nt = S;
        }
        if (st.empty()) st.resize(1);
        twst.ensure(sizeof(cplx<T>) * st.size(), total);
        CK(cudaMemcpy(twst.p, st.data(), sizeof(cplx<T>) * st.size(), cudaMemcpyHostToDevice));
        dev.twst = twst.as<cplx<T>>();
    }
    void release(size_t* total) { tw.release(total); rev.release(total); pos.release(total); twst.release(total); }
};

template <class T>
struct Geom {
    int D = 0;
    int L[3] = {1, 1, 1};
    int H = 1;
    long P = 0;
    LineFftHost<T> fcol[2];
    LineFftHost<T> frow;
    DevBuf twL, twLp, part, pairq, pairs, pairw, quadq, quadw;
    int npair0 = 0, nquad = 0;
    bool built = false;
    void build(int D_, const int* L_, size_t* total) {
        D = D_;
        for (int d = 0; d < D; ++d) L[d] = L_[d];
        H = L[D - 1] / 2;
        P = ((long)H + 1 + 7) / 8 * 8;
        for (int d = 0; d + 1 < D; ++d) fcol[d].build(L[d], total);
        frow.build(H, total);
        std::vector<cplx<T>> w(H);
        for (int k = 0; k < H; ++k) {
            const double a = -2.0 * M_PI * (double)k / (double)L[D - 1];
            w[k].x = (T)std::cos(a); w[k].y = (T)std::sin(a);
        }
        twL.ensure(sizeof(cplx<T>) * H, total);
        CK(cudaMemcpy(twL.p, w.data(), sizeof(cplx<T>) * H, cudaMemcpyHostToDevice));
        std::vector<cplx<T>> wp(H); std::vector<int> pt(H);
        for (int q = 0; q < H; ++q) {
            const int k = frow.hrev_[q];
            wp[q] = w[k];
            pt[q] = k == 0 ? 0 : frow.hpos_[H - k];
        }
        std::vector<int> pq;
        for (int q = 0; q < H; ++q) if (q <= pt[q]) pq.push_back(q);
        if ((int)pq.size() != H / 2 + 1) throw Error("internal: r2c pair table has the wrong size");
        pairq.ensure(sizeof(int) * pq.size(), total);
        CK(cudaMemcpy(pairq.p, pq.data(), sizeof(int) * pq.size(), cudaMemcpyHostToDevice));
        {
            const std::vector<int> rad = H > 1 ? choose_radices(H) : std::vector<int>();
            const int RL = rad.empty() ? 1 : rad.back();
            bool ok = rad.size() > 1 && RL % 2 == 0 && H % 2 == 0;
            std::vector<int> qd; std::vector<cplx<T>> qw;
            for (int qa = RL; ok && qa < H; qa += 2) {
                const int pa = pt[qa], pa1 = pt[qa + 1];
                if (pa != pa1 + 1 || (pa1 & 1) || pa1 < RL) { ok = false; break; }
                if (qa <= pa1) { qd.push_back(qa); qd.push_back(pa1); qw.push_back(wp[qa]); qw.push_back(wp[qa + 1]); }
            }
            if (!ok) { qd.clear(); qw.clear(); }
            nquad = (int)(qd.size() / 2);
            npair0 = 0;
            if (ok) { for (int q : pq) if (q < RL) ++npair0; } else npair0 = (int)pq.size();
            if (npair0 + 2 * nquad - (ok ? 0 : 0) < 0) throw Error("internal: quad table");
            std::vector<int> pr; std::vector<cplx<T>> pw;
            for (int q : pq) { pr.push_back(q); pr.push_back(q == 0 ? H : pt[q]); pw.push_back(wp[q]); }
            pairs.ensure(sizeof(int) * pr.size(), total); pairw.ensure(sizeof(cplx<T>) * pw.size(), total);
            CK(cudaMemcpy(pairs.p, pr.data(), sizeof(int) * pr.size(), cudaMemcpyHostToDevice));
            CK(cudaMemcpy(pairw.p, pw.data(), sizeof(cplx<T>) * pw.size(), cudaMemcpyHostToDevice));
            quadq.ensure(sizeof(int) * std::max<size_t>(qd.size(), 2), total); quadw.ensure(sizeof(cplx<T>) * std::max<size_t>(qw.size(), 2), total);
            if (!qd.empty()) {
                CK(cudaMemcpy(quadq.p, qd.data(), sizeof(int) * qd.size(), cudaMemcpyHostToDevice));
                CK(cudaMemcpy(quadw.p, qw.data(), sizeof(cplx<T>) * qw.size(), cudaMemcpyHostToDevice));
            }
        }
        twLp.ensure(sizeof(cplx<T>) * H, total); part.ensure(sizeof(int) * H, total);
        CK(cudaMemcpy(twLp.p, wp.data(), sizeof(cplx<T>) * H, cudaMemcpyHostToDevice));
        CK(cudaMemcpy(part.p, pt.data(), sizeof(int) * H, cudaMemcpyHostToDevice));
        built = true;
    }
    long spec_elems() const { long n = P; for (int d = 0; d + 1 < D; ++d) n *= L[d]; return n; }
    void release(size_t* total) { for (auto& f : fcol) f.release(total); frow.release(total); twL.release(total); twLp.release(total); part.release(total); pairq.release(total); pairs.release(total); pairw.release(total); quadq.release(total); quadw.release(total); built = false; }
};

struct RowsFusion {
    int mode = 0, dot_kind = 0, do_fft = 1;
    const void* in = nullptr; void* out = nullptr; void* v0 = nullptr; void* v1 = nullptr; const void* v2 = nullptr;
};

}

using namespace hipgp;

struct hipgp_plan {
    int dtype = 0, device = 0;
    int ndim_user = 0;
    std::vector<long> m_user;
    int D = 0;
    int m[3] = {1, 1, 1}, N[3] = {1, 1, 1};
    long M = 1, E = 1;
    int Ln[3] = {1, 1, 1}, Lw[3] = {1, 1, 1};
    size_t dev_bytes = 0;
    long launches = 0;
    bool have_spec = false, have_wide = false;
    bool wide_real = false;
    double clampv = 1e-6;
    long nclamped = 0;

    Geom<float> gn32, gw32;
    Geom<double> gn64, gw64;
    DevBuf specK, specCinv, specW;
    DevBuf Dm, Dinv, Dsqrt, colK, colG, colS, tmpA, tmpB, costab, counts;
    DevBuf W1, W2;
    DevBuf vr, vp, vz, vAp, partial, scal, cnt, flags;
    DevBuf stage_in, stage_out;
    DevBuf slabSpecK, slabSpecCinv;
    bool have_slabK = false, have_slabCinv = false;
    DevBuf costabs[3], cosmats[3];
    DevBuf gradA;
    DevBuf corrU, corrV, corrS, corrLag;
    void* pinned = nullptr;
    cudaStream_t copy_streams[2] = {nullptr, nullptr};
    DevBuf slot_in[2], slot_out[2];
    cudaEvent_t slot_ev[2][3] = {{nullptr, nullptr, nullptr}, {nullptr, nullptr, nullptr}};
    bool slot_busy[2] = {false, false};
    int* slot_flags = nullptr;
    long pcg_B = 0;
    DevBuf slabR1, slabR2;
    void* peerR1[16] = {}; void* peerR2[16] = {};
    void* ipc_opened[32] = {}; int n_ipc_opened = 0;
    bool peers_ready = false;
    int slab_chunks = 1;
    int slab_rank = 0, slab_nranks = 1;
    void* run_x = nullptr; long run_B = 0; bool run_precond = true; double run_tol = 0; bool run_active = false;
    bool profiling = false;
    struct ProfRec { int cls; cudaEvent_t e0, e1; };
    std::vector<ProfRec> prof;
    double prof_ms[4] = {0, 0, 0, 0};
    long prof_n[4] = {0, 0, 0, 0};
};

#ifdef HIPGP_EMU
#define PROF_BEGIN(pl, cls, st) ((void)0)
#define PROF_END(pl, st) ((void)0)
#else
#define PROF_BEGIN(pl, cls_, st)                                                   \
    if ((pl)->profiling) {                                                         \
        hipgp_plan::ProfRec r__; r__.cls = (cls_);                                 \
        cudaEventCreate(&r__.e0); cudaEventCreate(&r__.e1);                        \
        cudaEventRecord(r__.e0, (st)); (pl)->prof.push_back(r__);                  \
    }
#define PROF_END(pl, st) if ((pl)->profiling) cudaEventRecord((pl)->prof.back().e1, (st));
#endif


namespace hipgp {
template <class T, int LEN> void launch_rows_fast_len(hipgp_plan* pl, bool inverse, RowsParams<T>& P, cudaStream_t st);
template <class T, int LEN> bool launch_cols_fast_len(hipgp_plan* pl, ColsParams<T>& P, long n_outer, long B, cudaStream_t st);
}
```

Baseline: 452.0.

## Defer PCG x update into next p-update pass, add L2 hints and reversed tile order

Moves the x += alpha*p update out of the residual-update pass and fuses it into the next iteration's p-update pass, where the old p is already being read. A final close kernel applies any pending update. This removes one full read of p per iteration. It also adds L2 eviction-policy hints on bulk and vector loads/stores, and alternates tile traversal direction between passes so recently touched data is still in L2. The cost is more bookkeeping (alpha storage, flags, a close kernel plus a sync before callbacks), and the x-pending state could go stale.

```diff
diff --git a/hipgp_b200/csrc/cols_blk_kernel.cuh b/hipgp_b200/csrc/cols_blk_kernel.cuh
--- a/hipgp_b200/csrc/cols_blk_kernel.cuh
+++ b/hipgp_b200/csrc/cols_blk_kernel.cuh
@@ -111,7 +111,7 @@
     const long ntiles = (long)P.nx * P.ny * P.nz;
     unsigned tile_bz = 0;
     auto tile_origin = [&](long t, long& c0, size_t& ioff, size_t& ooff) {
-        const unsigned tt = (unsigned)t, nx = (unsigned)P.nx, ny = (unsigned)P.ny, nz = (unsigned)P.nz;
+        const unsigned tt = (unsigned)(P.rev ? ntiles - 1 - t : t), nx = (unsigned)P.nx, ny = (unsigned)P.ny, nz = (unsigned)P.nz;
         unsigned bx, by, bz;
         if (P.batch_fastest) { bz = tt % nz; const unsigned r = tt / nz; bx = r % nx; by = r / nx; }
         else { bx = tt % nx; const unsigned r = tt / nx; by = r % ny; bz = r / ny; }
diff --git a/hipgp_b200/csrc/conv_kernels.cuh b/hipgp_b200/csrc/conv_kernels.cuh
--- a/hipgp_b200/csrc/conv_kernels.cuh
+++ b/hipgp_b200/csrc/conv_kernels.cuh
@@ -19,6 +19,7 @@
     unsigned* row_cnt;
     unsigned* rhs_cnt;
     int* flags;
+    double* alpha;
     double tol;
     int B;
     int cg_mode;
@@ -109,6 +110,8 @@
     int vec16_ok;
     int tma_ok;
     int tma_op;
+    int rev;
+    int l2_ef;
     const void* spec; int spec_kind;
     PcgDev st;
 };
@@ -134,13 +137,19 @@
         const int b = (int)(g / P.nrows);
         const size_t off = (size_t)g * n;
         T acc = 0;
-        T coef = 0;
+        T coef = 0, coefx = 0;
         bool first = false;
         if (P.mode == RF_PUPDATE) {
             first = P.st.flags[2] != 0;
             coef = first ? (T)0 : (T)(P.st.zr[b] / P.st.zr_prev[b]);
+            if (P.v1 && !first) coefx = (T)P.st.alpha[b];
         } else if (P.mode == RF_XRUPDATE) {
-            coef = (T)(P.st.zr[b] / P.st.pAp[b]);
+            const double q = P.st.zr[b] / P.st.pAp[b];
+            coef = (T)q;
+            if (!P.v1) {
+                if (lane == 0 && g == (long)b * P.nrows) P.st.alpha[b] = q;
+                if (lane == 0 && blockIdx.x == 0 && line == warp) P.st.flags[3] = 1;
+            }
         }
         for (int k = lane; k < H; k += 32) {
             T e[2];
@@ -153,14 +162,17 @@
                         val = P.in[off + i];
                     } else if (P.mode == RF_PUPDATE) {
                         const T z = P.in[off + i];
+                        if (P.v1 && !first) P.v1[off + i] = P.v1[off + i] + coefx * P.v0[off + i];
                         val = first ? z : z + coef * P.v0[off + i];
                         P.v0[off + i] = val;
                     } else if (P.mode == RF_SELFDOT) {
                         val = P.in[off + i];
                         acc += val * val;
                     } else {
-                        const T pv = P.v2[off + i];
-                        P.v1[off + i] = P.v1[off + i] + coef * pv;
+                        if (P.v1) {
+                            const T pv = P.v2[off + i];
+                            P.v1[off + i] = P.v1[off + i] + coef * pv;
+                        }
                         val = P.v0[off + i] - coef * P.in[off + i];
                         P.v0[off + i] = val;
                         acc += val * val;
@@ -306,6 +318,7 @@
     int tma_in, tma_in_rows, tma_in_nbox;
     int tma_spec;
     int batch_fastest;
+    int rev;
     const int* done_flag;
     int out_split_len; long out_split_stride;
     int in_split_len; long in_split_stride;
diff --git a/hipgp_b200/csrc/fast_kernels.cuh b/hipgp_b200/csrc/fast_kernels.cuh
--- a/hipgp_b200/csrc/fast_kernels.cuh
+++ b/hipgp_b200/csrc/fast_kernels.cuh
@@ -50,6 +50,7 @@
     const size_t spitch = P.spec_pitch ? (size_t)P.spec_pitch : (size_t)P.pitch;
     const long ntiles = (long)P.nx * P.ny * P.nz;
     auto tile_origin = [&](long t, long& c0, size_t& ioff, size_t& ooff) {
+        if (P.rev) t = ntiles - 1 - t;
         long bx, by, bz;
         if (P.batch_fastest) { bz = t % P.nz; const long r = t / P.nz; bx = r % P.nx; by = r / P.nx; }
         else { bx = t % P.nx; const long r = t / P.nx; by = r % P.ny; bz = r / P.ny; }
@@ -269,7 +270,7 @@
     Lane<T>* s = reinterpret_cast<Lane<T>*>(smem_raw);
     const int tid = threadIdx.x;
     if (P.mode != RF_PLAIN && P.st.flags[0]) return;
-    const long g0 = (long)blockIdx.x * NROW;
+    const long g0 = (long)(P.rev ? gridDim.x - 1 - blockIdx.x : blockIdx.x) * NROW;
     const long g1 = g0 + NROW < P.total_rows ? g0 + NROW : P.total_rows;
     const int nl = (int)(g1 - g0);
     const int n = P.n_real;
@@ -277,7 +278,10 @@
     const bool vec = ((n & 1) == 0) && P.vec_ok;
     const bool first_it = (mode == RF_PUPDATE) && (P.st.flags[2] != 0);
     const bool want_dot = (mode == RF_XRUPDATE || mode == RF_SELFDOT);
-    __shared__ T s_coef[32];
+    const bool x_def = mode == RF_XRUPDATE && !P.v1;
+    const bool x_pend = mode == RF_PUPDATE && !first_it && P.v1;
+    const L2Pol pol = l2_policy(P.l2_ef != 0);
+    __shared__ T s_coef[32], s_coefx[32];
     __shared__ long s_wbase[32];
     __shared__ double s_part[32];
     if (tid < NROW && tid < nl) {
@@ -285,10 +289,17 @@
         const long b = gr / P.nrows;
         s_wbase[tid] = (b * P.W_rows + (gr - b * P.nrows)) * P.W_pitch;
         T coef = 0;
-        if (mode == RF_PUPDATE) coef = first_it ? (T)0 : (T)(P.st.zr[b] / P.st.zr_prev[b]);
-        else if (mode == RF_XRUPDATE) coef = (T)(P.st.zr[b] / P.st.pAp[b]);
+        if (mode == RF_PUPDATE) {
+            coef = first_it ? (T)0 : (T)(P.st.zr[b] / P.st.zr_prev[b]);
+            if (x_pend) s_coefx[tid] = (T)P.st.alpha[b];
+        } else if (mode == RF_XRUPDATE) {
+            const double q = P.st.zr[b] / P.st.pAp[b];
+            coef = (T)q;
+            if (x_def && gr == b * P.nrows) P.st.alpha[b] = q;
+        }
         s_coef[tid] = coef;
     }
+    if (x_def && blockIdx.x == 0 && tid == 0) P.st.flags[3] = 1;
     __syncthreads();
 
     const int SROW = (n + 3) & ~3;
@@ -303,14 +314,14 @@
         const size_t goff = (size_t)g0 * n;
         T* bufA = reinterpret_cast<T*>(smem_raw);
         T* bufB = bufA + (size_t)NROW * SROW;
-        const bool two = mode == RF_PUPDATE && !first_it, three = mode == RF_XRUPDATE;
+        const bool two = (mode == RF_PUPDATE && !first_it) || x_def, three = mode == RF_XRUPDATE && !x_def;
         if (tid == 0) { mbar_init(&s_mbar, 1); fence_proxy_async(); }
         __syncthreads();
         if (tid == 0) {
             mbar_arrive_expect_tx(&s_mbar, bytes * (three ? 3u : (two ? 2u : 1u)));
-            bulk_g2s(side, P.in + goff, bytes, &s_mbar);
-            if (two) bulk_g2s(bufA, (const T*)P.v0 + goff, bytes, &s_mbar);
-            if (three) { bulk_g2s(bufA, (const T*)P.v0 + goff, bytes, &s_mbar); bulk_g2s(bufB, P.v2 + goff, bytes, &s_mbar); }
+            bulk_g2s_hint(side, P.in + goff, bytes, &s_mbar, pol);
+            if (two) bulk_g2s_hint(bufA, (const T*)P.v0 + goff, bytes, &s_mbar, pol);
+            if (three) { bulk_g2s_hint(bufA, (const T*)P.v0 + goff, bytes, &s_mbar, pol); bulk_g2s_hint(bufB, P.v2 + goff, bytes, &s_mbar, pol); }
         }
         constexpr int NW = NT / 32, WPR = NW > NROW ? NW / NROW : 1;
         constexpr int tws = WPR > 1 ? 32 : (H / CH >= 32 ? 32 : (H / CH >= 16 ? 16 : (H / CH >= 8 ? 8 : 4)));
@@ -335,7 +346,7 @@
                         for (int cb = ln; cb < nch; cb += TW * BS) {
                             Vec16<T> xv[BS];
 #pragma unroll
-                            for (int k = 0; k < BS; ++k) { const int c = cb + TW * k; if (c < nch) xv[k] = ldv_stream((const T*)P.v1 + off + (size_t)c * CH); }
+                            for (int k = 0; k < BS; ++k) { const int c = cb + TW * k; if (c < nch) xv[k] = ldv_hint((const T*)P.v1 + off + (size_t)c * CH, pol); }
 #pragma unroll
                             for (int k = 0; k < BS; ++k) {
                                 const int c = cb + TW * k;
@@ -345,8 +356,36 @@
                                     const Vec16<T> pv = *reinterpret_cast<const Vec16<T>*>(brow + c * CH);
 #pragma unroll
                                     for (int e = 0; e < CH; ++e) { xv[k].v[e] = xv[k].v[e] + coef * pv.v[e]; q.v[e] = rv.v[e] - coef * q.v[e]; acc += (double)(q.v[e] * q.v[e]); }
-                                    stv_stream(P.v1 + off + (size_t)c * CH, xv[k]);
+                                    stv_hint(P.v1 + off + (size_t)c * CH, xv[k], pol);
                                     *reinterpret_cast<Vec16<T>*>(srow + c * CH) = q;
+                                }
+                            }
+                        }
+                    } else if (x_def) {
+                        for (int c = ln; c < nch; c += TW) {
+                            Vec16<T> q = *reinterpret_cast<const Vec16<T>*>(srow + c * CH);
+                            const Vec16<T> rv = *reinterpret_cast<const Vec16<T>*>(arow + c * CH);
+#pragma unroll
+                            for (int e = 0; e < CH; ++e) { q.v[e] = rv.v[e] - coef * q.v[e]; acc += (double)(q.v[e] * q.v[e]); }
+                            *reinterpret_cast<Vec16<T>*>(srow + c * CH) = q;
+                        }
+                    } else if (x_pend) {
+                        constexpr int BS = 4;
+                        const T coefx = s_coefx[row];
+                        for (int cb = ln; cb < nch; cb += TW * BS) {
+                            Vec16<T> xv[BS];
+#pragma unroll
+                            for (int k = 0; k < BS; ++k) { const int c = cb + TW * k; if (c < nch) xv[k] = ldv_hint((const T*)P.v1 + off + (size_t)c * CH, pol); }
+#pragma unroll
+                            for (int k = 0; k < BS; ++k) {
+                                const int c = cb + TW * k;
+                                if (c < nch) {
+                                    Vec16<T> z = *reinterpret_cast<const Vec16<T>*>(srow + c * CH);
+                                    const Vec16<T> pv = *reinterpret_cast<const Vec16<T>*>(arow + c * CH);
+#pragma unroll
+                                    for (int e = 0; e < CH; ++e) { xv[k].v[e] = xv[k].v[e] + coefx * pv.v[e]; z.v[e] = z.v[e] + coef * pv.v[e]; }
+                                    stv_hint(P.v1 + off + (size_t)c * CH, xv[k], pol);
+                                    *reinterpret_cast<Vec16<T>*>(srow + c * CH) = z;
                                 }
                             }
                         }
@@ -375,10 +414,7 @@
         if (mode == RF_PUPDATE || mode == RF_XRUPDATE) {
             fence_proxy_async();
             __syncthreads();
-            if (tid == 0) {
-                asm volatile("cp.async.bulk.global.shared::cta.bulk_group [%0], [%1], %2;" ::"l"(P.v0 + goff), "r"((unsigned)__cvta_generic_to_shared(side)), "r"(bytes) : "memory");
-                asm volatile("cp.async.bulk.commit_group;" ::: "memory");
-            }
+            if (tid == 0) bulk_s2g_issue_hint(P.v0 + goff, side, bytes, pol);
             bulk_store_pending = true;
         }
         if (want_dot) {
@@ -427,7 +463,27 @@
                         if (cb + step < nch) { PROC(1, cb + step); }                                        \
                     }                                                                                       \
                 }
-                if (mode == RF_XRUPDATE) {
+                if (x_def) {
+                    constexpr int BS = 2;
+                    Vec16<T> a[2][BS], rv[2][BS];
+#define HIPGP_LD(S, CB)                                                                                     \
+                    _Pragma("unroll") for (int k = 0; k < BS; ++k) {                                        \
+                        const int c = (CB) + TW * k;                                                        \
+                        if (c < nch) { const size_t o = off + (size_t)c * CH; a[S][k] = ldv_hint(P.in + o, pol); rv[S][k] = ldv_hint((const T*)P.v0 + o, pol); } \
+                    }
+#define HIPGP_PR(S, CB)                                                                                     \
+                    _Pragma("unroll") for (int k = 0; k < BS; ++k) {                                        \
+                        const int c = (CB) + TW * k;                                                        \
+                        if (c < nch) {                                                                      \
+                            _Pragma("unroll") for (int e = 0; e < CH; ++e) a[S][k].v[e] = rv[S][k].v[e] - coef * a[S][k].v[e]; \
+                            stv_hint(P.v0 + off + (size_t)c * CH, a[S][k], pol);                            \
+                            finish(c, a[S][k]);                                                             \
+                        }                                                                                   \
+                    }
+                    HIPGP_PIPE(HIPGP_LD, HIPGP_PR)
+#undef HIPGP_LD
+#undef HIPGP_PR
+                } else if (mode == RF_XRUPDATE) {
                     constexpr int BS = 1;
                     Vec16<T> a[2][BS], pv[2][BS], xv[2][BS], rv[2][BS];
 #define HIPGP_LD(S, CB)                                                                                     \
@@ -456,6 +512,36 @@
                     HIPGP_PIPE(HIPGP_LD, HIPGP_PR)
 #undef HIPGP_LD
 #undef HIPGP_PR
+                } else if (x_pend) {
+                    constexpr int BS = 1;
+                    const T coefx = s_coefx[ractive ? row : 0];
+                    Vec16<T> a[2][BS], pv[2][BS], xv[2][BS];
+#define HIPGP_LD(S, CB)                                                                                     \
+                    _Pragma("unroll") for (int k = 0; k < BS; ++k) {                                        \
+                        const int c = (CB) + TW * k;                                                        \
+                        if (c < nch) {                                                                      \
+                            const size_t o = off + (size_t)c * CH;                                          \
+                            a[S][k] = ldv_hint(P.in + o, pol); pv[S][k] = ldv_hint((const T*)P.v0 + o, pol); \
+                            xv[S][k] = ldv_hint((const T*)P.v1 + o, pol);                                   \
+                        }                                                                                   \
+                    }
+#define HIPGP_PR(S, CB)                                                                                     \
+                    _Pragma("unroll") for (int k = 0; k < BS; ++k) {                                        \
+                        const int c = (CB) + TW * k;                                                        \
+                        if (c < nch) {                                                                      \
+                            const size_t o = off + (size_t)c * CH;                                          \
+                            _Pragma("unroll") for (int e = 0; e < CH; ++e) {                                \
+                                xv[S][k].v[e] = xv[S][k].v[e] + coefx * pv[S][k].v[e];                      \
+                                a[S][k].v[e] = a[S][k].v[e] + coef * pv[S][k].v[e];                         \
+                            }                                                                               \
+                            stv_hint(P.v1 + o, xv[S][k], pol);                                              \
+                            stv_hint(P.v0 + o, a[S][k], pol);                                               \
+                            finish(c, a[S][k]);                                                             \
+                        }                                                                                   \
+                    }
+                    HIPGP_PIPE(HIPGP_LD, HIPGP_PR)
+#undef HIPGP_LD
+#undef HIPGP_PR
                 } else if (mode == RF_PUPDATE && !first_it) {
                     constexpr int BS = 2;
                     Vec16<T> a[2][BS], pv[2][BS];
@@ -497,11 +583,14 @@
                     const size_t o = off + i;
                     T a = ld_stream(P.in + o);
                     if (mode == RF_PUPDATE) {
+                        if (x_pend) { const T pv = ld_stream((const T*)P.v0 + o); st_stream(P.v1 + o, ld_stream((const T*)P.v1 + o) + s_coefx[row] * pv); }
                         if (!first_it) a = a + coef * ld_stream((const T*)P.v0 + o);
                         st_stream(P.v0 + o, a);
                     } else if (mode == RF_XRUPDATE) {
-                        const T pv = ld_stream(P.v2 + o);
-                        st_stream(P.v1 + o, ld_stream((const T*)P.v1 + o) + coef * pv);
+                        if (!x_def) {
+                            const T pv = ld_stream(P.v2 + o);
+                            st_stream(P.v1 + o, ld_stream((const T*)P.v1 + o) + coef * pv);
+                        }
                         a = ld_stream((const T*)P.v0 + o) - coef * a;
                         st_stream(P.v0 + o, a);
                     }
@@ -651,7 +740,8 @@
     Lane<T>* s = reinterpret_cast<Lane<T>*>(smem_raw);
     const int tid = threadIdx.x;
     if (P.mode != RI_PLAIN && P.st.flags[0]) return;
-    const long g0 = (long)blockIdx.x * NROW;
+    const long g0 = (long)(P.rev ? gridDim.x - 1 - blockIdx.x : blockIdx.x) * NROW;
+    const L2Pol pol = l2_policy(P.l2_ef != 0);
     const long g1 = g0 + NROW < P.total_rows ? g0 + NROW : P.total_rows;
     const int nl = (int)(g1 - g0);
     const int n = P.n_real;
@@ -718,8 +808,8 @@
             for (int l = 0; l < LPT; ++l) {
                 const int row = lane * LPT + l;
                 const cplx<T>* src = P.W + s_wbase[row < nl ? row : nl - 1];
-                WRow<T>::load2(src, qq[k].a, ya[k][l], ya1[k][l]);
-                WRow<T>::load2(src, qq[k].b, yb[k][l], yb1[k][l]);
+                WRow<T>::load2(src, qq[k].a, ya[k][l], ya1[k][l], pol);
+                WRow<T>::load2(src, qq[k].b, yb[k][l], yb1[k][l], pol);
             }
         }
 #pragma unroll
@@ -839,7 +929,7 @@
                     Vec16<T> ov[BS];
                     if (want_dot) {
 #pragma unroll
-                        for (int k = 0; k < BS; ++k) { const int c = cb + TW * k; if (c < nch) ov[k] = ldv_stream((const T*)P.v0 + off + (size_t)c * CH); }
+                        for (int k = 0; k < BS; ++k) { const int c = cb + TW * k; if (c < nch) ov[k] = ldv_hint((const T*)P.v0 + off + (size_t)c * CH, pol); }
                     }
 #pragma unroll
                     for (int k = 0; k < BS; ++k) {
diff --git a/hipgp_b200/csrc/fast_launch.cuh b/hipgp_b200/csrc/fast_launch.cuh
--- a/hipgp_b200/csrc/fast_launch.cuh
+++ b/hipgp_b200/csrc/fast_launch.cuh
@@ -4,6 +4,12 @@
 #include "cols_blk_kernel.cuh"
 
 namespace hipgp {
+
+static int next_pass_rev(hipgp_plan* pl) {
+    if (pl->pass_forward) return 0;
+    pl->pass_dir ^= 1;
+    return pl->pass_dir;
+}
 
 constexpr int cfg_min(int a, int b) { return a < b ? a : b; }
 constexpr int cfg_max(int a, int b) { return a > b ? a : b; }
@@ -59,6 +65,8 @@
     P.tma_ok = env_nt ? 0 : 1;
     P.tma_op = (!env_nf && !inverse && 2 * sizeof(T) * (size_t)((P.n_real + 3) & ~3) * NROW <= G::smem_bytes()) ? 1 : 0;
     dim3 grid((unsigned)((P.total_rows + NROW - 1) / NROW));
+    P.rev = next_pass_rev(pl);
+    P.l2_ef = pl->l2_hints ? 1 : 0;
     PROF_BEGIN(pl, inverse ? 2 : 0, st);
     if (inverse) {
         auto k = rows_inv_fast_kernel<T, C::NLR, C::NTR, C::MINBR, Rs...>;
@@ -112,6 +120,7 @@
     if (smem > 40 * 1024) HIPGP_SET_MAX_SMEM(k, smem);
     const long ntiles = (long)P.nx * P.ny * P.nz;
     const long grid = std::min<long>(ntiles, resident_ctas(k, C::NTC, smem));
+    P.rev = next_pass_rev(pl);
     PROF_BEGIN(pl, 1, st);
     HIPGP_LAUNCH(k, dim3((unsigned)grid), dim3(C::NTC), smem, st, P);
     PROF_END(pl, st);
@@ -173,6 +182,7 @@
             if (smem > 40 * 1024) HIPGP_SET_MAX_SMEM(k, smem);
             const long ntiles = (long)P.nx * P.ny * P.nz;
             const long grid = std::min<long>(ntiles, resident_ctas(k, C::NTC, smem));
+            P.rev = next_pass_rev(pl);
             PROF_BEGIN(pl, 1, st);
             HIPGP_LAUNCH(k, dim3((unsigned)grid), dim3(C::NTC), smem, st, P, maps);
             PROF_END(pl, st);
diff --git a/hipgp_b200/csrc/lane_fft.cuh b/hipgp_b200/csrc/lane_fft.cuh
--- a/hipgp_b200/csrc/lane_fft.cuh
+++ b/hipgp_b200/csrc/lane_fft.cuh
@@ -129,6 +129,61 @@
 #endif
 }
 
+#ifdef HIPGP_EMU
+typedef unsigned long long L2Pol;
+__device__ __forceinline__ L2Pol l2_policy(bool) { return 0; }
+template <class T> __device__ __forceinline__ Vec16<T> ldv_hint(const T* p, L2Pol) { return *reinterpret_cast<const Vec16<T>*>(p); }
+template <class T> __device__ __forceinline__ void stv_hint(T* p, Vec16<T> v, L2Pol) { *reinterpret_cast<Vec16<T>*>(p) = v; }
+template <class T> __device__ __forceinline__ Lane<T> lane_from_global_hint(const cplx<T>* p, L2Pol) { return lane_from_global(p); }
+template <class V> __device__ __forceinline__ V ld_hint(const V* p, L2Pol) { return *p; }
+#else
+typedef unsigned long long L2Pol;
+__device__ __forceinline__ L2Pol l2_policy(bool ef) {
+    L2Pol p;
+    if (ef) asm volatile("createpolicy.fractional.L2::evict_first.b64 %0, 1.0;" : "=l"(p));
+    else asm volatile("createpolicy.fractional.L2::evict_normal.b64 %0, 1.0;" : "=l"(p));
+    return p;
+}
+__device__ __forceinline__ Vec16<float> ldv_hint(const float* p, L2Pol pol) {
+    Vec16<float> r;
+    asm volatile("ld.global.cg.L2::cache_hint.v4.f32 {%0, %1, %2, %3}, [%4], %5;" : "=f"(r.v[0]), "=f"(r.v[1]), "=f"(r.v[2]), "=f"(r.v[3]) : "l"(p), "l"(pol));
+    return r;
+}
+__device__ __forceinline__ Vec16<double> ldv_hint(const double* p, L2Pol pol) {
+    Vec16<double> r;
+    asm volatile("ld.global.cg.L2::cache_hint.v2.f64 {%0, %1}, [%2], %3;" : "=d"(r.v[0]), "=d"(r.v[1]) : "l"(p), "l"(pol));
+    return r;
+}
+__device__ __forceinline__ void stv_hint(float* p, Vec16<float> v, L2Pol pol) {
+    asm volatile("st.global.cg.L2::cache_hint.v4.f32 [%0], {%1, %2, %3, %4}, %5;" ::"l"(p), "f"(v.v[0]), "f"(v.v[1]), "f"(v.v[2]), "f"(v.v[3]), "l"(pol) : "memory");
+}
+__device__ __forceinline__ void stv_hint(double* p, Vec16<double> v, L2Pol pol) {
+    asm volatile("st.global.cg.L2::cache_hint.v2.f64 [%0], {%1, %2}, %3;" ::"l"(p), "d"(v.v[0]), "d"(v.v[1]), "l"(pol) : "memory");
+}
+__device__ __forceinline__ Lane<float> lane_from_global_hint(const cplx<float>* p, L2Pol pol) {
+    const Vec16<float> t = ldv_hint(reinterpret_cast<const float*>(p), pol);
+    Lane<float> r; r.re = make_float2(t.v[0], t.v[1]); r.im = make_float2(t.v[2], t.v[3]); return r;
+}
+__device__ __forceinline__ Lane<double> lane_from_global_hint(const cplx<double>* p, L2Pol pol) {
+    const Vec16<double> t = ldv_hint(reinterpret_cast<const double*>(p), pol);
+    Lane<double> r; r.re = t.v[0]; r.im = t.v[1]; return r;
+}
+__device__ __forceinline__ float ld_hint(const float* p, L2Pol pol) {
+    float r; asm volatile("ld.global.cg.L2::cache_hint.f32 %0, [%1], %2;" : "=f"(r) : "l"(p), "l"(pol)); return r;
+}
+__device__ __forceinline__ cplx<double> ld_hint(const cplx<double>* p, L2Pol pol) {
+    const Vec16<double> t = ldv_hint(reinterpret_cast<const double*>(p), pol); return mk<double>(t.v[0], t.v[1]);
+}
+__device__ __forceinline__ void bulk_g2s_hint(void* smem_dst, const void* gmem_src, unsigned bytes, unsigned long long* bar, L2Pol pol) {
+    asm volatile("cp.async.bulk.shared::cluster.global.mbarrier::complete_tx::bytes.L2::cache_hint [%0], [%1], %2, [%3], %4;"
+                 ::"r"((unsigned)__cvta_generic_to_shared(smem_dst)), "l"(gmem_src), "r"(bytes), "r"((unsigned)__cvta_generic_to_shared(bar)), "l"(pol) : "memory");
+}
+__device__ __forceinline__ void bulk_s2g_issue_hint(void* gmem_dst, const void* smem_src, unsigned bytes, L2Pol pol) {
+    asm volatile("cp.async.bulk.global.shared::cta.bulk_group.L2::cache_hint [%0], [%1], %2, %3;" ::"l"(gmem_dst), "r"((unsigned)__cvta_generic_to_shared(smem_src)), "r"(bytes), "l"(pol) : "memory");
+    asm volatile("cp.async.bulk.commit_group;" ::: "memory");
+}
+#endif
+
 __device__ __forceinline__ float2 pack2(float a, float b) {
 #ifdef HIPGP_EMU
     return make_float2(a, b);
@@ -159,12 +214,19 @@
         const Lane<float> t = lane_from_global(row + q);
         v0 = mk<float>(t.re.x, t.im.x); v1 = mk<float>(t.re.y, t.im.y);
     }
+    static __device__ __forceinline__ void load2(const cplx<float>* row, int q, cplx<float>& v0, cplx<float>& v1, L2Pol pol) {
+        const Lane<float> t = lane_from_global_hint(row + q, pol);
+        v0 = mk<float>(t.re.x, t.im.x); v1 = mk<float>(t.re.y, t.im.y);
+    }
 };
 template <> struct WRow<double> {
     static __device__ __forceinline__ void store1(cplx<double>* row, int q, cplx<double> v) { st_stream(row + q, v); }
     static __device__ __forceinline__ cplx<double> load1(const cplx<double>* row, int q) { return ld_stream(row + q); }
     static __device__ __forceinline__ void store2(cplx<double>* row, int q, cplx<double> v0, cplx<double> v1) { st_stream(row + q, v0); st_stream(row + q + 1, v1); }
     static __device__ __forceinline__ void load2(const cplx<double>* row, int q, cplx<double>& v0, cplx<double>& v1) { v0 = ld_stream(row + q); v1 = ld_stream(row + q + 1); }
+    static __device__ __forceinline__ void load2(const cplx<double>* row, int q, cplx<double>& v0, cplx<double>& v1, L2Pol pol) {
+        v0 = ld_hint(row + q, pol); v1 = ld_hint(row + q + 1, pol);
+    }
 };
 
 template <int BYTES> __device__ __forceinline__ void cp_async(void* smem_dst, const void* gmem_src) {
@@ -424,4 +486,26 @@
     }
 };
 
-}
+template <class T>
+__global__ void __launch_bounds__(256) pcg_close_x_kernel(T* x, const T* p, const double* alpha, const int* flags, long M, int vec) {
+    if (!flags[3]) return;
+    const int b = blockIdx.y;
+    const T coef = (T)alpha[b];
+    T* xb = x + (size_t)b * M;
+    const T* pb = p + (size_t)b * M;
+    const long i0 = (long)blockIdx.x * blockDim.x + threadIdx.x, stride = (long)gridDim.x * blockDim.x;
+    if (vec) {
+        constexpr int CH = 16 / (int)sizeof(T);
+        for (long c = i0; c < M / CH; c += stride) {
+            Vec16<T> xv = ldv_stream(xb + c * CH);
+            const Vec16<T> pv = ldv_stream(pb + c * CH);
+#pragma unroll
+            for (int e = 0; e < CH; ++e) xv.v[e] = xv.v[e] + coef * pv.v[e];
+            stv_stream(xb + c * CH, xv);
+        }
+    } else {
+        for (long i = i0; i < M; i += stride) xb[i] = xb[i] + coef * pb[i];
+    }
+}
+
+}
diff --git a/hipgp_b200/csrc/plan.cu b/hipgp_b200/csrc/plan.cu
--- a/hipgp_b200/csrc/plan.cu
+++ b/hipgp_b200/csrc/plan.cu
@@ -1,4 +1,5 @@
 #include "plan_types.cuh"
+#include "lane_fft.cuh"
 #include "setup_kernels.cuh"
 #include "kxu_kernels.cuh"
 
@@ -216,6 +217,7 @@
             s2.zr = st.zr + b0; s2.zr_prev = st.zr_prev + b0; s2.pAp = st.pAp + b0; s2.rr = st.rr + b0;
             s2.rr_all = st.rr_all ? st.rr_all : st.rr;
             s2.row_cnt = st.row_cnt + b0;
+            s2.alpha = st.alpha + b0;
             s2.partial = st.partial + b0 * std::max(rows_in, rows_out);
         }
         run_pipeline_group<T>(pl, g, n_in, n_out, spec, spec_kind, nb, f2, i2, s2, gated, s);
@@ -456,14 +458,14 @@
     for (int d = 0; d + 1 < pl->D; ++d) nrows *= pl->m[d];
     for (DevBuf* b : {&pl->vr, &pl->vp, &pl->vz, &pl->vAp}) b->ensure(sizeof(T) * (size_t)(B * M), &pl->dev_bytes);
     pl->partial.ensure(sizeof(double) * (size_t)(B * nrows), &pl->dev_bytes);
-    pl->scal.ensure(sizeof(double) * (size_t)(4 * B), &pl->dev_bytes);
+    pl->scal.ensure(sizeof(double) * (size_t)(5 * B), &pl->dev_bytes);
     const bool fresh = pl->cnt.bytes < sizeof(unsigned) * (size_t)(B + 1);
     pl->cnt.ensure(sizeof(unsigned) * (size_t)(B + 1), &pl->dev_bytes);
     pl->flags.ensure(sizeof(int) * 4, &pl->dev_bytes);
     if (fresh) CK(cudaMemset(pl->cnt.p, 0, pl->cnt.bytes));
     PcgDev st{};
     double* sc = pl->scal.as<double>();
-    st.zr = sc; st.zr_prev = sc + B; st.pAp = sc + 2 * B; st.rr = sc + 3 * B;
+    st.zr = sc; st.zr_prev = sc + B; st.pAp = sc + 2 * B; st.rr = sc + 3 * B; st.alpha = sc + 4 * B;
     st.partial = pl->partial.as<double>();
     st.row_cnt = pl->cnt.as<unsigned>(); st.rhs_cnt = pl->cnt.as<unsigned>() + B;
     st.flags = pl->flags.as<int>();
@@ -513,6 +515,7 @@
         launch_vec<T>(pl, RF_SELFDOT, st, B, r, nullptr, nullptr, nullptr, s);
     }
     pl->run_x = x; pl->run_B = B; pl->run_precond = precond; pl->run_tol = tol; pl->run_active = true;
+    pl->x_pending = false;
 }
 
 template <class T>
@@ -526,21 +529,44 @@
     for (int d = 0; d < pl->D; ++d) nn[d] = pl->m[d];
     T* r = pl->vr.as<T>(); T* p = pl->vp.as<T>(); T* z = precond ? pl->vz.as<T>() : r; T* Ap = pl->vAp.as<T>();
     void* x = pl->run_x;
+    const bool defer = !pl->eager_x;
     RowsFusion ff, fi;
     for (int c = 0; c < niter; ++c) {
         ff = RowsFusion(); fi = RowsFusion();
-        ff.mode = RF_PUPDATE; ff.in = z; ff.v0 = p;
+        ff.mode = RF_PUPDATE; ff.in = z; ff.v0 = p; ff.v1 = pl->x_pending ? x : nullptr;
         fi.mode = RI_DOT; fi.dot_kind = DOT_PAP; fi.out = Ap; fi.v0 = p;
         run_pipeline<T>(pl, g, nn, nn, pl->specK.p, SPEC_REAL, B, ff, fi, st, true, s);
+        void* xu = defer ? nullptr : x;
+        const void* pu = defer ? nullptr : p;
         if (precond) {
             ff = RowsFusion(); fi = RowsFusion();
-            ff.mode = RF_XRUPDATE; ff.in = Ap; ff.v0 = r; ff.v1 = x; ff.v2 = p;
+            ff.mode = RF_XRUPDATE; ff.in = Ap; ff.v0 = r; ff.v1 = xu; ff.v2 = pu;
             fi.mode = RI_DOT; fi.dot_kind = DOT_ZR; fi.out = z; fi.v0 = r;
             run_pipeline<T>(pl, g, nn, nn, pl->specCinv.p, SPEC_REAL, B, ff, fi, st, true, s);
         } else {
-            launch_vec<T>(pl, RF_XRUPDATE, st, B, Ap, r, x, p, s);
+            launch_vec<T>(pl, RF_XRUPDATE, st, B, Ap, r, xu, pu, s);
         }
-    }
+        pl->x_pending = defer;
+    }
+}
+
+template <class T>
+static void pcg_close_x(hipgp_plan* pl, cudaStream_t s) {
+    if (!pl->x_pending) return;
+    const long B = pl->run_B, M = pl->M;
+    T* x = (T*)pl->run_x;
+    const T* p = pl->vp.as<T>();
+    constexpr long CH = 16 / (long)sizeof(T);
+    const int vec = (M % CH == 0 && (uintptr_t)x % 16 == 0 && (uintptr_t)p % 16 == 0) ? 1 : 0;
+    const long work = vec ? M / CH : M;
+    const unsigned bx = (unsigned)std::max<long>(1, std::min<long>((work + 255) / 256, (148L * 16 + B - 1) / B));
+    auto k = pcg_close_x_kernel<T>;
+    PROF_BEGIN(pl, 3, s);
+    HIPGP_LAUNCH(k, dim3(bx, (unsigned)B), dim3(256), 0, s, x, p, pl->scal.as<double>() + 4 * B, pl->flags.as<int>(), M, vec);
+    PROF_END(pl, s);
+    CK_LAUNCH(); pl->launches++;
+    CK(cudaMemsetAsync(pl->flags.as<int>() + 3, 0, sizeof(int), s));
+    pl->x_pending = false;
 }
 
 static void pcg_poll(hipgp_plan* pl, int* done, int* iters, double* max_resid, double* resid_out, cudaStream_t s) {
@@ -577,8 +603,9 @@
         pcg_iterate<T>(pl, chunk, s);
         pcg_poll(pl, &done, &iters, nullptr, nullptr, s);
         n += chunk;
-        if (cb && !done) cb(n - 1, x, user);
-    }
+        if (cb && !done) { pcg_close_x<T>(pl, s); CK(cudaStreamSynchronize(s)); cb(n - 1, x, user); }
+    }
+    pcg_close_x<T>(pl, s);
     if (iters_out) *iters_out = iters;
     if (callbacks_out) *callbacks_out = done ? iters - 1 : iters;
     if (resid_out) pcg_poll(pl, nullptr, nullptr, nullptr, resid_out, s);
@@ -630,6 +657,12 @@
     pl->D = D;
     const char* nf = getenv("HIPGP_NO_FAST");
     g_no_fast = nf && nf[0] == '1';
+    const char* ex = getenv("HIPGP_EAGER_X");
+    pl->eager_x = ex && ex[0] == '1';
+    const char* po = getenv("HIPGP_PASS_ORDER");
+    pl->pass_forward = po && std::string(po) == "forward";
+    const char* lh = getenv("HIPGP_L2_HINTS");
+    pl->l2_hints = !(lh && lh[0] == '0');
     const char* env = getenv("HIPGP_POW2_ONLY");
     const bool pow2 = env && env[0] == '1';
     for (int d = 0; d < D; ++d) {
@@ -756,7 +789,7 @@
     API_BEGIN
     set_device(pl);
     cudaStream_t s = (cudaStream_t)stream;
-    DISPATCH(pl, pcg_iterate<float>(pl, niter, s), pcg_iterate<double>(pl, niter, s));
+    DISPATCH(pl, (pcg_iterate<float>(pl, niter, s), pcg_close_x<float>(pl, s)), (pcg_iterate<double>(pl, niter, s), pcg_close_x<double>(pl, s)));
     if (done_out || iters_out || max_resid_out) pcg_poll(pl, done_out, iters_out, max_resid_out, nullptr, s);
     API_END
 }
@@ -872,8 +905,8 @@
     CK(cudaEventRecord(pl->slot_ev[slot][0], cin));
     CK(cudaStreamWaitEvent(s, pl->slot_ev[slot][0], 0));
 #endif
-    if (pl->dtype == HIPGP_F32) { pcg_begin<float>(pl, pl->slot_in[slot].p, pl->slot_out[slot].p, (long)B, tol, precond != 0, s); pcg_iterate<float>(pl, maxiter, s); }
-    else { pcg_begin<double>(pl, pl->slot_in[slot].p, pl->slot_out[slot].p, (long)B, tol, precond != 0, s); pcg_iterate<double>(pl, maxiter, s); }
+    if (pl->dtype == HIPGP_F32) { pcg_begin<float>(pl, pl->slot_in[slot].p, pl->slot_out[slot].p, (long)B, tol, precond != 0, s); pcg_iterate<float>(pl, maxiter, s); pcg_close_x<float>(pl, s); }
+    else { pcg_begin<double>(pl, pl->slot_in[slot].p, pl->slot_out[slot].p, (long)B, tol, precond != 0, s); pcg_iterate<double>(pl, maxiter, s); pcg_close_x<double>(pl, s); }
     pl->run_active = false;
     CK(cudaMemcpyAsync(pl->slot_flags + 4 * slot, pl->flags.p, sizeof(int) * 4, cudaMemcpyDeviceToHost, s));
 #ifndef HIPGP_EMU
diff --git a/hipgp_b200/csrc/plan_types.cuh b/hipgp_b200/csrc/plan_types.cuh
--- a/hipgp_b200/csrc/plan_types.cuh
+++ b/hipgp_b200/csrc/plan_types.cuh
@@ -288,6 +288,9 @@
     int slab_chunks = 1;
     int slab_rank = 0, slab_nranks = 1;
     void* run_x = nullptr; long run_B = 0; bool run_precond = true; double run_tol = 0; bool run_active = false;
+    bool x_pending = false;
+    bool eager_x = false, pass_forward = false, l2_hints = true;
+    int pass_dir = 0;
     bool profiling = false;
     struct ProfRec { int cls; cudaEvent_t e0, e1; };
     std::vector<ProfRec> prof;
```

After: 456.0 (median of 6 runs). No clear change (+0.9%).
